# p1an-lin-jung/WavThruVec_pytorch

Hardware: AMD Instinct MI355X
Metric: audio samples/sec (16 kHz) Vec2Wav generator, B=32×256-frame 768-d latents, 1/2/4/8 GPU (higher is better)
Workload: dtype f32; 1 GPU; BASELINE configs[1]: B=32/GPU x T=256 frames, 768-d latents, upsample (5,4,4,2,2) x320, ResBlock2, train-mode CondBN, f32; global_batch=32, frames=256, parallelism=single GPU

## Files before the change

### include/vec2wav_hip.h

```cpp
#ifndef VEC2WAV_HIP_H
#define VEC2WAV_HIP_H

#include <stdint.h>

#ifdef __cplusplus
extern "C" {
#endif

#define V2W_ABI_VERSION 35

#define V2W_E_ARG      (-1)
#define V2W_E_SHAPE    (-2)
#define V2W_E_ALGO     (-3)

#define V2W_ALGO_AUTO   0
#define V2W_ALGO_DIRECT 1
#define V2W_ALGO_MFMA   2
#define V2W_ALGO_BF16   4
#define V2W_ALGO_SPLIT  3
#define V2W_ALGO_WINO   5

int         v2w_abi_version(void);
const char* v2w_build_arch(void);

// ... 86 lines not shown
typedef struct {
    const float* in; const float* in_a; const float* in_s;
    const float* wp1[4]; const float* bias1[4]; const float* wp2[4]; const float* bias2[4];
    int32_t k[4], dil1[4], dil2[4];
    float* out;
    int32_t nk, B, C, L;
    float slope, out_div;
    const float* post_w; const float* post_b; float* post_out;
    int32_t post_k;
    float post_slope;
    const float* bwd_mask1[4]; float* bwd_mid[4];
    const float* bwd_mask2; const float* bwd_mask2_a; const float* bwd_mask2_s;
    float bwd_slope;
    float* bwd_rowsum[4];
} v2w_stage_args;
int v2w_resblock2_stage_fwd(const v2w_stage_args* a, void* stream);
int v2w_resblock2_stage_bwd_rows(const v2w_stage_args* a);
int v2w_resblock2_stage_wino_fwd(const v2w_stage_args* a, void* stream);
int v2w_resblock2_stage_wino_tile(const v2w_stage_args* a);
int v2w_resblock2_stage_wino_fwd_len(const v2w_stage_args* a, const int32_t* len, int len_mul, void* stream);
int v2w_resblock2_stage_small_fwd(const v2w_stage_args* a, void* stream);

typedef struct {
    const float* in; const float* in_a; const float* in_s;
    const void*  wps1[4]; const float* sc1[4]; const float* bias1[4];
    const void*  wps2[4]; const float* sc2[4]; const float* bias2[4];
    int32_t k[4], dil1[4], dil2[4];
    float* out;
    int32_t nk, B, C, L;
    float slope, out_div;
    int32_t bf16;
    int32_t io_bf16;
    const float* post_w; const float* post_b; float* post_out;
    int32_t post_k;
    float post_slope;
    const void* up_wps; const float* up_bias; void* up_out; float* up_stats_part;
    int32_t up_k, up_u;
    float up_slope;
    int32_t rb1;
    const void* in_b[4]; void* out_b[4];
    const void* add0; const void* add1;
} v2w_stage_split_args;
int v2w_resblock2_stage_split_fwd(const v2w_stage_split_args* a, void* stream);
int v2w_resblock2_stage_split_config(const v2w_stage_split_args* a);
int v2w_resblock2_stage_up_tiles(const v2w_stage_split_args* a);

typedef struct {
    const void* in[3];
    const float* in_a; const float* in_s;
    const void* wps[3]; const float* bias[3];
    void* out[3];
    int32_t k[3], dil[3];
    int32_t nbr, mode, B, C, L;
    float slope, out_div;
    int32_t _pad;
} v2w_branch_convs_args;
int v2w_branch_convs_bf16_fwd(const v2w_branch_convs_args* a, void* stream);

typedef struct {
    const float* in; const float* wf; const float* wp; const float* bias; float* out;
    float* stats_part;
    int32_t B, C_in, C_out, L, k, u;
    float   slope;
    int32_t algo;
    int32_t io_bf16;
    int32_t _pad;
    float*  splitk_ws;
    int64_t splitk_ws_bytes;
} v2w_convt1d_args;
int v2w_convt1d_fwd(const v2w_convt1d_args* a, void* stream);
long long v2w_convt1d_splitk_ws_bytes(const v2w_convt1d_args* a);

int       v2w_pack_bf16_convt(const float* wf, void* wps, int k, int c_in, int c_out, int u, void* stream);
long long v2w_pack_bf16_convt_bytes(int k, int c_in, int c_out, int u);
int       v2w_convt1d_bf16_fwd(const v2w_convt1d_args* a, void* stream);
int       v2w_convt1d_bf16_tiles(const v2w_convt1d_args* a);

int v2w_conv1d_tile_config(const v2w_conv1d_args* a, int32_t* cfg);
int v2w_convt1d_tile_config(const v2w_convt1d_args* a, int32_t* cfg);
int v2w_conv1d_bf16_config(const v2w_conv1d_args* a, int n, int32_t* cfg);
int v2w_convt1d_bf16_config(const v2w_convt1d_args* a, int32_t* cfg);

#define V2W_MAX_STAGES 8
typedef struct {
    const float* spk; const float* noise;
    const float* fc_w[V2W_MAX_STAGES]; const float* fc_b[V2W_MAX_STAGES];
    const float* sn_w[V2W_MAX_STAGES]; const float* sn_b[V2W_MAX_STAGES];
    float* sn_u[V2W_MAX_STAGES]; float* sn_v[V2W_MAX_STAGES];
    float* gb[V2W_MAX_STAGES];
    int32_t C[V2W_MAX_STAGES];
    float* z_ws; float* sigma_ws;
    int32_t n_stages, B, spk_dim, noise_dim, training;
} v2w_cond_args;
int v2w_cond_gamma_beta(const v2w_cond_args* a, void* stream);
int v2w_cond_sigma(const v2w_cond_args* a, void* stream);
typedef struct {
    v2w_cond_args c;
    const float* running_mean[V2W_MAX_STAGES]; const float* running_var[V2W_MAX_STAGES];
    float* a_out[V2W_MAX_STAGES]; float* s_out[V2W_MAX_STAGES];
    float eps[V2W_MAX_STAGES];
} v2w_cond_eval_args;
int v2w_cond_affine_eval(const v2w_cond_eval_args* e, void* stream);

#define V2W_BN_SPLITS 64
int v2w_bn_stats(const float* x, double* stats, double* partial_ws, int B, int C, int L, void* stream);
int v2w_bn_reduce_partials(const float* part, int ntiles, int C, double count, double* stats, void* stream);
int v2w_bn_finalize(const double* stats, const float* gb,
                    float* running_mean, float* running_var, int64_t* num_batches_tracked,
                    float* a_out, float* s_out, int B, int C, int training,
                    float momentum, float eps, void* stream);
int v2w_bn_reduce_finalize(const float* part, int ntiles, double count, const float* gb,
                           float* running_mean, float* running_var, int64_t* num_batches_tracked,
                           double* stats, float* a_out, float* s_out, int B, int C, float momentum, float eps, void* stream);
int v2w_bn_reduce_slices(const float* part, int ntiles, int C, double* slices, int nslices, void* stream);
int v2w_bn_finalize_slices(const double* slices, int nslices, double count, const float* gb,
                           float* running_mean, float* running_var, int64_t* num_batches_tracked,
                           float* a_out, float* s_out, int B, int C, float momentum, float eps, void* stream);

int v2w_affine_apply(const float* x, const float* a, const float* s, float* out, int B, int C, int L, void* stream);

int v2w_wgrad_slabs(int B, int c_in, int c_out, int Lq);
int v2w_wgrad(const float* x, const float* x_a, const float* x_s, const float* dy, float* dwf, float* slab_ws,
              int B, int c_in, int c_out, int Lq, int k, int dil, int u, float slope, void* stream);

int v2w_wgrad_bf16_slabs(int B, int c_in, int c_out, int Lq, int k);
int v2w_wgrad_bf16(const void* x, const float* x_a, const float* x_s, const void* dy, float* dwf, float* slab_ws,
                   int B, int c_in, int c_out, int Lq, int k, int dil, float slope, int io_bf16, void* stream);

int v2w_cbn_bwd_sums(const float* dx, const float* xr, const float* gb, const double* stats,
                     const float* running_mean, const float* running_var, float* s12_ws, float* dgb, double* csum,
                     int B, int C, int L, int training, float eps, void* stream);
int v2w_cbn_bwd_apply(const float* dx, const float* xr, const float* gb, const double* stats, const double* csum,
                      const float* running_mean, const float* running_var, float* tab_ws, float* dxr,
                      int B, int C, int L, int training, float eps, void* stream);
int v2w_tail_bwd(const float* dy, const float* y, const float* x, const float* wf, float* dp_ws, double* part_ws,
                 float* dx, float* dwf, int B, int C_in, int L, int k, float slope, void* stream);
int v2w_wn_bwd(const float* dwf, const float* v, const float* g, float* dv, float* dg,
               int c_in, int c_out, int k, int transposed, void* stream);
int v2w_cond_bwd(const float* dgb, const float* z, const float* sn_w, const float* sn_u, const float* sn_v, const float* sigma,
                 const float* spk, const float* noise, float* d_sn_w, float* d_sn_b, float* d_fc_w, float* d_fc_b,
                 float* dz_ws, int B, int C, int spk_dim, int noise_dim, void* stream);

int v2w_conv_post_tanh_bf16in(const void* x_bf16, const float* wf, const float* bias, float* out,
                              int B, int c_in, int L, int k, float slope, void* stream);
int v2w_conv_post_tanh(const float* in, const float* wf, const float* bias, float* out,
                       int B, int C_in, int L, int k, float slope, void* stream);

int v2w_conv1d_fwd_len(const v2w_conv1d_args* a, int n, const int32_t* len, int len_mul, void* stream);
int v2w_convt1d_fwd_len(const v2w_convt1d_args* a, const int32_t* len, int len_mul, void* stream);
int v2w_conv1d_wino_sum_fwd(const v2w_conv1d_args* a, int n, const int32_t* len, int len_mul, void* stream);
int v2w_conv1d_wino_sum_fwd_order(const v2w_conv1d_args* a, int n, const int32_t* len, int len_mul, const int32_t* order, void* stream);
int v2w_wino_sum_order(const int32_t* k, int n, int32_t* order);
int v2w_conv1d_wino_fan_fwd(const v2w_conv1d_args* a, int n, void* stream);
int v2w_resblock2_stage_fwd_len(const v2w_stage_args* a, const int32_t* len, int len_mul, void* stream);
int v2w_conv_post_tanh_len(const float* in, const float* wf, const float* bias, float* out,
                           int B, int C_in, int L, int k, float slope, const int32_t* len, int len_mul, void* stream);

int v2w_mel_phases(const float* y, float* xp, int B, int L, int hop, int pad, int FP, void* stream);
int v2w_mel_finish(const float* spec, const float* basis, float* out, int B, int Cs, int FP, int F, int nb, int n_mels, void* stream);
int v2w_mel_finish_bwd(const float* spec, const float* basis, const float* basisT, const float* gout, float* dspec,
                       int B, int Cs, int FP, int F, int nb, int n_mels, void* stream);
int v2w_mel_phases_bwd(const float* dxp, float* dy, int B, int L, int hop, int pad, int FP, void* stream);
int v2w_mel_phases_len(const float* y, float* xp, int B, int L, int hop, int pad, int FP, const int32_t* len, int len_mul, void* stream);
int v2w_mel_finish_len(const float* spec, const float* basis, float* out, int B, int Cs, int FP, int F, int nb, int n_mels,
                       const int32_t* len, int len_mul, int hop, int n_fft, void* stream);
int v2w_mel_phases_geo(const float* y, float* xp, int B, int L, int n_fft, int win, int hop, int CP, int pad, int left, int k, int FP,
                       void* stream);
int v2w_mel_phases_geo_len(const float* y, float* xp, int B, int L, int n_fft, int win, int hop, int CP, int pad, int left, int k, int FP,
                           const int32_t* len, int len_mul, void* stream);
int v2w_mel_phases_geo_bwd(const float* dxp, float* dy, int B, int L, int n_fft, int win, int hop, int CP, int pad, int left, int k, int FP,
                           void* stream);
int v2w_mel_finish_geo(const float* spec, const float* basis, float* out, int B, int Cs, int FP, int F, int nb, int n_mels, void* stream);
int v2w_mel_finish_geo_len(const float* spec, const float* basis, float* out, int B, int Cs, int FP, int F, int nb, int n_mels,
                           const int32_t* len, int len_mul, int hop, int n_fft, void* stream);
int v2w_mel_finish_geo_bwd(const float* spec, const float* basis, const float* basisT, const float* gout, float* dspec,
                           int B, int Cs, int FP, int F, int nb, int n_mels, void* stream);

int v2w_phase_split(const float* x, float* out, int B, int C, int Cg, int L, int inner, int s, int ipitch, int opitch, void* stream);
int v2w_unfold1(const float* x, float* out, int B, int T, int H, int inner, int s, int k, int pad, int rows, int opitch, void* stream);
int v2w_zero_tail(float* x, long long rows, int pitch, int valid, void* stream);
int v2w_unfold_taps(const float* x, float* out, int B, int C, int L, int inner, int s, int k, int pad, int ipitch, int opitch, void* stream);
int v2w_avgpool4(const float* x, float* out, int B, int L, void* stream);

int v2w_wgrad_slice(const float* x, const float* dy, float* dwf, float* slab_ws, int B, int c_in, int c_out, int Lq,
                    int k, int dil, int tap0, int x_ct, int dy_ct, void* stream);
int v2w_wgrad_group_slabs(int B, int c_in, int c_out, int Lq, int ngroups);
int v2w_wgrad_groups(const float* x, const float* dy, float* dwf, float* slab_ws, int B, int c_in, int c_out, int Lq,
                     int k, int dil, int tap0, int ngroups, void* stream);
int v2w_disc_dz(const float* f, const float* g, const float* d, float* dz, float* rowsum, long long rows, int pitch, int valid, float slope,
                void* stream);
int v2w_rowsum_reduce(const float* rowsum, float* db, int B, int C, void* stream);
int v2w_disc_dz_merge(const float* f, const float* g, const float* dxs, float* dz, float* rowsum, int B, int C, int Cg, int L, int inner,
                      int s, int dpitch, int pitch, float slope, void* stream);
int v2w_phase_merge(const float* dxs, float* out, int B, int C, int Cg, int L, int inner, int s, int ipitch, int opitch, void* stream);
int v2w_fold1(const float* dxu, float* dx, int B, int T, int H, int inner, int s, int k, int pad, int rows, int ipitch, void* stream);
int v2w_avgpool4_bwd(const float* dout, float* dx, int B, int L, void* stream);
int v2w_cout1_wgrad(const float* x, const float* dz, float* dwf, int B, int C, int L, int k, int dil, int tap0, void* stream);

#define V2W_LOSS_MAX_ITEMS 64
#define V2W_L1_TARGET_WGS  2048
typedef struct {
    const float* a; const float* b;
    float* da; float* db;
    int64_t rows;
    int32_t valid, pitch_a, pitch_b, _pad;
} v2w_l1_pair;
typedef struct {
    const float* s;
    float* ds;
    int64_t rows;
    int32_t valid, pitch;
    float target;
    int32_t _pad;
} v2w_lsgan_item;
int       v2w_l1_multi_plan(const v2w_l1_pair* pairs, int n, int32_t* starts);
long long v2w_l1_multi_scratch_bytes(const v2w_l1_pair* pairs, int n);
int v2w_l1_mean_multi(const v2w_l1_pair* pairs, int n, float scale, float* term, float* total, void* scratch, void* stream);
int v2w_l1_mean_multi_bwd(const v2w_l1_pair* pairs, int n, float scale, const float* gout, void* stream);
int v2w_lsgan_multi(const v2w_lsgan_item* items, int n, float* term, float* total, void* stream);
int v2w_lsgan_multi_bwd(const v2w_lsgan_item* items, int n, const float* gout, const float* gterm, void* stream);
int v2w_l1_masked_plan(int C, int F);
int v2w_l1_masked(const float* a, const float* b, int B, int C, int F, const int32_t* len, int len_mul, int hop, int n_fft,
                  float* per_item, float* total, void* ws, void* stream);
int v2w_l1_masked_geo(const float* a, const float* b, int B, int C, int F, const int32_t* len, int len_mul, int hop, int n_fft,
                      float* per_item, float* total, void* ws, void* stream);

#define V2W_STFT_LOSS_MAX_ITEMS  8
#define V2W_STFT_LOSS_TARGET_WGS 1024
typedef struct {
    const float* spec_x; const float* spec_y;
    float* dspec_x;
    int32_t B, Cs, FP, F, nb, _pad;
} v2w_stft_loss_item;
int       v2w_stft_loss_plan(const v2w_stft_loss_item* items, int n, int32_t* starts);
long long v2w_stft_loss_scratch_bytes(const v2w_stft_loss_item* items, int n);
int v2w_stft_loss_multi(const v2w_stft_loss_item* items, int n, float* sc, float* mag, float* total, double* sums, void* scratch,
                        void* stream);
int v2w_stft_loss_multi_bwd(const v2w_stft_loss_item* items, int n, const double* sums, const float* g_sc, const float* g_mag,
                            const float* gterm_sc, const float* gterm_mag, void* stream);

#define V2W_ADAMW_MAX_ITEMS  80
#define V2W_ADAMW_TARGET_WGS 2048
typedef struct {
    float* p;
    const float* g;
    float* m;
    float* v;
    int64_t numel;
} v2w_adamw_item;
typedef struct {
    float lr, beta1, beta2, eps, weight_decay, bias_corr1, bias_corr2_sqrt;
    int32_t _pad;
} v2w_adamw_hyper;
int v2w_adamw_multi_plan(const v2w_adamw_item* items, int n, int32_t* starts);
int v2w_adamw_multi(const v2w_adamw_item* items, int n, const v2w_adamw_hyper* h, void* stream);

int v2w_grad_sumsq_partials(const v2w_adamw_item* items, int n);
int v2w_grad_sumsq_multi(const v2w_adamw_item* items, int n, float* partials, void* stream);
int v2w_grad_norm_finish(const float* partials, int n_partials, float max_norm, float* out, void* stream);
int v2w_scale_multi(const v2w_adamw_item* items, int n, const float* coef, void* stream);
int v2w_adamw_multi_clipped(const v2w_adamw_item* items, int n, const v2w_adamw_hyper* h, const float* clip, int skip_nonfinite, void* stream);

#define V2W_ADAMW_EMA_MAX_ITEMS 64
typedef struct {
    float* p;
    const float* g;
    float* m;
    float* v;
    float* e;
    int64_t numel;
} v2w_adamw_ema_item;
typedef struct {
    const float* p;
    float* e;
    int64_t numel;
} v2w_ema_item;
typedef struct {
    float* p;
    float* e;
    int64_t numel;
} v2w_swap_item;
int v2w_adamw_ema_multi_plan(const v2w_adamw_ema_item* items, int n, int32_t* starts);
int v2w_adamw_ema_multi(const v2w_adamw_ema_item* items, int n, const v2w_adamw_hyper* h, const float* clip, int skip_nonfinite, float ema_omd,
                        void* stream);
int v2w_ema_multi_plan(const v2w_ema_item* items, int n, int32_t* starts);
int v2w_ema_multi(const v2w_ema_item* items, int n, float ema_omd, void* stream);
int v2w_swap_multi(const v2w_swap_item* items, int n, void* stream);

#define V2W_SN_MAX_LAYERS 64
typedef struct {
    const float* w;
    float* u;
    float* v;
    float* wf;
    int32_t c_out, c_in, k;
    int32_t blk_t, blk_r, blk_s;
    int64_t ws_off, keep_off;
} v2w_sn_desc;
typedef struct {
    int32_t n, grid_t, grid_r, grid_s;
    int64_t ws_bytes, keep_bytes;
} v2w_sn_grids;
long long v2w_sn_plan(v2w_sn_desc* descs, int n, v2w_sn_grids* g);
int v2w_sn_step(const v2w_sn_desc* descs_dev, int n, int training, const v2w_sn_grids* g, float* keep, void* ws, long long ws_bytes,
                void* stream);
int v2w_sn_bwd(const v2w_sn_desc* descs_dev, int n, const v2w_sn_grids* g, const float* keep, const float* const* dwf, float* const* dw,
// ... 7 lines not shown
```

### wavthruvec_pytorch_amd/_hip.py

```python
from __future__ import annotations

import ctypes as C
import os
import threading

from . import build as _build

ABI_VERSION = 35
V2W_MAX_STAGES = 8
V2W_BN_SPLITS = 64
ALGO_AUTO, ALGO_DIRECT, ALGO_MFMA, ALGO_SPLIT, ALGO_BF16, ALGO_WINO = 0, 1, 2, 3, 4, 5

_fp = C.c_void_p


class Conv1dArgs(C.Structure):
    _fields_ = [('in_', _fp), ('in_a', _fp), ('in_s', _fp), ('wf', _fp), ('wp', _fp), ('bias', _fp),
                ('res', _fp), ('res_a', _fp), ('res_s', _fp), ('add0', _fp), ('add1', _fp),
                ('mask_src', _fp), ('mask_a', _fp), ('mask_s', _fp), ('out', _fp),
                ('B', C.c_int32), ('C_in', C.c_int32), ('C_out', C.c_int32), ('L', C.c_int32),
                ('k', C.c_int32), ('dil', C.c_int32), ('slope', C.c_float), ('accumulate', C.c_int32),
                ('out_div', C.c_float), ('algo', C.c_int32), ('mask_slope', C.c_float),
                ('in_stride', C.c_int32), ('in_phase', C.c_int32), ('pad_left', C.c_int32),
                ('wps', _fp), ('winv', _fp), ('in_ct', C.c_int32), ('out_ct', C.c_int32), ('out_slope', C.c_float),
# ... 74 lines not shown
    _fields_ = [('c', CondArgs), ('running_mean', _PA), ('running_var', _PA), ('a_out', _PA), ('s_out', _PA),
                ('eps', C.c_float * V2W_MAX_STAGES)]


class L1Pair(C.Structure):
    _fields_ = [('a', _fp), ('b', _fp), ('da', _fp), ('db', _fp), ('rows', C.c_int64),
                ('valid', C.c_int32), ('pitch_a', C.c_int32), ('pitch_b', C.c_int32), ('_pad', C.c_int32)]


class LsganItem(C.Structure):
    _fields_ = [('s', _fp), ('ds', _fp), ('rows', C.c_int64), ('valid', C.c_int32), ('pitch', C.c_int32),
                ('target', C.c_float), ('_pad', C.c_int32)]


LOSS_MAX_ITEMS = 64
L1_TARGET_WGS = 2048


class StftLossItem(C.Structure):
    _fields_ = [('spec_x', _fp), ('spec_y', _fp), ('dspec_x', _fp), ('B', C.c_int32), ('Cs', C.c_int32), ('FP', C.c_int32),
                ('F', C.c_int32), ('nb', C.c_int32), ('_pad', C.c_int32)]


STFT_LOSS_MAX_ITEMS = 8
STFT_LOSS_TARGET_WGS = 1024


class AdamWItem(C.Structure):
    _fields_ = [('p', _fp), ('g', _fp), ('m', _fp), ('v', _fp), ('numel', C.c_int64)]


class AdamWHyper(C.Structure):
    _fields_ = [('lr', C.c_float), ('beta1', C.c_float), ('beta2', C.c_float), ('eps', C.c_float), ('weight_decay', C.c_float),
                ('bias_corr1', C.c_float), ('bias_corr2_sqrt', C.c_float), ('_pad', C.c_int32)]


ADAMW_MAX_ITEMS = 80
ADAMW_TARGET_WGS = 2048


class AdamWEmaItem(C.Structure):
    _fields_ = [('p', _fp), ('g', _fp), ('m', _fp), ('v', _fp), ('e', _fp), ('numel', C.c_int64)]


class EmaItem(C.Structure):
    _fields_ = [('p', _fp), ('e', _fp), ('numel', C.c_int64)]


ADAMW_EMA_MAX_ITEMS = 64


class SnDesc(C.Structure):
    _fields_ = [('w', _fp), ('u', _fp), ('v', _fp), ('wf', _fp), ('c_out', C.c_int32), ('c_in', C.c_int32), ('k', C.c_int32),
                ('blk_t', C.c_int32), ('blk_r', C.c_int32), ('blk_s', C.c_int32), ('ws_off', C.c_int64), ('keep_off', C.c_int64)]


class SnGrids(C.Structure):
    _fields_ = [('n', C.c_int32), ('grid_t', C.c_int32), ('grid_r', C.c_int32), ('grid_s', C.c_int32), ('ws_bytes', C.c_int64), ('keep_bytes', C.c_int64)]


SN_MAX_LAYERS = 64

SIGNATURES = {
    'v2w_abi_version': (C.c_int, []),
    'v2w_build_arch': (C.c_char_p, []),
    'v2w_wn_fold_conv': (C.c_int, [_fp, _fp, _fp, _fp, C.c_int, C.c_int, C.c_int, _fp]),
    'v2w_wn_fold_convt': (C.c_int, [_fp, _fp, _fp, _fp, C.c_int, C.c_int, C.c_int, _fp]),
    'v2w_wf_transpose_flip': (C.c_int, [_fp, _fp, C.c_int, C.c_int, C.c_int, _fp]),
    'v2w_wf_gather_transpose': (C.c_int, [_fp, _fp, C.c_int, C.c_int, C.c_int, C.c_int, C.c_int, C.c_int, _fp]),
    'v2w_pack_mfma': (C.c_int, [_fp, _fp, C.c_int, C.c_int, C.c_int, C.c_int, _fp]),
    'v2w_pack_mfma_batch': (C.c_int, [_fp, _fp, C.c_int, C.c_int, C.c_int, C.c_int, C.c_int, _fp]),
    'v2w_pack_mfma_dgrad': (C.c_int, [_fp, _fp, C.c_int, C.c_int, C.c_int, _fp]),
    'v2w_pack_wino': (C.c_int, [_fp, _fp, C.c_int, C.c_int, C.c_int, _fp]),
    'v2w_wino_terms': (C.c_int, [C.c_int]),
    'v2w_split_supported': (C.c_int, [C.c_int, C.c_int, C.c_int]),
    'v2w_pack_split': (C.c_int, [_fp, _fp, _fp, C.c_int, C.c_int, C.c_int, _fp]),
    'v2w_mel_phases': (C.c_int, [_fp, _fp, C.c_int, C.c_int, C.c_int, C.c_int, C.c_int, _fp]),
    'v2w_mel_finish': (C.c_int, [_fp, _fp, _fp, C.c_int, C.c_int, C.c_int, C.c_int, C.c_int, C.c_int, _fp]),
    'v2w_mel_finish_bwd': (C.c_int, [_fp, _fp, _fp, _fp, _fp, C.c_int, C.c_int, C.c_int, C.c_int, C.c_int, C.c_int, _fp]),
    'v2w_phase_split': (C.c_int, [_fp, _fp, C.c_int, C.c_int, C.c_int, C.c_int, C.c_int, C.c_int, C.c_int, C.c_int, _fp]),
    'v2w_unfold1': (C.c_int, [_fp, _fp, C.c_int, C.c_int, C.c_int, C.c_int, C.c_int, C.c_int, C.c_int, C.c_int, C.c_int, _fp]),
    'v2w_unfold_taps': (C.c_int, [_fp, _fp] + [C.c_int] * 9 + [_fp]),
    'v2w_wgrad_slice': (C.c_int, [_fp, _fp, _fp, _fp] + [C.c_int] * 9 + [_fp]),
    'v2w_wgrad_group_slabs': (C.c_int, [C.c_int] * 5),
    'v2w_wgrad_groups': (C.c_int, [_fp, _fp, _fp, _fp] + [C.c_int] * 8 + [_fp]),
    'v2w_disc_dz': (C.c_int, [_fp, _fp, _fp, _fp, _fp, C.c_longlong, C.c_int, C.c_int, C.c_float, _fp]),
    'v2w_rowsum_reduce': (C.c_int, [_fp, _fp, C.c_int, C.c_int, _fp]),
    'v2w_disc_dz_merge': (C.c_int, [_fp, _fp, _fp, _fp, _fp] + [C.c_int] * 8 + [C.c_float, _fp]),
    'v2w_phase_merge': (C.c_int, [_fp, _fp] + [C.c_int] * 8 + [_fp]),
    'v2w_fold1': (C.c_int, [_fp, _fp] + [C.c_int] * 9 + [_fp]),
    'v2w_avgpool4_bwd': (C.c_int, [_fp, _fp, C.c_int, C.c_int, _fp]),
    'v2w_cout1_wgrad': (C.c_int, [_fp, _fp, _fp] + [C.c_int] * 6 + [_fp]),
    'v2w_zero_tail': (C.c_int, [_fp, C.c_longlong, C.c_int, C.c_int, _fp]),
    'v2w_avgpool4': (C.c_int, [_fp, _fp, C.c_int, C.c_int, _fp]),
    'v2w_mel_phases_bwd': (C.c_int, [_fp, _fp, C.c_int, C.c_int, C.c_int, C.c_int, C.c_int, _fp]),
    'v2w_split_packable': (C.c_int, [C.c_int, C.c_int]),
    'v2w_resblock2_stage_split_fwd': (C.c_int, [C.POINTER(StageSplitArgs), _fp]),
    'v2w_resblock2_stage_split_config': (C.c_int, [C.POINTER(StageSplitArgs)]),
    'v2w_resblock2_stage_up_tiles': (C.c_int, [C.POINTER(StageSplitArgs)]),
    'v2w_pack_bf16': (C.c_int, [_fp, _fp, _fp, C.c_int, C.c_int, C.c_int, _fp]),
    'v2w_split_pack_batch': (C.c_int, [_fp, _fp, C.c_int, C.c_int, C.c_int, C.c_int, C.c_int, _fp]),
    'v2w_fold_plan': (C.c_int, [C.POINTER(FoldDesc), C.c_int, C.POINTER(C.c_int32)]),
    'v2w_fold_pack_batch': (C.c_int, [_fp, _fp, C.c_int, C.c_int, C.c_int, C.c_int, _fp]),
    'v2w_conv1d_fwd': (C.c_int, [C.POINTER(Conv1dArgs), _fp]),
    'v2w_conv1d_fwd_multi': (C.c_int, [C.POINTER(Conv1dArgs), C.c_int, _fp]),
    'v2w_conv1d_splitk_ws_bytes': (C.c_longlong, [C.POINTER(Conv1dArgs), C.c_int]),
    'v2w_convt1d_splitk_ws_bytes': (C.c_longlong, [C.POINTER(ConvT1dArgs)]),
    'v2w_resblock_pair_fwd': (C.c_int, [C.POINTER(PairArgs), C.c_int, _fp]),
    'v2w_resblock2_stage_bwd_rows': (C.c_int, [C.POINTER(StageArgs)]),
    'v2w_resblock2_stage_fwd': (C.c_int, [C.POINTER(StageArgs), _fp]),
    'v2w_resblock2_stage_wino_fwd': (C.c_int, [C.POINTER(StageArgs), _fp]),
    'v2w_resblock2_stage_wino_tile': (C.c_int, [C.POINTER(StageArgs)]),
    'v2w_resblock2_stage_wino_fwd_len': (C.c_int, [C.POINTER(StageArgs), _fp, C.c_int, _fp]),
    'v2w_resblock2_stage_small_fwd': (C.c_int, [C.POINTER(StageArgs), _fp]),
    'v2w_branch_convs_bf16_fwd': (C.c_int, [C.POINTER(BranchConvsArgs), _fp]),
    'v2w_convt1d_fwd': (C.c_int, [C.POINTER(ConvT1dArgs), _fp]),
    'v2w_pack_bf16_convt': (C.c_int, [_fp, _fp, C.c_int, C.c_int, C.c_int, C.c_int, _fp]),
    'v2w_pack_bf16_convt_bytes': (C.c_longlong, [C.c_int, C.c_int, C.c_int, C.c_int]),
    'v2w_convt1d_bf16_fwd': (C.c_int, [C.POINTER(ConvT1dArgs), _fp]),
    'v2w_convt1d_bf16_tiles': (C.c_int, [C.POINTER(ConvT1dArgs)]),
    'v2w_conv1d_tile_config': (C.c_int, [C.POINTER(Conv1dArgs), C.POINTER(C.c_int32)]),
    'v2w_convt1d_tile_config': (C.c_int, [C.POINTER(ConvT1dArgs), C.POINTER(C.c_int32)]),
    'v2w_conv1d_bf16_config': (C.c_int, [C.POINTER(Conv1dArgs), C.c_int, C.POINTER(C.c_int32)]),
    'v2w_convt1d_bf16_config': (C.c_int, [C.POINTER(ConvT1dArgs), C.POINTER(C.c_int32)]),
    'v2w_cond_gamma_beta': (C.c_int, [C.POINTER(CondArgs), _fp]),
    'v2w_cond_sigma': (C.c_int, [C.POINTER(CondArgs), _fp]),
    'v2w_cond_affine_eval': (C.c_int, [C.POINTER(CondEvalArgs), _fp]),
    'v2w_bn_stats': (C.c_int, [_fp, _fp, _fp, C.c_int, C.c_int, C.c_int, _fp]),
    'v2w_bn_reduce_partials': (C.c_int, [_fp, C.c_int, C.c_int, C.c_double, _fp, _fp]),
    'v2w_bn_finalize': (C.c_int, [_fp, _fp, _fp, _fp, _fp, _fp, _fp, C.c_int, C.c_int, C.c_int,
                                  C.c_float, C.c_float, _fp]),
    'v2w_bn_reduce_finalize': (C.c_int, [_fp, C.c_int, C.c_double, _fp, _fp, _fp, _fp, _fp, _fp, _fp, C.c_int, C.c_int, C.c_float, C.c_float, _fp]),
    'v2w_bn_reduce_slices': (C.c_int, [_fp, C.c_int, C.c_int, _fp, C.c_int, _fp]),
    'v2w_bn_finalize_slices': (C.c_int, [_fp, C.c_int, C.c_double, _fp, _fp, _fp, _fp, _fp, _fp, C.c_int, C.c_int, C.c_float, C.c_float, _fp]),
    'v2w_affine_apply': (C.c_int, [_fp, _fp, _fp, _fp, C.c_int, C.c_int, C.c_int, _fp]),
    'v2w_wgrad_slabs': (C.c_int, [C.c_int, C.c_int, C.c_int, C.c_int]),
    'v2w_wgrad': (C.c_int, [_fp, _fp, _fp, _fp, _fp, _fp, C.c_int, C.c_int, C.c_int, C.c_int, C.c_int, C.c_int, C.c_int,
                            C.c_float, _fp]),
    'v2w_wgrad_bf16_slabs': (C.c_int, [C.c_int] * 5),
    'v2w_wgrad_bf16': (C.c_int, [_fp] * 6 + [C.c_int] * 6 + [C.c_float, C.c_int, _fp]),
    'v2w_cbn_bwd_sums': (C.c_int, [_fp] * 9 + [C.c_int, C.c_int, C.c_int, C.c_int, C.c_float, _fp]),
    'v2w_cbn_bwd_apply': (C.c_int, [_fp] * 9 + [C.c_int, C.c_int, C.c_int, C.c_int, C.c_float, _fp]),
    'v2w_tail_bwd': (C.c_int, [_fp] * 8 + [C.c_int, C.c_int, C.c_int, C.c_int, C.c_float, _fp]),
    'v2w_wn_bwd': (C.c_int, [_fp] * 5 + [C.c_int, C.c_int, C.c_int, C.c_int, _fp]),
    'v2w_cond_bwd': (C.c_int, [_fp] * 13 + [C.c_int, C.c_int, C.c_int, C.c_int, _fp]),
    'v2w_conv_post_tanh_bf16in': (C.c_int, [_fp, _fp, _fp, _fp, C.c_int, C.c_int, C.c_int, C.c_int, C.c_float, _fp]),
    'v2w_conv_post_tanh': (C.c_int, [_fp, _fp, _fp, _fp, C.c_int, C.c_int, C.c_int, C.c_int, C.c_float, _fp]),
    'v2w_conv1d_fwd_len': (C.c_int, [C.POINTER(Conv1dArgs), C.c_int, _fp, C.c_int, _fp]),
    'v2w_convt1d_fwd_len': (C.c_int, [C.POINTER(ConvT1dArgs), _fp, C.c_int, _fp]),
    'v2w_conv1d_wino_sum_fwd': (C.c_int, [C.POINTER(Conv1dArgs), C.c_int, _fp, C.c_int, _fp]),
    'v2w_conv1d_wino_sum_fwd_order': (C.c_int, [C.POINTER(Conv1dArgs), C.c_int, _fp, C.c_int, C.POINTER(C.c_int32), _fp]),
    'v2w_wino_sum_order': (C.c_int, [C.POINTER(C.c_int32), C.c_int, C.POINTER(C.c_int32)]),
    'v2w_conv1d_wino_fan_fwd': (C.c_int, [C.POINTER(Conv1dArgs), C.c_int, _fp]),
    'v2w_resblock2_stage_fwd_len': (C.c_int, [C.POINTER(StageArgs), _fp, C.c_int, _fp]),
    'v2w_conv_post_tanh_len': (C.c_int, [_fp, _fp, _fp, _fp, C.c_int, C.c_int, C.c_int, C.c_int, C.c_float, _fp, C.c_int, _fp]),
    'v2w_mel_phases_len': (C.c_int, [_fp, _fp, C.c_int, C.c_int, C.c_int, C.c_int, C.c_int, _fp, C.c_int, _fp]),
    'v2w_mel_finish_len': (C.c_int, [_fp, _fp, _fp, C.c_int, C.c_int, C.c_int, C.c_int, C.c_int, C.c_int, _fp, C.c_int, C.c_int, C.c_int, _fp]),
    'v2w_l1_masked_plan': (C.c_int, [C.c_int, C.c_int]),
    'v2w_l1_masked': (C.c_int, [_fp, _fp, C.c_int, C.c_int, C.c_int, _fp, C.c_int, C.c_int, C.c_int, _fp, _fp, _fp, _fp]),
    'v2w_mel_phases_geo': (C.c_int, [_fp, _fp] + [C.c_int] * 10 + [_fp]),
    'v2w_mel_phases_geo_len': (C.c_int, [_fp, _fp] + [C.c_int] * 10 + [_fp, C.c_int, _fp]),
    'v2w_mel_phases_geo_bwd': (C.c_int, [_fp, _fp] + [C.c_int] * 10 + [_fp]),
    'v2w_mel_finish_geo': (C.c_int, [_fp, _fp, _fp] + [C.c_int] * 6 + [_fp]),
    'v2w_mel_finish_geo_len': (C.c_int, [_fp, _fp, _fp] + [C.c_int] * 6 + [_fp, C.c_int, C.c_int, C.c_int, _fp]),
    'v2w_mel_finish_geo_bwd': (C.c_int, [_fp] * 5 + [C.c_int] * 6 + [_fp]),
    'v2w_l1_masked_geo': (C.c_int, [_fp, _fp, C.c_int, C.c_int, C.c_int, _fp, C.c_int, C.c_int, C.c_int, _fp, _fp, _fp, _fp]),
    'v2w_l1_multi_plan': (C.c_int, [C.POINTER(L1Pair), C.c_int, C.POINTER(C.c_int32)]),
    'v2w_l1_multi_scratch_bytes': (C.c_longlong, [C.POINTER(L1Pair), C.c_int]),
    'v2w_l1_mean_multi': (C.c_int, [C.POINTER(L1Pair), C.c_int, C.c_float, _fp, _fp, _fp, _fp]),
    'v2w_l1_mean_multi_bwd': (C.c_int, [C.POINTER(L1Pair), C.c_int, C.c_float, _fp, _fp]),
    'v2w_lsgan_multi': (C.c_int, [C.POINTER(LsganItem), C.c_int, _fp, _fp, _fp]),
    'v2w_lsgan_multi_bwd': (C.c_int, [C.POINTER(LsganItem), C.c_int, _fp, _fp, _fp]),
    'v2w_stft_loss_plan': (C.c_int, [C.POINTER(StftLossItem), C.c_int, C.POINTER(C.c_int32)]),
    'v2w_stft_loss_scratch_bytes': (C.c_longlong, [C.POINTER(StftLossItem), C.c_int]),
    'v2w_stft_loss_multi': (C.c_int, [C.POINTER(StftLossItem), C.c_int, _fp, _fp, _fp, _fp, _fp, _fp]),
    'v2w_stft_loss_multi_bwd': (C.c_int, [C.POINTER(StftLossItem), C.c_int, _fp, _fp, _fp, _fp, _fp, _fp]),
    'v2w_adamw_multi_plan': (C.c_int, [C.POINTER(AdamWItem), C.c_int, C.POINTER(C.c_int32)]),
    'v2w_adamw_multi': (C.c_int, [C.POINTER(AdamWItem), C.c_int, C.POINTER(AdamWHyper), _fp]),
    'v2w_grad_sumsq_partials': (C.c_int, [C.POINTER(AdamWItem), C.c_int]),
    'v2w_grad_sumsq_multi': (C.c_int, [C.POINTER(AdamWItem), C.c_int, _fp, _fp]),
    'v2w_grad_norm_finish': (C.c_int, [_fp, C.c_int, C.c_float, _fp, _fp]),
    'v2w_scale_multi': (C.c_int, [C.POINTER(AdamWItem), C.c_int, _fp, _fp]),
    'v2w_adamw_multi_clipped': (C.c_int, [C.POINTER(AdamWItem), C.c_int, C.POINTER(AdamWHyper), _fp, C.c_int, _fp]),
    'v2w_adamw_ema_multi_plan': (C.c_int, [C.POINTER(AdamWEmaItem), C.c_int, C.POINTER(C.c_int32)]),
    'v2w_adamw_ema_multi': (C.c_int, [C.POINTER(AdamWEmaItem), C.c_int, C.POINTER(AdamWHyper), _fp, C.c_int, C.c_float, _fp]),
    'v2w_ema_multi_plan': (C.c_int, [C.POINTER(EmaItem), C.c_int, C.POINTER(C.c_int32)]),
    'v2w_ema_multi': (C.c_int, [C.POINTER(EmaItem), C.c_int, C.c_float, _fp]),
    'v2w_swap_multi': (C.c_int, [C.POINTER(EmaItem), C.c_int, _fp]),
    'v2w_sn_plan': (C.c_longlong, [C.POINTER(SnDesc), C.c_int, C.POINTER(SnGrids)]),
    'v2w_sn_step': (C.c_int, [_fp, C.c_int, C.c_int, C.POINTER(SnGrids), _fp, _fp, C.c_longlong, _fp]),
    'v2w_sn_bwd': (C.c_int, [_fp, C.c_int, C.POINTER(SnGrids), _fp, C.POINTER(_fp), C.POINTER(_fp), _fp, C.c_longlong, _fp]),
}

LAUNCHERS = frozenset(n for n, (_r, a) in SIGNATURES.items() if a and a[-1] is _fp)

_lib = None
_tls = threading.local()


class HipLibraryError(RuntimeError):

    def __init__(self, msg, code=None):
        super().__init__(msg)
        self.code = code


E_ARG, E_SHAPE, E_ALGO = -1, -2, -3


def lib_path() -> str:
    return os.environ.get('V2W_LIB') or _build.LIB_PATH


def load():
    global _lib
    rec = getattr(_tls, 'recorder', None)
    if rec is not None:
        return rec
    if _lib is not None:
        return _lib
    import torch
    path = lib_path()
    if not os.path.exists(path):
        raise HipLibraryError(
            f'{path} not found: build it with `python -m wavthruvec_pytorch_amd.build` '
            '(or __graft_entry__.build()); there is no CPU/PyTorch fallback for the Vec2Wav hot path')
    lib = C.CDLL(path)
    for name, (res, args) in SIGNATURES.items():
        try:
            fn = getattr(lib, name)
        except AttributeError as e:
            raise HipLibraryError(f'{path} does not export {name}') from e
        fn.restype = res
        fn.argtypes = args
    if lib.v2w_abi_version() != ABI_VERSION:
        raise HipLibraryError(f'ABI version mismatch: library {lib.v2w_abi_version()}, binding {ABI_VERSION}')
    _lib = lib
    return lib


def set_recorder(rec):
    prev = getattr(_tls, 'recorder', None)
    _tls.recorder = rec
    return prev


class NameSink(C.Structure):
    _fields_ = [('magic', C.c_uint64), ('buf', C.c_void_p), ('cap', C.c_int32), ('len', C.c_int32)]


NAME_SINK_MAGIC = 0x5632574e414d4531


def kernel_name_short(full: str) -> str:
    s = full.strip()
    if s.startswith('void '):
        s = s[5:]
    s = s.replace('(anonymous namespace)::', '')
    depth = 0
    for i, ch in enumerate(s):
        if ch == '<':
            depth += 1
        elif ch == '>':
            depth -= 1
        elif ch == '(' and depth == 0:
            return s[:i]
    return s


def kernel_names(fn, *args, short=True):
    buf = C.create_string_buffer(8192)
    sink = NameSink(NAME_SINK_MAGIC, C.addressof(buf), len(buf), 0)
    rc = fn(*args, C.c_void_p(C.addressof(sink) | 1))
    names = [n for n in buf.value.decode().split('\n') if n]
    return rc, ([kernel_name_short(n) for n in names] if short else names)


def check(rc: int, what: str) -> None:
    if rc == 0:
        return
    if rc < 0:
        msg = {-1: 'bad argument', -2: 'unsupported shape for the requested algorithm', -3: 'unknown algorithm'}.get(rc, '?')
        raise HipLibraryError(f'{what}: V2W error {rc} ({msg})', rc)
    raise HipLibraryError(f'{what}: hipError_t {rc}', rc)


def ptr(t):
    return None if t is None else t.data_ptr()


def on_tensor_device(fn):
    import functools

    @functools.wraps(fn)
    def wrapper(*args, **kw):
        import torch
        for a in args:
            if isinstance(a, torch.Tensor) and a.is_cuda:
                with torch.cuda.device(a.device):
                    return fn(*args, **kw)
        return fn(*args, **kw)
    return wrapper


def current_stream_handle(device) -> int:
    import torch
# ... 2 lines not shown
```

### wavthruvec_pytorch_amd/csrc/v2w_conv_mfma.hip

```cpp
#include <type_traits>
#include "v2w_tile.h"
#include "v2w_internal.h"
#include "v2w_wino.h"

#ifdef V2W_TIMELINE
V2W_TL_SETTER(v2w_timeline_set_tile)
#endif

namespace {

template <int MF, int U, int MI, int NI, int WM, int WN, int CK, int NPF, int RING, int EPI, bool VEC>
__global__ void __launch_bounds__(64 * WM * WN, (U == 1 && MI * NI >= 4) ? 3 : 1)
conv_tile_kernel(const MultiArgs m) {
    constexpr bool LEN = EPI == 3;
    typedef Frag<MF> F;
    typedef typename F::acc_t acc_t;
    constexpr int NTHREADS = 64 * WM * WN;
    constexpr int MT = MF * MI * WM;
    constexpr int NT = MF * NI * WN;
    constexpr int KSTEP = F::KSTEP;
    constexpr int CKG = 4 * KSTEP;
    constexpr int GPC = CK / CKG;
    constexpr int RS = TileGeom<MF, CK>::RS;
    static_assert(CK % CKG == 0, "chunk must hold whole A fragments");
// ... 592 lines not shown
        for (int i = 0; i < nprob && ok; ++i) {
            const TileArgs& p = m.p[i];
            const size_t n = (size_t)p.B * p.Cout * p.L * U;
            ok = !p.stats_part && p.CoutT == p.Cout && p.Cin / CK == nch;
            vec = vec && (p.L * U) % 4 == 0 && v2w_al16(p.out) && v2w_al16(p.res) && v2w_al16(p.add0) && v2w_al16(p.add1);
            floats += n * s2;
        }
        if (m.p[0].ws_query) {
            *m.p[0].ws_query = ok ? (long long)(floats * sizeof(float)) : 0;
            return 0;
        }
        if (ok && m.p[0].splitk_ws && (long long)(floats * sizeof(float)) <= m.p[0].splitk_ws_bytes) {
            float* ws = m.p[0].splitk_ws;
            {
                S = s2;
                red_vec = vec;
                size_t off = 0;
                long long f4 = 0;
                for (int i = 0; i < nprob; ++i) {
                    TileArgs& p = m.p[i];
                    const size_t n = (size_t)p.B * p.Cout * p.L * U;
                    red.e[i] = SplitEpi{ws + off, p.out, p.bias, p.res, p.res_a, p.res_s, p.add0, p.add1, p.accumulate, p.out_div, p.Cout, p.L * U, n};
                    red.start[i] = f4;
                    f4 += vec ? (long long)(n / 4) : (long long)p.B * p.Cout * p.L * U;
                    p.out = ws + off; p.bias = nullptr; p.res = p.res_a = p.res_s = nullptr; p.add0 = p.add1 = nullptr;
                    p.accumulate = 0; p.out_div = 0.f; p.ksplit = S;
                    p.evec = U == 1 && p.L % 4 == 0;
                    off += n * S;
                    blocks[i] *= S;
                }
                grid = v2w_fill_starts(m.start, V2W_MAX_MULTI, blocks, nprob);
                red.start[nprob] = f4;
                red.n = nprob; red.S = S;
            }
        }
    }
    if (m.p[0].ws_query) { *m.p[0].ws_query = 0; return 0; }
    bool vec = true, len = false;
    for (int i = 0; i < nprob; ++i) { vec = vec && m.p[i].vec4; len = len || m.p[i].len; }
    if (len && epi != 0) return V2W_E_ARG;
    const int e = len ? 3 : epi;
    auto pick = [&](auto vec_c) {
        constexpr bool V = decltype(vec_c)::value;
        return e == 1 ? conv_tile_kernel<MF, U, MI, NI, WM, WN, CK, NPF, RING, 1, V>
             : e == 2 ? conv_tile_kernel<MF, U, MI, NI, WM, WN, CK, NPF, RING, 2, V>
             : e == 3 ? conv_tile_kernel<MF, U, MI, NI, WM, WN, CK, NPF, RING, 3, V> : conv_tile_kernel<MF, U, MI, NI, WM, WN, CK, NPF, RING, 0, V>;
    };
    const int rc = v2w_launch_lds(vec ? pick(std::true_type{}) : pick(std::false_type{}), dim3(grid), dim3(NTHREADS), lds, stream, m);
    if (rc != 0 || S == 1) return rc;
    long long rblocks = (red.start[nprob] + 255) / 256;
    if (rblocks > 2048) rblocks = 2048;
    if (red_vec) V2W_LAUNCH(splitk_reduce_kernel<true>, dim3((int)rblocks), dim3(256), 0, stream, red);
    else V2W_LAUNCH(splitk_reduce_kernel<false>, dim3((int)rblocks), dim3(256), 0, stream, red);
    return v2w_launch_status();
}

template <int U>
int launch_convt_u(TileArgs p, hipStream_t stream) {
    if (p.Cout % 64 == 0) return launch_tile<32, U, 1, 1, 2, 2, 16>(&p, 1, stream);
    if (p.Cout == 32) return launch_tile<32, U, 1, 1, 1, 4, 16>(&p, 1, stream);
    if (p.Cout == 16) return launch_tile<16, U, 1, 2, 1, 4, 16>(&p, 1, stream);
    return V2W_E_SHAPE;
}

__global__ void __launch_bounds__(256)
pack_mfma_kernel(const float* wf, float* wp, int K, int Cin, int Cout, int MF, int CK, int U, int tflip = 0) {
    const int KSTEP = MF == 32 ? 2 : 4, CKG = 4 * KSTEP, GPC = CK / CKG, nch = Cin / CK;
    const int pad = (K - U) / 2;
    const size_t total = (size_t)K * Cin * Cout;
    wf += (size_t)blockIdx.y * total; wp += (size_t)blockIdx.y * total;
    for (size_t o = (size_t)blockIdx.x * 256 + threadIdx.x; o < total; o += (size_t)gridDim.x * 256) {
        const int j = o & 3;
        const int lane = (o >> 2) & 63;
        size_t rest = o >> 8;
        const int gg = rest % GPC; rest /= GPC;
        const int ts = rest % K; rest /= K;
        const int ch = rest % nch;
        const int mb = rest / nch;
        int t = ts;
        if (U > 1) {
            int left = ts;
            for (int r = 0; r < U; ++r) {
                const int t0 = (r + pad) % U, nt = (K - t0 + U - 1) / U;
                if (left < nt) { t = t0 + left * U; break; }
                left -= nt;
            }
        }
        const int c = ch * CK + gg * CKG + j * KSTEP + lane / MF;
        const int co = mb * MF + lane % MF;
        wp[o] = tflip ? wf[((size_t)(K - 1 - t) * Cout + co) * Cin + c] : wf[((size_t)t * Cin + c) * Cout + co];
    }
}


__device__ __forceinline__ int find_layer(const int32_t* __restrict__ starts, int n, int blk) {
    int lo = 0, hi = n;
    while (hi - lo > 1) { const int mid = (lo + hi) >> 1; if (starts[mid] <= blk) lo = mid; else hi = mid; }
    return lo;
}

__global__ void __launch_bounds__(256)
fold_scale_batch_kernel(const v2w_fold_desc* __restrict__ descs, const int32_t* __restrict__ starts, int n) {
    __shared__ double red[16];
    const int li = find_layer(starts, n, blockIdx.x);
    const v2w_fold_desc d = descs[li];
    const int row = blockIdx.x - starts[li];
    const int inner = (d.transposed ? d.c_out : d.c_in) * d.k;
    const float* src = d.v + (size_t)row * inner;
    double acc = 0.0;
    if (d.g)
        for (int i = threadIdx.x; i < inner; i += 256) { const double x = (double)src[i]; acc += x * x; }
    const double n2 = v2w_block_sum(acc, red);
    if (threadIdx.x == 0) d.scale[row] = d.g ? (float)((double)d.g[row] / sqrt(n2)) : 1.f;
}

__global__ void __launch_bounds__(256)
fold_pack_batch_kernel(const v2w_fold_desc* __restrict__ descs, const int32_t* __restrict__ starts, int n) {
    extern __shared__ float tile[];
    const int li = find_layer(starts, n, blockIdx.x);
    const v2w_fold_desc d = descs[li];
    const int blk = blockIdx.x - starts[li];
    const int MF = d.mf, CK = d.ck, K = d.k, U = d.u;
    const int KSTEP = MF == 32 ? 2 : 4, CKG = 4 * KSTEP, GPC = CK / CKG, nch = d.c_in / CK;
    const int mb = blk / nch, ch = blk % nch;
    const int nrow = d.transposed ? CK : MF;
    const int rlen = (d.transposed ? MF : CK) * K;
    const int rstride = rlen + 1;
    for (int idx = threadIdx.x; idx < nrow * rlen; idx += 256) {
        const int r = idx / rlen, x = idx - r * rlen;
        const float* src = d.transposed ? d.v + ((size_t)(ch * CK + r) * d.c_out + mb * MF) * K
                                        : d.v + ((size_t)(mb * MF + r) * d.c_in + ch * CK) * K;
        const float sc = d.scale[d.transposed ? ch * CK + r : mb * MF + r];
        tile[r * rstride + x] = src[x] * sc;
    }
    __syncthreads();
    const int pad = (K - U) / 2;
    float* dst = d.wp + (size_t)(mb * nch + ch) * K * GPC * 256;
    for (int o = threadIdx.x; o < K * GPC * 256; o += 256) {
        const int j = o & 3, lane = (o >> 2) & 63;
        const int rest = o >> 8;
        const int gg = rest % GPC, ts = rest / GPC;
        int t = ts;
        if (U > 1) {
            int left = ts;
            for (int r = 0; r < U; ++r) {
                const int t0 = (r + pad) % U, nt = (K - t0 + U - 1) / U;
                if (left < nt) { t = t0 + left * U; break; }
                left -= nt;
            }
        }
        const int c = gg * CKG + j * KSTEP + lane / MF, co = lane % MF;
        dst[o] = d.transposed ? tile[c * rstride + co * K + t] : tile[co * rstride + c * K + t];
    }
    if (d.wpw) {
        const int nfr = wino_terms(K) * GPC;
        float* dw = d.wpw + (size_t)(mb * nch + ch) * nfr * 256;
        for (int o = threadIdx.x; o < nfr * 256; o += 256) {
            const int j = o & 3, lane = (o >> 2) & 63;
            int s0, ntap, gg, term;
            wino_frag(K, GPC, o >> 8, s0, ntap, gg, term);
            const int c = gg * CKG + j * KSTEP + lane / MF, co = lane % MF;
            const float* w = tile + co * rstride + c * K + s0;
            dw[o] = wino_weight(ntap, term, w[0], ntap > 1 ? w[1] : 0.f, ntap > 2 ? w[2] : 0.f);
        }
    }
    if (d.wf) {
        for (int idx = threadIdx.x; idx < K * CK * MF; idx += 256) {
            const int col = idx % MF, c = (idx / MF) % CK, t = idx / (MF * CK);
            d.wf[((size_t)t * d.c_in + ch * CK + c) * d.c_out + mb * MF + col] =
                d.transposed ? tile[c * rstride + col * K + t] : tile[col * rstride + c * K + t];
        }
    }
    if (d.wpd) {
        const int nchd = d.c_out / CK;
        float* dd = d.wpd + (size_t)(ch * nchd + mb) * K * GPC * 256;
        for (int o = threadIdx.x; o < K * GPC * 256; o += 256) {
            const int j = o & 3, lane = (o >> 2) & 63;
            const int rest = o >> 8;
            const int gg = rest % GPC, ts = rest / GPC;
            const int kc = gg * CKG + j * KSTEP + lane / MF, row = lane % MF;
            dd[o] = tile[kc * rstride + row * K + (K - 1 - ts)];
        }
    }
}

}

struct LayerCfg { int mf, ck; };
static LayerCfg v2w_layer_cfg(int c_in, int c_out, int u) {
    LayerCfg c{0, 0};
    if (c_in % 16 != 0) return c;
    if (u == 1) {
        if (c_out % 32 == 0 && c_in % 32 == 0) c = {32, 32};
        else if (c_out % 32 == 0) c = {32, 16};
        else if (c_out == 16) c = {16, 16};
    } else if (u == 2 || u == 4 || u == 5 || u == 8) {
        if (c_out % 64 == 0 || c_out == 32) c = {32, 16};
        else if (c_out == 16) c = {16, 16};
    }
    return c;
}

static int pack_mfma(const float* wf, float* wp, int k, int c_in, int c_out, int u, int n, int tflip, void* stream) {
    if (!wf || !wp || k <= 0 || c_in <= 0 || c_out <= 0 || u <= 0) return V2W_E_ARG;
    const LayerCfg cfg = v2w_layer_cfg(c_in, c_out, u);
    if (!cfg.mf) return V2W_E_SHAPE;
    const size_t total = (size_t)k * c_in * c_out;
    int grid = (int)((total + 255) / 256); if (grid > 4096) grid = 4096;
    V2W_LAUNCH(pack_mfma_kernel, dim3(grid, n), dim3(256), 0, (hipStream_t)stream, wf, wp, k, c_in, c_out, cfg.mf, cfg.ck, u, tflip);
    return v2w_launch_status();
}

extern "C" int v2w_pack_mfma(const float* wf, float* wp, int k, int c_in, int c_out, int u, void* stream) {
    return pack_mfma(wf, wp, k, c_in, c_out, u, 1, 0, stream);
}

extern "C" int v2w_pack_mfma_dgrad(const float* wf, float* wp, int k, int c_in, int c_out, void* stream) {
    return pack_mfma(wf, wp, k, c_in, c_out, 1, 1, 1, stream);
}

extern "C" int v2w_pack_mfma_batch(const float* wf, float* wp, int k, int c_in, int c_out, int u, int n, void* stream) {
    if (n <= 0 || n > 65535) return V2W_E_ARG;
    return pack_mfma(wf, wp, k, c_in, c_out, u, n, 0, stream);
}

int v2w_conv1d_mfma(const v2w_conv1d_args* a, int n, hipStream_t stream, int* cfg_out, long long* ws_query, const int32_t* len, int len_mul) {
    if (n < 1 || n > V2W_MAX_MULTI) return V2W_E_ARG;
    const LayerCfg cfg = v2w_layer_cfg(a->C_in, a->C_out, 1);
    if (!cfg.mf) return V2W_E_SHAPE;
    TileArgs ps[V2W_MAX_MULTI];
    long tiles128 = 0;
    for (int i = 0; i < n; ++i) {
        const v2w_conv1d_args* q = a + i;
        if (q->B != a->B || q->C_in != a->C_in || q->C_out != a->C_out || q->L != a->L) return V2W_E_SHAPE;
        if (!q->wp && !cfg_out && !ws_query) return V2W_E_SHAPE;
        TileArgs p{};
        p.cfg_out = cfg_out;
        p.in = q->in; p.in_a = q->in_a; p.in_s = q->in_s; p.wp = q->wp; p.bias = q->bias;
        p.res = q->res; p.res_a = q->res_a; p.res_s = q->res_s; p.out = q->out;
        p.add0 = q->add0; p.add1 = q->add1;
        p.mask_src = q->mask_src; p.mask_a = q->mask_a; p.mask_s = q->mask_s; p.mask_slope = q->mask_slope;
        p.stats_part = q->rowsum_part;
        p.B = q->B; p.Cin = q->C_in; p.Cout = q->C_out; p.L = q->L; p.K = q->k; p.dil = q->dil;
        p.CinT = q->in_ct > 0 ? q->in_ct : q->C_in; p.CoutT = q->out_ct > 0 ? q->out_ct : q->C_out;
        p.out_slope = q->out_slope > 0.f ? q->out_slope : 1.f;
        p.pad = 0; p.hl = p.hr = q->dil * (q->k - 1) / 2;
        if (q->pad_left >= 0) { p.hl = q->pad_left; p.hr = q->dil * (q->k - 1) - q->pad_left; if (p.hr < 0) return V2W_E_ARG; }
        p.in_stride = q->in_stride > 0 ? q->in_stride : 1; p.in_phase = q->in_phase;
        p.slope = q->slope; p.accumulate = q->accumulate; p.out_div = q->out_div;
        p.splitk_ws = a->splitk_ws; p.splitk_ws_bytes = a->splitk_ws ? a->splitk_ws_bytes : 0; p.ws_query = ws_query;
        if (len) {
            if (len_mul < 1 || q->mask_src || q->rowsum_part || p.out_slope != 1.f || p.in_stride != 1 || p.CinT != p.Cin || p.CoutT != p.Cout)
                return V2W_E_ARG;
            p.len = len; p.len_mul = len_mul;
        }
        ps[i] = p;
        tiles128 += (long)p.B * ((p.L + 127) / 128) * (p.Cout / 128);
    }
    int halo = 0;
    for (int i = 0; i < n; ++i) { const int h = ((ps[i].hl + 3) & ~3) > ps[i].hr ? ((ps[i].hl + 3) & ~3) : ps[i].hr; if (h > halo) halo = h; }
    if (halo > 32) {
        if (halo > 48 || cfg.mf != 32 || cfg.ck != 32 || a->C_out % 64 != 0) return V2W_E_SHAPE;
        if (a->C_out % 128 == 0 && tiles128 >= 4 * 256) return launch_tile<32, 1, 2, 2, 2, 2, 32, 48>(ps, n, stream);
        return launch_tile<32, 1, 1, 2, 2, 2, 32, 48>(ps, n, stream);
    }
    if (cfg.mf == 32 && cfg.ck == 32 && a->C_out % 64 == 0 && (long)n * a->B * ((a->L + 63) / 64) * (a->C_out / 64) < 512)
        return launch_tile<32, 1, 1, 1, 2, 2, 32>(ps, n, stream);
    if (cfg.mf == 32 && cfg.ck == 32 && a->C_out % 128 == 0) {
        if (tiles128 >= 4 * 256) return launch_tile<32, 1, 2, 2, 2, 2, 32>(ps, n, stream);
        return launch_tile<32, 1, 2, 1, 2, 2, 32>(ps, n, stream);
    }
    if (cfg.mf == 32 && cfg.ck == 32 && a->C_out % 64 == 0) return launch_tile<32, 1, 1, 2, 2, 2, 32>(ps, n, stream);
    if (cfg.mf == 32 && cfg.ck == 16) return launch_tile<32, 1, 1, 2, 1, 4, 16>(ps, n, stream);
    if (cfg.mf == 32) return launch_tile<32, 1, 1, 2, 1, 4, 32>(ps, n, stream);
    if (cfg.mf == 16) return launch_tile<16, 1, 1, 4, 1, 4, 16>(ps, n, stream);
    return V2W_E_SHAPE;
}

int v2w_convt1d_mfma(const v2w_convt1d_args* a, hipStream_t stream, int* cfg_out, long long* ws_query, const int32_t* len, int len_mul) {
    const LayerCfg cfg = v2w_layer_cfg(a->C_in, a->C_out, a->u);
    if ((!a->wp && !cfg_out && !ws_query) || !cfg.mf) return V2W_E_SHAPE;
    TileArgs p{};
    p.cfg_out = cfg_out;
    p.splitk_ws = a->splitk_ws; p.splitk_ws_bytes = a->splitk_ws ? a->splitk_ws_bytes : 0; p.ws_query = ws_query;
    p.in = a->in; p.wp = a->wp; p.bias = a->bias; p.out = a->out; p.stats_part = a->stats_part;
    if (len && (len_mul < 1 || a->stats_part)) return V2W_E_ARG;
    p.len = len; p.len_mul = len_mul;
    p.B = a->B; p.Cin = a->C_in; p.Cout = a->C_out; p.L = a->L; p.K = a->k; p.dil = 1;
    p.CinT = p.Cin; p.CoutT = p.Cout; p.out_slope = 1.f;
    p.pad = (a->k - a->u) / 2;
    p.slope = a->slope; p.accumulate = 0; p.out_div = 0.f;
    int hl = 0, hr = 0;
    for (int r = 0; r < a->u; ++r) {
        const int rp = r + p.pad, t0 = rp % a->u, c = rp / a->u, nt = (a->k - t0 + a->u - 1) / a->u;
        if (c > hr) hr = c;
        if (nt - 1 - c > hl) hl = nt - 1 - c;
    }
    p.hl = hl; p.hr = hr;
    switch (a->u) {
        case 2: return launch_convt_u<2>(p, stream);
        case 4: return launch_convt_u<4>(p, stream);
        case 5: return launch_convt_u<5>(p, stream);
        case 8: return launch_convt_u<8>(p, stream);
        default: return V2W_E_SHAPE;
    }
}

extern "C" int v2w_fold_plan(v2w_fold_desc* descs, int n, int32_t* starts) {
    if (!descs || !starts || n <= 0) return V2W_E_ARG;
    int bs = 0, bp = 0, lds = 0;
    for (int i = 0; i < n; ++i) {
        v2w_fold_desc& d = descs[i];
        if (d.c_in <= 0 || d.c_out <= 0 || d.k <= 0 || d.u <= 0) return V2W_E_ARG;
        const LayerCfg cfg = v2w_layer_cfg(d.c_in, d.c_out, d.transposed ? d.u : 1);
        if (!cfg.mf) return V2W_E_SHAPE;
        d.mf = cfg.mf; d.ck = cfg.ck;
        if (d.wpd && (d.transposed || d.c_in != d.c_out || cfg.mf != cfg.ck)) return V2W_E_ARG;
        if (d.wpw && (d.transposed || cfg.mf != 32 || cfg.ck != 32 || wino_terms(d.k) == 0)) return V2W_E_ARG;
        starts[i] = bs; starts[n + 1 + i] = bp;
        bs += d.transposed ? d.c_in : d.c_out;
        bp += (d.c_out / cfg.mf) * (d.c_in / cfg.ck);
        const int nrow = d.transposed ? cfg.ck : cfg.mf, rlen = (d.transposed ? cfg.mf : cfg.ck) * d.k;
        const int bytes = nrow * (rlen + 1) * (int)sizeof(float);
        if (bytes > lds) lds = bytes;
    }
    starts[n] = bs; starts[2 * n + 1] = bp;
    if (lds > 160 * 1024) return V2W_E_SHAPE;
    return lds;
}

extern "C" int v2w_fold_pack_batch(const v2w_fold_desc* descs_dev, const int32_t* starts_dev, int n,
                                   int nblk_scale, int nblk_pack, int lds_bytes, void* stream) {
    if (!descs_dev || !starts_dev || n <= 0 || nblk_scale <= 0 || nblk_pack <= 0 || lds_bytes <= 0) return V2W_E_ARG;
    hipStream_t st = (hipStream_t)stream;
    if (lds_bytes > 64 * 1024) {
        hipError_t e = v2w_max_lds(reinterpret_cast<const void*>(fold_pack_batch_kernel), lds_bytes, st);
        if (e != hipSuccess) return (int)e;
    }
    V2W_LAUNCH(fold_scale_batch_kernel, dim3(nblk_scale), dim3(256), 0, st, descs_dev, starts_dev, n);
    V2W_LAUNCH(fold_pack_batch_kernel, dim3(nblk_pack), dim3(256), lds_bytes, st, descs_dev, starts_dev + n + 1, n);
    return v2w_launch_status();
}
```

### wavthruvec_pytorch_amd/csrc/v2w_conv_wino.hip

```cpp
#include "v2w_tile.h"
#include "v2w_internal.h"
#include "v2w_wino.h"

namespace {

constexpr int WCK = 32;
typedef TileGeom<32, WCK> WG;
constexpr int WGPC = 4;
constexpr int WHMAX = 32;
__host__ __device__ inline int wino_tpos(int P, int d) { const int q = P / d; return 2 * d * q + (P - q * d); }
__host__ __device__ inline int wino_npairs(int L, int d) { return d * ((L + 2 * d - 1) / (2 * d)); }

__host__ __device__ inline void wino_tile_order(int v, int B, int ntl, bool tail_last, int& b, int& tl) {
    b = v / ntl; tl = v - b * ntl;
    if (tail_last) {
        const int nf = ntl - 1, nfull = B * nf;
        if (v >= nfull) { b = v - nfull; tl = nf; }
        else { b = v / nf; tl = v - b * nf; }
    }
}

constexpr int WSRC = 3;
struct WinoSumArgs {
    TileArgs p;
    const float* in[WSRC]; const float* wp[WSRC];
    int K[WSRC], hl[WSRC];
    const float* res[WSRC]; const float* bias[WSRC];
    int nsrc;
};
struct WinoFanArgs {
    TileArgs p;
    const float* wp[WSRC]; const float* bias[WSRC]; float* out[WSRC];
    int K[WSRC], hl[WSRC];
    int nsrc;
};
__device__ __forceinline__ const TileArgs& wino_problem(const MultiArgs& m, int pq) { return m.p[pq]; }
__device__ __forceinline__ const TileArgs& wino_problem(const WinoSumArgs& a, int) { return a.p; }
__device__ __forceinline__ const TileArgs& wino_problem(const WinoFanArgs& a, int) { return a.p; }

template <int MI, int WN, int NPF, bool VEC, bool LEN, class ARGS>
__device__ __forceinline__ void conv_wino_body(const ARGS& m) {
    constexpr bool SUM = std::is_same<ARGS, WinoSumArgs>::value;
    constexpr bool FAN = std::is_same<ARGS, WinoFanArgs>::value;
    static_assert(!FAN || (MI == 1 && !LEN), "the fan-out form is written for MI = 1 without per-item lengths");
    typedef Frag<32> F;
    typedef F::acc_t acc_t;
    constexpr int WM = 2;
    constexpr int NTHREADS = 64 * WM * WN;
    constexpr int MT = 32 * MI * WM;
    constexpr int NTP = 32 * WN;
    constexpr int RING = 4;

    extern __shared__ __attribute__((aligned(16))) float smem[];

    int pq = 0, id = blockIdx.x;
    if constexpr (!SUM && !FAN) { pq = tile_problem(m); id = blockIdx.x - m.start[pq]; }
    const TileArgs& p = wino_problem(m, pq);
    const int mtiles = p.Cout / MT;
    const TileId ti = tile_coords(mtiles, id);
    const int mt = ti.mt;
    if (ti.tile >= p.ntiles) return;
    const int d = p.dil;
    int b, tl;
    wino_tile_order(ti.tile, p.B, p.ntl, wino_npairs(p.L, d) % NTP != 0, b, tl);
    const int P0 = tl * NTP;
    const int m0 = mt * MT;
    int Lb = p.L;
    if constexpr (LEN) {
        const int lv = p.len[b] * p.len_mul;
        Lb = lv < p.L ? lv : p.L;
        if (wino_tpos(P0, d) >= Lb) return;
    }

    const int tid = threadIdx.x;
    const int lane = tid & 63;
    const int wave = __builtin_amdgcn_readfirstlane(tid >> 6);
    const int lr = lane & 31;
    const int hk = lane >> 5;
    const int wm0 = (wave / WN) * (32 * MI);
    const int wn0 = (wave % WN) * 32;
    const bool live = wino_tpos(P0 + wn0, d) < Lb;
    const int L = p.L;
    int K = p.K, hl = p.hl;
    const float* sin = p.in;
    int pos0 = (wino_tpos(P0, d) - hl) & ~3;
    if constexpr (FAN) { K = m.K[0]; hl = m.hl[0]; }
    const float slope = p.slope;
    const int nch = p.Cin / WCK;
    const int bufsz = p.xrows * WG::RS;
    float* const etab = smem + p.atab_off;
    float* const atab = etab + (FAN ? WSRC + 2 : 3) * MT;

    acc_t acc[4][MI];
#pragma unroll
    for (int c = 0; c < 4; ++c)
#pragma unroll
        for (int i = 0; i < MI; ++i)
#pragma unroll
            for (int e = 0; e < 16; ++e) acc[c][i][e] = 0.f;

    const int nq = p.xrows >> 2;
    const int nq8 = (nq + 7) >> 3;
    const unsigned magic = (unsigned)(((1ull << 32) + nq8 - 1) / nq8);
    f32x4 pf[NPF][2];
    const f32x4 zero4 = {0.f, 0.f, 0.f, 0.f};
    auto item = [&](int s, int& c0, int& row, bool& in_img, bool& in_seq) {
        int t = tid;
        asm volatile("" : "+v"(t));
        const int idx = t + s * NTHREADS;
        const int g = idx >> 4;
        const int pg = (int)__umulhi((unsigned)g, magic);
        const int quad = (g - pg * nq8) * 8 + (idx & 7);
        const int P = 2 * pg + ((idx >> 3) & 1);
        row = quad * 4;
        in_img = quad < nq && P < WCK / 2;
        c0 = WG::pair_c0(in_img ? P : 0);
        const int pos = pos0 + row;
        in_seq = in_img && pos >= 0 && pos < L;
    };
    auto prefetch = [&](int ci0) {
        const float* xsrc = sin + (size_t)(b * p.CinT + ci0) * L + pos0;
#pragma unroll
        for (int s = 0; s < NPF; ++s) {
            int c0, row; bool in_img, in_seq;
            item(s, c0, row, in_img, in_seq);
            pf[s][0] = zero4; pf[s][1] = zero4;
            if (in_seq) {
                pf[s][0] = *reinterpret_cast<const f32x4*>(xsrc + (size_t)c0 * L + row);
                pf[s][1] = *reinterpret_cast<const f32x4*>(xsrc + (size_t)(c0 + 2) * L + row);
            }
        }
    };
    auto commit = [&](int ci0, float* Xs) {
#pragma unroll
        for (int s = 0; s < NPF; ++s) {
            int c0, row; bool in_img, in_seq;
            item(s, c0, row, in_img, in_seq);
            if (!in_img) continue;
            float a0 = 1.f, s0 = 0.f, a1 = 1.f, s1 = 0.f;
            if (!SUM && p.in_a) {
                a0 = atab[ci0 + c0]; s0 = atab[p.Cin + ci0 + c0];
                a1 = atab[ci0 + c0 + 2]; s1 = atab[p.Cin + ci0 + c0 + 2];
            }
            float* dst = Xs + row * WG::RS + WG::slot(c0);
#pragma unroll
            for (int e = 0; e < 4; ++e) {
                f32x2 v = {0.f, 0.f};
                if (in_seq && (!LEN || pos0 + row + e < Lb)) {
                    v[0] = v2w_lrelu(fmaf(a0, pf[s][0][e], s0), slope); v[1] = v2w_lrelu(fmaf(a1, pf[s][1][e], s1), slope);
                }
                *reinterpret_cast<f32x2*>(dst + e * WG::RS) = v;
            }
        }
    };
    auto stage_scalar = [&](int ci0, float* Xs) {
        for (int c = wave; c < WCK; c += WM * WN) {
            const int ch = b * p.CinT + ci0 + c;
            const float* xsrc = sin + (size_t)ch * L;
            const float av = !SUM && p.in_a ? p.in_a[ch] : 1.f;
            const float sv = !SUM && p.in_s ? p.in_s[ch] : 0.f;
            float* dst = Xs + WG::slot(c);
            for (int j = lane; j < p.xrows; j += 64) {
                const int l = pos0 + j;
                float v = 0.f;
                if (l >= 0 && l < Lb) v = v2w_lrelu(fmaf(av, xsrc[l], sv), slope);
                dst[j * WG::RS] = v;
            }
        }
    };

    int nfrag = nch * wino_terms(K) * WGPC;
    const f32x4* ap[MI];
#pragma unroll
    for (int i = 0; i < MI; ++i)
        ap[i] = reinterpret_cast<const f32x4*>(p.wp) + ((size_t)((m0 + wm0) / 32 + i) * nfrag) * 64;
    int fidx = 0;
    f32x4 ar[RING][MI];
    const unsigned lane16 = (unsigned)lane * 16u;
    auto load_next = [&](f32x4 (&a)[MI]) {
        const int f = fidx < nfrag ? fidx : nfrag - 1;
        unsigned l16 = lane16;
        asm volatile("" : "+v"(l16));
#pragma unroll
        for (int i = 0; i < MI; ++i)
            a[i] = *reinterpret_cast<const f32x4*>(reinterpret_cast<const char*>(ap[i] + (size_t)f * 64) + l16);
        ++fidx;
    };

    auto segment = [&](auto ntap_c, const float* x, int dstep) {
        constexpr int NTAP = decltype(ntap_c)::value;
        constexpr int NX = NTAP + 1;
        constexpr int NTERM = wino_seg_terms(NTAP);
#pragma unroll
        for (int gg = 0; gg < WGPC; ++gg) {
            f32x4 xr[NX];
#pragma unroll
            for (int j = 0; j < NX; ++j) xr[j] = *reinterpret_cast<const f32x4*>(x + j * dstep + 8 * gg);
            f32x4 u[NTERM];
            if constexpr (NTAP == 3) {
                u[0] = xr[0] - xr[2]; u[1] = xr[1] + xr[2];
                u[2] = xr[2] - xr[1]; u[3] = xr[1] - xr[3];
            } else if constexpr (NTAP == 2) {
                u[0] = xr[0] - xr[1]; u[1] = xr[1]; u[2] = xr[1] - xr[2];
            } else {
                u[0] = xr[0]; u[1] = xr[1];
            }
            __builtin_amdgcn_sched_barrier(0);
#pragma unroll
            for (int t = 0; t < NTERM; ++t) {
                const int cls = NTAP == 3 ? t : (NTAP == 2 ? (t == 2 ? 3 : t) : (t == 1 ? 3 : 0));
                const int slot = (gg * NTERM + t) % RING;
                load_next(ar[(slot + RING - 1) % RING]);
#pragma unroll
                for (int kk = 0; kk < 4; ++kk)
#pragma unroll
                    for (int i = 0; i < MI; ++i) acc[cls][i] = F::mfma(ar[slot][i][kk], u[t][kk], acc[cls][i]);
            }
        }
    };

    int nsrc = 1;
    if constexpr (SUM || FAN) nsrc = m.nsrc;
    for (int c = tid; c < MT; c += NTHREADS) {
        if constexpr (FAN) {
            for (int j = 0; j < nsrc; ++j) etab[j * MT + c] = m.bias[j] ? m.bias[j][m0 + c] : 0.f;
            etab[WSRC * MT + c] = p.res_a ? p.res_a[b * p.Cout + m0 + c] : 1.f;
            etab[(WSRC + 1) * MT + c] = p.res_a ? p.res_s[b * p.Cout + m0 + c] : 0.f;
            continue;
        }
        if constexpr (SUM) {
            float bv = m.bias[0] ? m.bias[0][m0 + c] : 0.f;
            for (int j = 1; j < nsrc; ++j) bv += m.bias[j] ? m.bias[j][m0 + c] : 0.f;
            etab[c] = bv;
            continue;
        }
        etab[c] = p.bias ? p.bias[m0 + c] : 0.f;
        etab[MT + c] = p.res_a ? p.res_a[b * p.Cout + m0 + c] : 1.f;
        etab[2 * MT + c] = p.res_a ? p.res_s[b * p.Cout + m0 + c] : 0.f;
    }
    if (!SUM && p.in_a) {
        for (int c = tid; c < p.Cin; c += NTHREADS) {
            atab[c] = p.in_a[b * p.Cin + c];
            atab[p.Cin + c] = p.in_s[b * p.Cin + c];
        }
        __syncthreads();
    }
    if constexpr (VEC) { prefetch(0); commit(0, smem); }
    else stage_scalar(0, smem);
#pragma unroll
    for (int g = 0; g + 1 < RING; ++g) load_next(ar[g]);
    __builtin_amdgcn_sched_barrier(0);
    __syncthreads();

    const int P = P0 + wn0 + lr;
    const int t0 = wino_tpos(P, d);
    int lbase = (t0 - hl - pos0) * WG::RS + 4 * hk;
    const int dstep = d * WG::RS;
    typedef std::integral_constant<int, 3> S3;
    typedef std::integral_constant<int, 2> S2;
    typedef std::integral_constant<int, 1> S1;
    auto fan_epilogue = [&](int j) {
        if constexpr (FAN) {
            float* const outp = m.out[j];
            const float* const res = p.res;
            const float* const bt = etab + j * MT;
            constexpr int EB = 4;
            int lq = tid;
            asm volatile("" : "+v"(lq));
            const int tq = wino_tpos(P0 + wn0 + (lq & 31), d), hq = (lq & 63) >> 5;
#pragma unroll
            for (int e0 = 0; e0 < 16; e0 += EB) {
                float rv[EB][2];
#pragma unroll
                for (int q = 0; q < EB; ++q) {
                    const size_t rowoff = ((size_t)b * p.CoutT + m0 + wm0 + F::row(e0 + q, hq)) * L;
#pragma unroll
                    for (int h = 0; h < 2; ++h) {
                        const int pos = tq + h * d;
                        rv[q][h] = (res && pos < L) ? res[rowoff + pos] : 0.f;
                    }
                }
#pragma unroll
                for (int q = 0; q < EB; ++q) {
                    const int e = e0 + q, col = wm0 + F::row(e, hq);
                    const float M0 = acc[0][0][e], M1 = acc[1][0][e], M2 = acc[2][0][e], M3 = acc[3][0][e];
                    const float y[2] = {(M0 + M1) + M2, (M1 - M2) - M3};
                    const size_t rowoff = ((size_t)b * p.CoutT + m0 + col) * L;
                    const float bias = bt[col], ra = etab[WSRC * MT + col], rs = etab[(WSRC + 1) * MT + col];
#pragma unroll
                    for (int h = 0; h < 2; ++h) {
                        const int pos = tq + h * d;
                        if (pos >= L) continue;
                        float t = y[h] + bias;
                        if (res) t += fmaf(ra, rv[q][h], rs);
                        outp[rowoff + pos] = t;
                    }
                }
            }
        }
    };
    for (int js = 0, cc = 0; js < nsrc; ++js) {
        for (int ch = 0; ch < nch; ++ch, ++cc) {
            const int par = SUM ? cc : ch;
            const float* Xs = smem + (par & 1) * bufsz;
            float* Xn = smem + ((par + 1) & 1) * bufsz;
            bool more = ch + 1 < nch;
            if constexpr (FAN) more = more && js == 0;
            int cn = (ch + 1) * WCK;
            if (live) {
                const float* xt = Xs + lbase;
                int s = 0;
                for (; s + 3 <= K; s += 3) segment(S3{}, xt + s * dstep, dstep);
                if (K - s == 2) segment(S2{}, xt + s * dstep, dstep);
                else if (K - s == 1) segment(S1{}, xt + s * dstep, dstep);
            }
            if constexpr (SUM) {
                if (!more && js + 1 < nsrc) {
                    more = true; cn = 0;
                    K = m.K[js + 1]; hl = m.hl[js + 1]; sin = m.in[js + 1];
                    pos0 = (wino_tpos(P0, d) - hl) & ~3;
                    lbase = (t0 - hl - pos0) * WG::RS + 4 * hk;
                    nfrag = nch * wino_terms(K) * WGPC;
#pragma unroll
                    for (int i = 0; i < MI; ++i)
                        ap[i] = reinterpret_cast<const f32x4*>(m.wp[js + 1]) + ((size_t)((m0 + wm0) / 32 + i) * nfrag) * 64;
                    fidx = 0;
#pragma unroll
                    for (int g = 0; g + 1 < RING; ++g) load_next(ar[g]);
                }
            }
            if (more) {
                if constexpr (VEC) { prefetch(cn); commit(cn, Xn); }
                else stage_scalar(cn, Xn);
                __syncthreads();
            }
        }
        if constexpr (FAN) {
            if (!live) return;
            if (js + 1 < nsrc) {
                K = m.K[js + 1];
                lbase += (hl - m.hl[js + 1]) * WG::RS;
                hl = m.hl[js + 1];
                nfrag = nch * wino_terms(K) * WGPC;
#pragma unroll
                for (int i = 0; i < MI; ++i)
                    ap[i] = reinterpret_cast<const f32x4*>(m.wp[js + 1]) + ((size_t)((m0 + wm0) / 32 + i) * nfrag) * 64;
                fidx = 0;
#pragma unroll
                for (int g = 0; g + 1 < RING; ++g) load_next(ar[g]);
            }
            fan_epilogue(js);
#pragma unroll
            for (int c = 0; c < 4; ++c)
#pragma unroll
                for (int i = 0; i < MI; ++i)
#pragma unroll
                    for (int e = 0; e < 16; ++e) acc[c][i][e] = 0.f;
        }
    }
    if constexpr (FAN) return;

    if (!live) return;
    float* const outp = p.out;
    const float dinv = p.out_div != 0.f ? 1.f / p.out_div : 1.f;
    if constexpr (SUM) {
        auto epilogue = [&](auto ns_c) {
            constexpr int NS = decltype(ns_c)::value;
            constexpr int NR = NS ? NS : WSRC;
            constexpr int EB = 4;
            const int ns = NS ? NS : nsrc;
#pragma unroll
            for (int e0 = 0; e0 < 16; e0 += EB) {
                float rv[EB][2][NR];
#pragma unroll
                for (int q = 0; q < EB; ++q) {
                    const size_t rowoff = ((size_t)b * p.CoutT + m0 + wm0 + F::row(e0 + q, hk)) * L;
#pragma unroll
                    for (int h = 0; h < 2; ++h) {
                        const int pos = t0 + h * d;
#pragma unroll
                        for (int j = 0; j < NR; ++j) rv[q][h][j] = (pos < L && j < ns) ? m.res[j][rowoff + pos] : 0.f;
                    }
                }
#pragma unroll
                for (int q = 0; q < EB; ++q) {
                    const int e = e0 + q, col = wm0 + F::row(e, hk);
                    const float M0 = acc[0][0][e], M1 = acc[1][0][e], M2 = acc[2][0][e], M3 = acc[3][0][e];
                    const float y[2] = {(M0 + M1) + M2, (M1 - M2) - M3};
                    const size_t rowoff = ((size_t)b * p.CoutT + m0 + col) * L;
                    const float bias = etab[col];
#pragma unroll
                    for (int h = 0; h < 2; ++h) {
                        const int pos = t0 + h * d;
                        if (pos >= L) continue;
                        float t = y[h] + bias;
                        float r = rv[q][h][0];
                        if (NS == 3) r = (r + rv[q][h][1]) + rv[q][h][2];
                        else {
#pragma unroll
                            for (int j = 1; j < NR; ++j) if (j < ns) r += rv[q][h][j];
                        }
                        t += r;
                        if (p.out_div != 0.f) t = v2w_div_by(t, p.out_div, dinv);
                        outp[rowoff + pos] = t;
                    }
                }
            }
        };
        static_assert(!SUM || MI == 1, "the summed form's epilogue is written for MI = 1");
        if (nsrc == 3) epilogue(std::integral_constant<int, 3>{});
        else epilogue(std::integral_constant<int, 0>{});
        return;
    }
#pragma unroll
    for (int i = 0; i < MI; ++i) {
#pragma unroll
        for (int e = 0; e < 16; ++e) {
            const int col = wm0 + i * 32 + F::row(e, hk);
            const float M0 = acc[0][i][e], M1 = acc[1][i][e], M2 = acc[2][i][e], M3 = acc[3][i][e];
            const float y[2] = {(M0 + M1) + M2, (M1 - M2) - M3};
            const size_t rowoff = ((size_t)b * p.CoutT + m0 + col) * L;
            const float bias = etab[col], ra = etab[MT + col], rs = etab[2 * MT + col];
#pragma unroll
            for (int h = 0; h < 2; ++h) {
                const int pos = t0 + h * d;
                if (pos >= L) continue;
                const size_t go = rowoff + pos;
                float t = y[h] + bias;
                if (p.res) t += fmaf(ra, p.res[go], rs);
                if (p.add1) t += p.add0[go] + p.add1[go];
                else if (p.accumulate) t += outp[go];
                else if (p.add0) t += p.add0[go];
                if (p.out_div != 0.f) t = v2w_div_by(t, p.out_div, dinv);
                outp[go] = t;
            }
        }
    }
}

template <int MI, int WN, int NPF, bool VEC>
__global__ void __launch_bounds__(128 * WN, 3)
conv_wino_kernel(const MultiArgs m) {
    conv_wino_body<MI, WN, NPF, VEC, false>(m);
}

template <int MI, int WN, int NPF, bool VEC>
__global__ void __launch_bounds__(128 * WN, 3)
conv_wino_len_kernel(const MultiArgs m) {
    conv_wino_body<MI, WN, NPF, VEC, true>(m);
}

template <int MI, int WN, int NPF, bool VEC>
__global__ void __launch_bounds__(128 * WN, 3)
conv_wino_sum_kernel(const WinoSumArgs a) {
    conv_wino_body<MI, WN, NPF, VEC, false>(a);
}

template <int MI, int WN, int NPF, bool VEC>
__global__ void __launch_bounds__(128 * WN, 3)
conv_wino_sum_len_kernel(const WinoSumArgs a) {
    conv_wino_body<MI, WN, NPF, VEC, true>(a);
}

template <int MI, int WN, int NPF, bool VEC>
__global__ void __launch_bounds__(128 * WN, 3)
conv_wino_fan_kernel(const WinoFanArgs a) {
    conv_wino_body<MI, WN, NPF, VEC, false>(a);
}

template <int MI, int WN>
int launch_wino(const TileArgs* ps, int nprob, hipStream_t stream) {
    constexpr int MT = 64 * MI, NTP = 32 * WN, NTHREADS = 128 * WN;
    constexpr int NPF = ((WCK / 2) * (((2 * NTP + 2 * WHMAX) / 4 + 7) / 8 * 8) + NTHREADS - 1) / NTHREADS;
    static_assert(NTHREADS * NPF < 8 * 8192, "item index range of the magic division");
    MultiArgs m{};
    size_t lds = 0;
    int blocks[V2W_MAX_MULTI];
    bool vec = true;
    for (int i = 0; i < nprob; ++i) {
        TileArgs p = ps[i];
        if (p.Cout % MT != 0) return V2W_E_SHAPE;
        const int d = p.dil;
        p.ntl = (wino_npairs(p.L, d) + NTP - 1) / NTP;
        p.ntiles = p.B * p.ntl;
        int rows = 0;
        for (int tl = 0; tl < p.ntl; ++tl) {
            const int P0 = tl * NTP;
            const int pos0 = (wino_tpos(P0, d) - p.hl) & ~3;
            const int r = wino_tpos(P0 + NTP - 1, d) + d + p.hr - pos0 + 1;
            if (r > rows) rows = r;
        }
        p.xrows = (rows + 3) & ~3;
        if (p.xrows > 2 * NTP + 2 * WHMAX) return V2W_E_SHAPE;
        p.vec4 = (p.L % 4 == 0) && v2w_al16(p.in);
        vec = vec && p.vec4;
        const int nbuf = p.Cin / WCK > 1 ? 2 : 1;
        p.atab_off = nbuf * p.xrows * WG::RS;
        const size_t l = ((size_t)p.atab_off + 3 * MT + (p.in_a ? 2 * p.Cin : 0)) * sizeof(float);
        if (l > lds) lds = l;
        m.p[i] = p;
        blocks[i] = tile_blocks(p.ntiles, p.Cout / MT);
    }
    const int grid = v2w_fill_starts(m.start, V2W_MAX_MULTI, blocks, nprob);
    const bool lens = m.p[0].len != nullptr;
    auto kern = lens ? (vec ? conv_wino_len_kernel<MI, WN, NPF, true> : conv_wino_len_kernel<MI, WN, NPF, false>)
                    : (vec ? conv_wino_kernel<MI, WN, NPF, true> : conv_wino_kernel<MI, WN, NPF, false>);
    return v2w_launch_lds(kern, dim3(grid), dim3(NTHREADS), lds, stream, m);
}

inline void wino_sum_order(const int* Ks, int nsrc, int* walk) {
    (void)Ks;
    for (int j = 0; j < nsrc; ++j) walk[j] = j;
}

template <int MI, int WN>
int launch_wino_sum(const TileArgs* ps, int nsrc, const int32_t* order, hipStream_t stream) {
    constexpr int MT = 64 * MI, NTP = 32 * WN, NTHREADS = 128 * WN;
    constexpr int NPF = ((WCK / 2) * (((2 * NTP + 2 * WHMAX) / 4 + 7) / 8 * 8) + NTHREADS - 1) / NTHREADS;
    WinoSumArgs a{};
    int walk[WSRC];
    int Ks[WSRC];
    for (int j = 0; j < nsrc; ++j) Ks[j] = ps[j].K;
    wino_sum_order(Ks, nsrc, walk);
    if (order) {
        unsigned seen = 0;
        for (int j = 0; j < nsrc; ++j) {
            if (order[j] < 0 || order[j] >= nsrc || (seen >> order[j] & 1u)) return V2W_E_ARG;
            seen |= 1u << order[j];
            walk[j] = order[j];
        }
    }
    TileArgs p = ps[walk[0]];
    if (p.Cout % MT != 0) return V2W_E_SHAPE;
    const int d = p.dil;
    p.ntl = (wino_npairs(p.L, d) + NTP - 1) / NTP;
    p.ntiles = p.B * p.ntl;
    int rows = 0;
    bool vec = p.L % 4 == 0;
    for (int j = 0; j < nsrc; ++j) {
        for (int tl = 0; tl < p.ntl; ++tl) {
            const int P0 = tl * NTP;
            const int pos0 = (wino_tpos(P0, d) - ps[j].hl) & ~3;
            const int r = wino_tpos(P0 + NTP - 1, d) + d + ps[j].hr - pos0 + 1;
            if (r > rows) rows = r;
        }
        vec = vec && v2w_al16(ps[j].in);
        const TileArgs& w = ps[walk[j]];
        a.in[j] = w.in; a.wp[j] = w.wp; a.K[j] = w.K; a.hl[j] = w.hl;
        a.res[j] = ps[j].in; a.bias[j] = ps[j].bias;
    }
    a.nsrc = nsrc;
    p.xrows = (rows + 3) & ~3;
    if (p.xrows > 2 * NTP + 2 * WHMAX) return V2W_E_SHAPE;
    p.vec4 = vec;
    const int nbuf = nsrc * (p.Cin / WCK) > 1 ? 2 : 1;
    p.atab_off = nbuf * p.xrows * WG::RS;
    const size_t lds = ((size_t)p.atab_off + 3 * MT) * sizeof(float);
    a.p = p;
    const int grid = tile_blocks(p.ntiles, p.Cout / MT);
    auto kern = p.len ? (vec ? conv_wino_sum_len_kernel<MI, WN, NPF, true> : conv_wino_sum_len_kernel<MI, WN, NPF, false>)
                      : (vec ? conv_wino_sum_kernel<MI, WN, NPF, true> : conv_wino_sum_kernel<MI, WN, NPF, false>);
    return v2w_launch_lds(kern, dim3(grid), dim3(NTHREADS), lds, stream, a);
}

template <int MI, int WN>
int launch_wino_fan(const TileArgs* ps, int nsrc, hipStream_t stream) {
    constexpr int MT = 64 * MI, NTP = 32 * WN, NTHREADS = 128 * WN;
    constexpr int NPF = ((WCK / 2) * (((2 * NTP + 2 * WHMAX) / 4 + 7) / 8 * 8) + NTHREADS - 1) / NTHREADS;
    WinoFanArgs a{};
    TileArgs p = ps[0];
    const int nch = p.Cin / WCK;
    if (p.Cout % MT != 0 || nch > 2) return V2W_E_SHAPE;
    int hmax = 0;
    for (int j = 0; j < nsrc; ++j) {
        a.wp[j] = ps[j].wp; a.bias[j] = ps[j].bias; a.out[j] = ps[j].out; a.K[j] = ps[j].K; a.hl[j] = ps[j].hl;
        if (ps[j].hl > hmax) hmax = ps[j].hl;
    }
    a.nsrc = nsrc;
    p.hl = p.hr = hmax;
    const int d = p.dil;
    p.ntl = (wino_npairs(p.L, d) + NTP - 1) / NTP;
    p.ntiles = p.B * p.ntl;
    int rows = 0;
    for (int tl = 0; tl < p.ntl; ++tl) {
        const int P0 = tl * NTP;
        const int pos0 = (wino_tpos(P0, d) - hmax) & ~3;
        const int r = wino_tpos(P0 + NTP - 1, d) + d + hmax - pos0 + 1;
        if (r > rows) rows = r;
    }
    p.xrows = (rows + 3) & ~3;
    if (p.xrows > 2 * NTP + 2 * WHMAX) return V2W_E_SHAPE;
    const bool vec = (p.L % 4 == 0) && v2w_al16(p.in);
    p.vec4 = vec;
    p.atab_off = nch * p.xrows * WG::RS;
    const size_t lds = ((size_t)p.atab_off + (WSRC + 2) * MT + (p.in_a ? 2 * p.Cin : 0)) * sizeof(float);
    a.p = p;
    const int grid = tile_blocks(p.ntiles, p.Cout / MT);
    auto kern = vec ? conv_wino_fan_kernel<MI, WN, NPF, true> : conv_wino_fan_kernel<MI, WN, NPF, false>;
    return v2w_launch_lds(kern, dim3(grid), dim3(NTHREADS), lds, stream, a);
}

__global__ void __launch_bounds__(256)
pack_wino_kernel(const float* __restrict__ wf, float* __restrict__ wp, int K, int Cin, int Cout) {
    const int nch = Cin / WCK, nfr = wino_terms(K) * WGPC;
    const size_t total = (size_t)(Cout / 32) * nch * nfr * 256;
    for (size_t o = (size_t)blockIdx.x * 256 + threadIdx.x; o < total; o += (size_t)gridDim.x * 256) {
        const int j = o & 3, lane = (o >> 2) & 63;
        size_t rest = o >> 8;
        const int fi = rest % nfr; rest /= nfr;
        const int ch = rest % nch;
        const int mb = rest / nch;
        int s0, ntap, gg, term;
        wino_frag(K, WGPC, fi, s0, ntap, gg, term);
        const int c = ch * WCK + gg * 8 + 2 * j + lane / 32, co = mb * 32 + lane % 32;
        auto g = [&](int t) { return t < ntap ? wf[((size_t)(s0 + t) * Cin + c) * Cout + co] : 0.f; };
        wp[o] = wino_weight(ntap, term, g(0), g(1), g(2));
    }
}

}

int v2w_conv1d_wino(const v2w_conv1d_args* a, int n, hipStream_t stream, const int32_t* len, int len_mul) {
    if (n < 1 || n > V2W_MAX_MULTI) return V2W_E_ARG;
    TileArgs ps[V2W_MAX_MULTI];
    long wgs = 0;
    const int MT = 64;
    for (int i = 0; i < n; ++i) {
        const v2w_conv1d_args* q = a + i;
        if (q->B != a->B || q->C_in != a->C_in || q->C_out != a->C_out || q->L != a->L) return V2W_E_SHAPE;
        if (q->C_in % WCK != 0 || q->C_in < 64 || q->C_out % 64 != 0 || wino_terms(q->k) == 0 || q->pad_left >= 0) return V2W_E_SHAPE;
        if (q->in_stride > 1 || q->mask_src || q->rowsum_part || (q->out_slope != 0.f && q->out_slope != 1.f)) return V2W_E_SHAPE;
        if ((q->in_ct > 0 && q->in_ct != q->C_in) || (q->out_ct > 0 && q->out_ct != q->C_out)) return V2W_E_SHAPE;
        if (!q->wp) return V2W_E_ARG;
        if (len && len_mul < 1) return V2W_E_ARG;
        TileArgs p{};
        p.len = len; p.len_mul = len_mul;
        p.in = q->in; p.in_a = q->in_a; p.in_s = q->in_s; p.wp = q->wp; p.bias = q->bias;
        p.res = q->res; p.res_a = q->res_a; p.res_s = q->res_s; p.out = q->out;
        p.add0 = q->add0; p.add1 = q->add1;
        p.B = q->B; p.Cin = q->C_in; p.Cout = q->C_out; p.L = q->L; p.K = q->k; p.dil = q->dil;
        p.CinT = q->C_in; p.CoutT = q->C_out;
        p.hl = p.hr = q->dil * (q->k - 1) / 2;
        p.slope = q->slope; p.accumulate = q->accumulate; p.out_div = q->out_div;
        ps[i] = p;
        wgs += (long)q->B * ((wino_npairs(q->L, q->dil) + 63) / 64) * (q->C_out / MT);
    }
    if (wgs <= 128) return V2W_E_SHAPE;
    return launch_wino<1, 2>(ps, n, stream);
}

extern "C" int v2w_conv1d_wino_sum_fwd(const v2w_conv1d_args* a, int n, const int32_t* len, int len_mul, void* stream) {
    return v2w_conv1d_wino_sum_fwd_order(a, n, len, len_mul, nullptr, stream);
}

extern "C" int v2w_conv1d_wino_sum_fwd_order(const v2w_conv1d_args* a, int n, const int32_t* len, int len_mul, const int32_t* order, void* stream) {
    if (!a || n < 1 || n > WSRC || (len && len_mul < 1)) return V2W_E_ARG;
    TileArgs ps[WSRC];
    for (int i = 0; i < n; ++i) {
        const v2w_conv1d_args* q = a + i;
        if (!q->in || !q->wp || !a->out) return V2W_E_ARG;
        if (q->B <= 0 || q->C_in <= 0 || q->L <= 0 || q->k <= 0 || q->dil <= 0) return V2W_E_ARG;
        if (q->res || q->res_a || q->add0 || q->add1 || q->accumulate || (q->in_a == nullptr) != (q->in_s == nullptr)) return V2W_E_ARG;
        if (q->B != a->B || q->C_in != a->C_in || q->C_out != a->C_in || q->L != a->L || q->dil != a->dil || q->slope != a->slope) return V2W_E_SHAPE;
        if (q->in_a) return V2W_E_SHAPE;
        if (q->C_in % 64 != 0 || wino_terms(q->k) == 0 || q->pad_left >= 0) return V2W_E_SHAPE;
        if (q->in_stride > 1 || q->mask_src || q->rowsum_part || q->out_slope != 0.f || q->in_ct > 0 || q->out_ct > 0) return V2W_E_SHAPE;
        TileArgs p{};
        p.len = len; p.len_mul = len_mul;
        p.in = q->in; p.wp = q->wp; p.bias = q->bias; p.out = a->out;
        p.B = q->B; p.Cin = p.Cout = p.CinT = p.CoutT = q->C_in; p.L = q->L; p.K = q->k; p.dil = q->dil;
        p.hl = p.hr = q->dil * (q->k - 1) / 2;
        p.slope = q->slope; p.out_div = a->out_div;
        ps[i] = p;
    }
    return launch_wino_sum<1, 2>(ps, n, order, (hipStream_t)stream);
}

extern "C" int v2w_conv1d_wino_fan_fwd(const v2w_conv1d_args* a, int n, void* stream) {
    if (!a || n < 1 || n > WSRC) return V2W_E_ARG;
    TileArgs ps[WSRC];
    for (int i = 0; i < n; ++i) {
        const v2w_conv1d_args* q = a + i;
        if (!q->in || !q->wp || !q->out) return V2W_E_ARG;
        if (q->B <= 0 || q->C_in <= 0 || q->C_out <= 0 || q->L <= 0 || q->k <= 0 || q->dil <= 0) return V2W_E_ARG;
        if ((q->in_a == nullptr) != (q->in_s == nullptr) || (q->res_a == nullptr) != (q->res_s == nullptr)) return V2W_E_ARG;
        if (q->in != a->in || q->in_a != a->in_a || q->in_s != a->in_s || q->res != a->res || q->res_a != a->res_a || q->res_s != a->res_s)
            return V2W_E_ARG;
        if (q->B != a->B || q->C_in != a->C_in || q->C_out != a->C_out || q->L != a->L || q->dil != a->dil || q->slope != a->slope) return V2W_E_ARG;
        for (int j = 0; j < i; ++j)
            if (a[j].out == q->out) return V2W_E_ARG;
        if (q->C_in % WCK != 0 || q->C_in < 64 || q->C_out % 64 != 0 || wino_terms(q->k) == 0 || q->pad_left >= 0) return V2W_E_SHAPE;
        if (q->in_stride > 1 || q->mask_src || q->rowsum_part || (q->out_slope != 0.f && q->out_slope != 1.f)) return V2W_E_SHAPE;
        if (q->in_ct > 0 || q->out_ct > 0) return V2W_E_SHAPE;
        if (q->add0 || q->add1 || q->accumulate || q->out_div != 0.f) return V2W_E_SHAPE;
        TileArgs p{};
        p.in = q->in; p.in_a = q->in_a; p.in_s = q->in_s; p.wp = q->wp; p.bias = q->bias;
        p.res = q->res; p.res_a = q->res_a; p.res_s = q->res_s; p.out = q->out;
        p.B = q->B; p.Cin = q->C_in; p.Cout = q->C_out; p.L = q->L; p.K = q->k; p.dil = q->dil;
        p.CinT = q->C_in; p.CoutT = q->C_out;
        p.hl = p.hr = q->dil * (q->k - 1) / 2;
        p.slope = q->slope;
        ps[i] = p;
    }
    return launch_wino_fan<1, 2>(ps, n, (hipStream_t)stream);
}

extern "C" int v2w_wino_sum_order(const int32_t* k, int n, int32_t* order) {
    if (!k || !order || n < 1 || n > WSRC) return V2W_E_ARG;
    int Ks[WSRC], walk[WSRC];
    for (int j = 0; j < n; ++j) Ks[j] = k[j];
    wino_sum_order(Ks, n, walk);
    for (int j = 0; j < n; ++j) order[j] = walk[j];
    return 0;
}

extern "C" int v2w_wino_terms(int k) { return wino_terms(k); }

extern "C" int v2w_pack_wino(const float* wf, float* wpw, int k, int c_in, int c_out, void* stream) {
    if (!wf || !wpw || k <= 0 || c_in <= 0 || c_out <= 0) return V2W_E_ARG;
    if (wino_terms(k) == 0 || c_in % WCK != 0 || c_out % 32 != 0) return V2W_E_SHAPE;
    const size_t total = (size_t)wino_terms(k) * c_in * c_out;
    int grid = (int)((total + 255) / 256); if (grid > 4096) grid = 4096;
    V2W_LAUNCH(pack_wino_kernel, dim3(grid), dim3(256), 0, (hipStream_t)stream, wf, wpw, k, c_in, c_out);
    return v2w_launch_status();
}
```

### wavthruvec_pytorch_amd/forward_plan.py

```python
from __future__ import annotations

import contextlib

import torch

from . import hipops

LRELU_SLOPE = 0.1
_Z_CHANNEL = 128


class DirectStreams:

    def __init__(self, main, side, side2=None):
        self.main, self.side, self.side2 = main, side, side if side2 is None else side2
        self.events = {}
        self.nfork = 1
        self.tag = None

    def stream(self, sid):
        return (self.main, self.side, self.side2)[sid]

    def fork(self, sides=1):
        self.nfork = sides
        for q in (self.side, self.side2)[:sides]:
            q.wait_stream(self.main)

    def join(self):
        for q in (self.side, self.side2)[:self.nfork]:
            self.main.wait_stream(q)

    def mark(self, name, sid=1):
        ev = torch.cuda.Event()
        ev.record(self.stream(sid))
        self.events[name] = ev

    def need(self, name):
        self.main.wait_event(self.events[name])

    def py(self, fn, tag=None):
        return fn()

    def keep(self, obj):
        pass


STAGE_WINO_BLOCKS = [(3, 1, 3), (7, 1, 3), (11, 1, 3)]


def stage_wino_selected(wino_stage, precision, algo, C, blocks) -> bool:
    return bool(wino_stage) and precision == 'f32' and algo != hipops.ALGO_DIRECT and C == 32 and list(blocks) == STAGE_WINO_BLOCKS


def wino_sum_selected(wino_sum, precision, algo, C, blocks) -> bool:
    blocks = list(blocks)
    return (C in tuple(wino_sum or ()) and precision == 'f32' and algo != hipops.ALGO_DIRECT and C % 64 == 0 and 2 <= len(blocks) <= 3
            and all(k >= 3 and k % 2 == 1 and d == blocks[0][1] for k, d in blocks))


def wino_fan_selected(wino_fan, precision, algo, C, blocks, *, save=False, lengths=False, streams=True) -> bool:
    blocks = list(blocks)
    return (C in tuple(wino_fan or ()) and precision == 'f32' and algo != hipops.ALGO_DIRECT and not save and not lengths and bool(streams)
            and 1 <= len(blocks) <= 3 and all(k >= 3 and k % 2 == 1 and d == blocks[0][1] for k, d in blocks))


def _branches(rbs, names, wps):
    return [dict(wps1=wps[nm + '.convs.0'], b1=rb.convs[0].bias.detach(), wps2=wps[nm + '.convs.1'], b2=rb.convs[1].bias.detach(),
                 k=rb.kernel_size, dil1=rb.convs[0].dilation, dil2=rb.convs[1].dilation) for nm, rb in zip(names, rbs)]


class ForwardPlanner:
    def __init__(self, g, x, spk, nz, save, S, lens=None):
        self.g, self.x, self.spk, self.nz, self.save, self.S = g, x, spk, nz, save, S
        self.lens = lens
        self.lmul = 1
        self.dev = x.device
        self.B, _, self.T = x.shape
        self.training = g.training
        self.algo = g.algo
        self.nk, self.ns = g.num_kernels, g.num_upsamples
        self.marked = set()
        self.order = []
        self.needed = set()

    def run(self):
        g = self.g
        keep_ws = None
        if self.save is not None:
            keep_ws, g._ws = g._ws, {}
        try:
            with torch.no_grad():
                self.begin()
                self.weights()
                self.conv_pre()
                for i in range(self.ns):
                    self.stage(i)
                y = self.tail()
            if self.save is not None:
                self.hand_over(y)
        finally:
            if keep_ws is not None:
                g._ws = keep_ws
        return y

    def timed(self, tag, fn, *args, **kw):
        g = self.g
        self.S.tag = tag
        try:
            if g._profile is None or not isinstance(self.S, DirectStreams):
                return fn(*args, **kw)
            e0, e1 = torch.cuda.Event(enable_timing=True), torch.cuda.Event(enable_timing=True)
            pn = g._profile_names
            e0.record()
            if pn is not None:
                from . import _hip, schedule
                prev = _hip.set_recorder(schedule.NameProbe(_hip.load(), pn.setdefault(tag, [])))
                try:
                    r = fn(*args, **kw)
                finally:
                    _hip.set_recorder(prev)
            else:
                r = fn(*args, **kw)
            e1.record()
            g._profile.append((tag, e0, e1))
            return r
        finally:
            self.S.tag = None

    def on_side(self, sid=1):
        return torch.cuda.stream(self.S.stream(sid))

    def mark(self, name, sid=1):
        self.S.mark(name, sid)
        self.marked.add(name)
        self.order.append((name, sid))

    def need(self, *names):
        want = [nm for nm in names if nm in self.marked and nm not in self.needed]
        if not self.g.merge_waits:
            for nm in want:
                self.needed.add(nm)
                self.S.need(nm)
            return
        for sid in sorted({s for n, s in self.order if n in want}):
            seq = [n for n, s in self.order if s == sid]
            last = max(seq.index(n) for n in want if n in seq)
            self.S.need(seq[last])
            self.needed.update(seq[:last + 1])

    def join_side(self):
        if not self.joined:
            self.S.join()
            self.joined = True

    def begin(self):
        g, x = self.g, self.x
        from .models import ResBlock1, ResBlock2
        self.fuse_stage = () if self.save is not None else g.fuse_stage
        self.fuse_pairs = () if self.save is not None else g.fuse_pairs
        self.adt = torch.float32
        rb1_net = all(isinstance(rb, ResBlock1) for rb in g.resblocks)
        if (g.precision == 'bf16' and g.bf16_storage and self.save is None and self.algo == hipops.ALGO_AUTO and self.nk <= 3
                and (all(isinstance(rb, ResBlock2) for rb in g.resblocks) or rb1_net) and x.shape[2] % 4 == 0 and g.h.num_wv_feat % 32 == 0
                and all((up.out_channels >= 64 and up.out_channels % 64 == 0) or up.out_channels in self.fuse_stage for up in g.ups)
                and all(up.in_channels % 32 == 0 and 2 <= up.stride <= 8 for up in g.ups)
                and g._bf16_storage_kernels_exist(self.B, self.T)):
            self.adt = torch.bfloat16
        self.st = self.adt == torch.bfloat16
        cs = g.cond_stream if g.cond_stream is not None else 3072 <= self.B * self.T <= 10240
        self.cond_sid = 2 if (self.st and self.training and cs) else 1
        self.joined = False
        self.S.fork(self.cond_sid)
        self.slab = g._slab(self.dev)
        self.y = None
        self.wps32 = {}
        self.up_done = None

    def buf(self, name, shape, dtype=torch.float32):
        return self.g._buf(name, shape, dtype=dtype, device=self.dev)

    def lkw(self, mul=None):
        if self.lens is None:
            return {}
        return dict(lengths=self.lens, len_mul=self.lmul if mul is None else mul)

    def weights(self):
        g, st, dev = self.g, self.st, self.dev
        B, ns = self.B, self.ns
        self.gbs = [self.buf(f'gb.{i}', (B, 2 * g.cbns[i].num_features)) for i in range(ns)]
        self.z_ws = self.buf('z_ws', (ns * B * _Z_CHANNEL,))
        self.sigma_ws = self.buf('sigma_ws', (ns,))
        self.affs = None
        self.cond_ran = False
        if self.cond_sid == 2:
            self.cond()
        with (self.on_side() if st else contextlib.nullcontext()):
            self.wf, self.wp = g._fold_weights(dev, need_wf=self.save is not None, bf16_only=st)
        self.wps = g._split_weights(dev, all_ups=st, ups_stream=self.S.side, mark=self.mark if st else None,
                                    between=self.cond if st else None)
        self.cond()

    def cond(self):
        if self.cond_ran:
            return
        self.cond_ran = True
        g, dev, ns, B = self.g, self.dev, self.ns, self.B
        with self.on_side(self.cond_sid):
            if not self.training and self.save is None:
                sn_p = [q for c in g.cbns for q in (c.layer.weight_orig, c.layer.weight_u, c.layer.weight_v)]
                skey = (tuple((q.data_ptr(), q._version) for q in sn_p), str(dev))
                if g._fold_key.get('sigma') != skey:
                    hipops.cond_sigma([c.layer.weight_orig.detach() for c in g.cbns], [c.layer.weight_u for c in g.cbns],
                                      [c.layer.weight_v for c in g.cbns], self.sigma_ws, training=False)
                    g._fold_key['sigma'] = skey
                self.affs = [(self.buf(f'bn.a{i}', (B, g.cbns[i].num_features)), self.buf(f'bn.s{i}', (B, g.cbns[i].num_features))) for i in range(ns)]
                hipops.cond_affine_eval(
                    self.spk, self.nz, [f.weight.detach() for f in g.fcs], [f.bias.detach() for f in g.fcs],
                    [c.layer.weight_orig.detach() for c in g.cbns], [c.layer.bias.detach() for c in g.cbns], self.sigma_ws,
                    [c.batch_nrom.running_mean for c in g.cbns], [c.batch_nrom.running_var for c in g.cbns],
                    [c.batch_nrom.eps for c in g.cbns], [q[0] for q in self.affs], [q[1] for q in self.affs])
            else:
                g._fold_key.pop('sigma', None)
                hipops.cond_gamma_beta(
                    self.spk, self.nz, [f.weight.detach() for f in g.fcs], [f.bias.detach() for f in g.fcs],
                    [c.layer.weight_orig.detach() for c in g.cbns], [c.layer.bias.detach() for c in g.cbns],
                    [c.layer.weight_u for c in g.cbns], [c.layer.weight_v for c in g.cbns], self.gbs, self.z_ws, self.sigma_ws, self.training)
        if self.st:
            self.mark('cond', self.cond_sid)

    def ck(self, nm, io=3):
        g = self.g
        if nm in self.wps32:
            return dict(algo=hipops.ALGO_BF16, wps=self.wps32[nm])
        if nm in self.wps and nm in g._split_wide:
            if self.st:
                return dict(algo=hipops.ALGO_BF16, wps=self.wps[nm], io_bf16=io)
            return dict(algo=hipops.ALGO_BF16 if g.precision == 'bf16' else hipops.ALGO_SPLIT, wps=self.wps[nm])
        if self.st:
            raise RuntimeError(f'bf16 storage: layer {nm} has no bf16 kernel (set generator.bf16_storage = False)')
        wpw = g._fold_key.get('wpw', {}).get(nm)
        if wpw is not None:
            return dict(algo=self.algo, wp=self.wp[nm], wpw=wpw)
        return dict(algo=self.algo, wp=self.wp[nm])

    def conv_pre(self):
        g = self.g
        self.cur = self.buf('act.pre', (self.B, g.h.upsample_initial_channel, self.T), dtype=self.adt)
        self.timed('conv_pre', hipops.conv1d, self.x, self.wf['conv_pre'], g.conv_pre.bias.detach(), self.cur, k=7, dil=1,
                   slope=1.0, splitk_ws=self.slab, **self.ck('conv_pre', io=2), **self.lkw())
        self.L = self.T

    def stage(self, i):
        self.stage_i = i
        up = self.g.ups[i]
        self.C, self.Lo = up.out_channels, self.L * up.stride
        self.xr = self.buf(f'act.up{i}', (self.B, self.C, self.Lo), dtype=self.adt)
        nt_stats, part = self.upsample(i)
        self.aff = self.statistics(i, nt_stats, part)
        self.need('rest', f'ups.{i + 1}' if i + 1 < self.ns else 'post')
        self.xs = self.buf(f'act.rb{i}', (self.B, self.C, self.Lo), dtype=self.adt)
        self.residual(i)
        self.cur, self.L = self.xs, self.Lo
        self.lmul *= self.g.ups[i].stride

    def upsample(self, i):
        g, st, up, C = self.g, self.st, self.g.ups[i], self.C
        B, L, dev = self.B, self.L, self.dev
        if st:
            if self.up_done is None:
                self.need(f'ups.{i}')
        elif f'ups.{i}' in self.wps:
            self.join_side()
        part, nt_stats = None, 0
        if self.training:
            if self.up_done is not None:
                nt_stats = self.up_done
            elif f'ups.{i}' in self.wps:
                nt_stats = hipops.convt_bf16_stats_tiles(self.cur, self.xr, up.kernel_size, up.stride, io_bf16=3 if st else 0)
            elif self.algo != hipops.ALGO_DIRECT and self.wp[f'ups.{i}'] is not None:
                nt_stats = hipops.convt_stats_tiles(B, up.in_channels, C, L, up.kernel_size, up.stride)
            if nt_stats:
                part = self.buf(f'bn.part{i}', (nt_stats * C * 2,))
        if self.up_done is not None:
            pass
        elif f'ups.{i}' in self.wps and (nt_stats or not self.training):
            self.timed(f'ups.{i}', hipops.convt1d_bf16, self.cur, self.wps[f'ups.{i}'], up.bias.detach(), self.xr, k=up.kernel_size,
                       u=up.stride, slope=LRELU_SLOPE, stats_part=part, io_bf16=3 if st else 0)
        elif st:
            raise RuntimeError(f'bf16 storage: ups.{i} has no bf16 kernel (set generator.bf16_storage = False)')
        else:
            self.timed(f'ups.{i}', hipops.convt1d, self.cur, self.wf[f'ups.{i}'], up.bias.detach(), self.xr, k=up.kernel_size,
                       u=up.stride, slope=LRELU_SLOPE, algo=self.algo, wp=self.wp[f'ups.{i}'], stats_part=part, splitk_ws=self.slab, **self.lkw())
        self.up_done = None
        return nt_stats, part

    def statistics(self, i, nt_stats, part):
        g, C, B, Lo = self.g, self.C, self.B, self.Lo
        bn = g.cbns[i].batch_nrom
        sliced = self.training and nt_stats >= 4096 and g.stat_sync is None and self.save is None
        stats = None
        fused = g.fuse_bn_finalize and self.training and not sliced and nt_stats and g.stat_sync is None and self.affs is None
        if self.training and not sliced:
            stats = self.buf(f'bn.stats{i}', (2 * C + 1,), dtype=torch.float64)
            if fused:
                pass
            elif nt_stats:
                hipops.bn_reduce_partials(part, nt_stats, C, B * Lo, stats)
            else:
                hipops.bn_stats(self.xr, stats, self.buf('bn.partial', (2 * max(C, 256) * 64,), dtype=torch.float64))
            if g.stat_sync is not None:
                sync = g.stat_sync
                self.timed(f'stat_sync.{i}', self.S.py, lambda: sync(stats))
        a_t, s_t = self.buf(f'bn.a{i}', (B, C)), self.buf(f'bn.s{i}', (B, C))
        self.need('cond')
        if not self.st:
            self.join_side()
        if sliced:
            sl = self.buf(f'bn.slices{i}', (hipops.BN_SLICES * 2 * C,), dtype=torch.float64)
            hipops.bn_reduce_finalize_slices(part, nt_stats, B * Lo, sl, self.gbs[i], bn.running_mean, bn.running_var, bn.num_batches_tracked,
                                             a_t, s_t, momentum=bn.momentum, eps=bn.eps)
        elif fused:
            hipops.bn_reduce_finalize(part, nt_stats, B * Lo, stats, self.gbs[i], bn.running_mean, bn.running_var, bn.num_batches_tracked,
                                      a_t, s_t, momentum=bn.momentum, eps=bn.eps)
        elif self.affs is None:
            hipops.bn_finalize(stats, self.gbs[i], bn.running_mean, bn.running_var, bn.num_batches_tracked, a_t, s_t,
                               training=self.training, momentum=bn.momentum, eps=bn.eps)
        return a_t, s_t

    def residual(self, i):
        from .models import ResBlock2
        g, nk = self.g, self.nk
        self.rbs = [g.resblocks[i * nk + j] for j in range(nk)]
        self.names = [f'resblocks.{i * nk + j}' for j in range(nk)]
        self.wps32 = {}
        if (self.save is not None and g.precision == 'bf16' and not self.st and self.C == 32 and self.Lo % 4 == 0 and self.algo == hipops.ALGO_AUTO
                and all(isinstance(rb, ResBlock2) and rb.kernel_size >= 3 and rb.kernel_size % 2 == 1 for rb in self.rbs)):
            for nm in self.names:
                for c in (0, 1):
                    self.wps32[f'{nm}.convs.{c}'] = hipops.pack_split(self.wf[f'{nm}.convs.{c}'], bf16=True)
        if not (self.algo != hipops.ALGO_DIRECT and nk <= 3):
            return self.residual_serial(i)
        B, C, Lo = self.B, self.C, self.Lo
        self.t1s = [self.buf(f'act.t1_{i}_{j}', (B, C, Lo), dtype=self.adt) for j in range(nk)]
        self.outs = [self.buf(f'act.o_{i}_{j}', (B, C, Lo), dtype=self.adt) for j in range(nk - 1)] + [self.xs]
        self.heavy_first = sorted(range(nk), key=lambda j: -self.rbs[j].kernel_size)
        if not isinstance(self.rbs[0], ResBlock2):
            return self.residual1(i)
        self.all_wps = all(f'{nm}.convs.{c}' in self.wps for nm in self.names for c in (0, 1))
        self.all_wp = all(self.wp.get(f'{nm}.convs.{c}') is not None for nm in self.names for c in (0, 1))
        for cand in (self.rb2_stage_with_upsampler, self.rb2_narrow_stage_split, self.rb2_wide_stage_bf16, self.rb2_stage_f32,
                     self.rb2_stage_small, self.rb2_pairs, self.rb2_branch_convs_bf16, self.rb2_layers):
            if cand(i):
                return
            if self.st and cand is self.rb2_wide_stage_bf16 and C in (16, 32):
                raise RuntimeError('bf16 storage: the fused narrow-stage kernel did not take this shape (set generator.bf16_storage = False)')

    def launch(self, tag_sfx, probs):
        probs = [probs[j] for j in self.heavy_first if j in probs]
        if self.lens is not None:
            lk = self.lkw(self.lmul * self.g.ups[self.stage_i].stride)
            probs = [(j, (*pr[:4], {**pr[4], **lk})) for j, pr in probs]
        tag = '+'.join(f'{self.names[j]}.{tag_sfx}' for j, _ in probs)
        self.timed(tag, hipops.conv1d_multi, [pr for _, pr in probs], splitk_ws=self.slab)

    def final_kw(self, j):
        if j < self.nk - 1:
            return {}
        return dict(add=self.outs[:self.nk - 1], out_div=float(self.nk))

    def stage_tag(self, sfx=''):
        return 'stage:' + '+'.join(f'{nm}.0&1' for nm in self.names) + sfx

    def rb2_stage_with_upsampler(self, i):
        g, C, B, Lo, rbs = self.g, self.C, self.B, self.Lo, self.rbs
        if not (self.st and g.fuse_up and i + 1 < self.ns and C >= 32 and (C >= 64 and g.fuse_wide_stage or C in self.fuse_stage)
                and f'ups.{i + 1}' in self.wps and self.all_wps):
            return False
        nup = g.ups[i + 1]
        if not (nup.kernel_size == 2 * nup.stride and nup.stride in (2, 4) and nup.out_channels * 2 == C):
            return False
        ntn = hipops.resblock2_stage_up_tiles(B, C, Lo, [rb.kernel_size for rb in rbs], [rb.convs[0].dilation for rb in rbs],
                                              [rb.convs[1].dilation for rb in rbs], slope=LRELU_SLOPE,
                                              up_k=nup.kernel_size, up_u=nup.stride, up_slope=LRELU_SLOPE)
        if not ntn:
            return False
        xr_n = self.buf(f'act.up{i + 1}', (B, nup.out_channels, Lo * nup.stride), dtype=self.adt)
        part_n = self.buf(f'bn.part{i + 1}', (ntn * nup.out_channels * 2,)) if self.training else None
        ok = self.timed(self.stage_tag(f'+ups.{i + 1}'), hipops.resblock2_stage_split, self.xr, self.aff, _branches(rbs, self.names, self.wps), None,
                        slope=LRELU_SLOPE, out_div=float(self.nk), bf16=True, io_bf16=3,
                        up=(self.wps[f'ups.{i + 1}'], nup.bias.detach(), xr_n, part_n, nup.kernel_size, nup.stride, LRELU_SLOPE))
        if ok:
            self.up_done = ntn
        return ok

    def rb2_narrow_stage_split(self, i):
        g, C, B, Lo, rbs = self.g, self.C, self.B, self.Lo, self.rbs
        if not (C in (16, 32) and C in self.fuse_stage and self.all_wps):
            return False
        branches = _branches(rbs, self.names, self.wps)
        std_set = [(rb.kernel_size, rb.convs[0].dilation, rb.convs[1].dilation) for rb in rbs] == [(3, 1, 3), (7, 1, 3), (11, 1, 3)]
        kp = g.conv_post.kernel_size
        if self.st and g.fuse_post and i == self.ns - 1 and C == 16 and kp <= 9 and ((std_set and kp == 7) or g.fuse_post == 'any'):
            y = torch.empty((B, 1, Lo), device=self.dev, dtype=torch.float32)
            if self.timed(self.stage_tag('+conv_post'), hipops.resblock2_stage_split, self.xr, self.aff, branches, None, slope=LRELU_SLOPE,
                          out_div=float(self.nk), bf16=True, io_bf16=3, post=(self.wf['conv_post'], g.conv_post.bias.detach(), y, kp, 0.01)):
                self.y = y
                return True
        return self.timed(self.stage_tag(), hipops.resblock2_stage_split, self.xr, self.aff, branches, self.xs, slope=LRELU_SLOPE,
                          out_div=float(self.nk), bf16=g.precision == 'bf16', io_bf16=3 if self.st else 0)

    def rb2_wide_stage_bf16(self, i):
        g = self.g
        if not (self.st and g.fuse_wide_stage and self.C >= 64 and self.all_wps):
            return False
        return self.timed(self.stage_tag(), hipops.resblock2_stage_split, self.xr, self.aff, _branches(self.rbs, self.names, self.wps), self.xs,
                          slope=LRELU_SLOPE, out_div=float(self.nk), bf16=True, io_bf16=3)

    def _f32_branches(self, w, k1, k2):
        return [dict(**{k1: w[nm + '.convs.0'], k2: w[nm + '.convs.1']}, b1=rb.convs[0].bias.detach(), b2=rb.convs[1].bias.detach(),
                     k=rb.kernel_size, dil1=rb.convs[0].dilation, dil2=rb.convs[1].dilation) for nm, rb in zip(self.names, self.rbs)]

    def rb2_stage_f32(self, i):
        g = self.g
        if self.st or not (self.C in self.fuse_stage and self.all_wp):
            return False
        lk = self.lkw(self.lmul * g.ups[i].stride)
        wpw = g._fold_key.get('wpw_stage', {})
        if (all(f'{nm}.convs.{c}' in wpw for nm in self.names for c in (0, 1)) and stage_wino_selected(
                g.wino_stage, g.precision, self.algo, self.C, [(rb.kernel_size, rb.convs[0].dilation, rb.convs[1].dilation) for rb in self.rbs])):
            if self.timed(self.stage_tag(), hipops.resblock2_stage_wino, self.xr, self.aff, self._f32_branches(wpw, 'wpw1', 'wpw2'), self.xs,
                          slope=LRELU_SLOPE, out_div=float(self.nk), **lk):
                return True
        branches = self._f32_branches(self.wp, 'wp1', 'wp2')
        kp = g.conv_post.kernel_size
        if g.fuse_post and i == self.ns - 1 and self.C == 16 and kp <= 9 and kp % 2 == 1 and g.conv_post.in_channels == 16:
            y = torch.empty((self.B, 1, self.Lo), device=self.dev, dtype=torch.float32)
            if self.timed(self.stage_tag('+conv_post'), hipops.resblock2_stage, self.xr, self.aff, branches, None, slope=LRELU_SLOPE,
                          out_div=float(self.nk), post=(self.wf['conv_post'], g.conv_post.bias.detach(), y, kp, 0.01), **lk):
                self.y = y
                return True
        return self.timed(self.stage_tag(), hipops.resblock2_stage, self.xr, self.aff, branches, self.xs, slope=LRELU_SLOPE, out_div=float(self.nk),
                          **lk)

    def rb2_stage_small(self, i):
        if not (self.C == 8 and 8 in self.fuse_stage and not self.st and self.nk <= 4
                and all(self.wf.get(f'{nm}.convs.{c}') is not None for nm in self.names for c in (0, 1))):
            return False
# ... 173 lines not shown
```

### wavthruvec_pytorch_amd/hipops.py

```python
from __future__ import annotations

import ctypes as C
from typing import Optional, Sequence

import torch

from . import _hip

ALGO_AUTO, ALGO_DIRECT, ALGO_MFMA, ALGO_SPLIT, ALGO_BF16, ALGO_WINO = (_hip.ALGO_AUTO, _hip.ALGO_DIRECT, _hip.ALGO_MFMA, _hip.ALGO_SPLIT,
                                                                        _hip.ALGO_BF16, _hip.ALGO_WINO)


def _chk(t: Optional[torch.Tensor], name: str, dtype=torch.float32):
    if t is None:
        return
    if not t.is_cuda:
        raise RuntimeError(f'{name} must live on a GPU: the Vec2Wav HIP path has no CPU fallback')
    if t.dtype != dtype:
        raise TypeError(f'{name} must be {dtype}, got {t.dtype}')
    if not t.is_contiguous():
        raise RuntimeError(f'{name} must be contiguous')


def _stream(t: torch.Tensor) -> int:
# ... 170 lines not shown
    def __init__(self):
        self.t = None
        self.retired = []

    def ensure(self, nbytes, device):
        if self.t is None or self.t.device != device or self.t.numel() * 4 < nbytes:
            if self.t is not None:
                self.retired.append(self.t)
            self.t = torch.empty(((nbytes + 3) // 4,), device=device, dtype=torch.float32)
        return self.t


def _attach_slab(a, slab, nbytes, device):
    if slab is not None and nbytes > 0:
        t = slab.ensure(int(nbytes), device)
        a.splitk_ws, a.splitk_ws_bytes = t.data_ptr(), t.numel() * 4


_SPLITK_BYTES = {}


def _splitk_bytes(a, n):
    qs = [a[i] for i in range(n)] if n > 1 else [a]
    key = (n,) + tuple((q.B, q.C_in, q.C_out, q.L, q.k, q.dil, q.algo, q.accumulate, q.in_stride, q.pad_left, q.in_ct, q.out_ct, q.io_bf16,
                        bool(q.res), bool(q.add0), bool(q.add1), bool(q.mask_src), bool(q.in_a), bool(q.rowsum_part), bool(q.wps), bool(q.wp),
                        q.out_div != 0.0, q.out_slope != 0.0) for q in qs)
    v = _SPLITK_BYTES.get(key)
    if v is None:
        v = _SPLITK_BYTES[key] = int(_hip.load().v2w_conv1d_splitk_ws_bytes(a if n > 1 else C.byref(a), n))
    return v


def conv1d(x, wf, bias, out, splitk_ws=None, **kw):
    if kw.get('wpw') is not None:
        conv1d_wino_multi([(x, wf, bias, out, kw)], splitk_ws=splitk_ws)
        return out
    kw.pop('wpw', None)
    kw, lengths, len_mul = _pop_len(kw)
    a = _hip.Conv1dArgs()
    _conv1d_args(a, x, wf, bias, out, **kw)
    if splitk_ws is not None:
        _attach_slab(a, splitk_ws, _splitk_bytes(a, 1), x.device)
    if lengths is not None:
        _hip.check(_hip.load().v2w_conv1d_fwd_len(C.byref(a), 1, _len_ptr(lengths, len_mul), len_mul, _stream(x)), 'v2w_conv1d_fwd_len')
        return out
    _hip.check(_hip.load().v2w_conv1d_fwd(C.byref(a), _stream(x)), 'v2w_conv1d_fwd')
    return out


def conv1d_multi(problems, splitk_ws=None):
    n = len(problems)
    if any(kw.get('wpw') is not None for *_r, kw in problems):
        return conv1d_wino_multi(problems, splitk_ws=splitk_ws)
    problems = [(x, wf, bias, out, {q: v for q, v in kw.items() if q != 'wpw'}) for x, wf, bias, out, kw in problems]
    if 1 < n <= 4:
        arr = (_hip.Conv1dArgs * n)()
        lengths = len_mul = None
        for a, (x, wf, bias, out, kw) in zip(arr, problems):
            kw, lengths, len_mul = _pop_len(kw)
            _conv1d_args(a, x, wf, bias, out, **kw)
        if splitk_ws is not None:
            _attach_slab(arr[0], splitk_ws, _splitk_bytes(arr, n), problems[0][0].device)
        if lengths is not None:
            rc = _hip.load().v2w_conv1d_fwd_len(arr, n, _len_ptr(lengths, len_mul), len_mul, _stream(problems[0][0]))
        else:
            rc = _hip.load().v2w_conv1d_fwd_multi(arr, n, _stream(problems[0][0]))
        if rc == 0:
            return
        if rc != -2:
            _hip.check(rc, 'v2w_conv1d_fwd_multi')
    for x, wf, bias, out, kw in problems:
        conv1d(x, wf, bias, out, splitk_ws=splitk_ws, **kw)


def conv1d_wino_multi(problems, splitk_ws=None):
    n = len(problems)
    if 1 <= n <= 4 and all(kw.get('wpw') is not None for *_r, kw in problems):
        arr = (_hip.Conv1dArgs * n)()
        lengths = len_mul = None
        for a, (x, wf, bias, out, kw) in zip(arr, problems):
            kw2, lengths, len_mul = _pop_len({q: v for q, v in kw.items() if q != 'wpw'})
            _conv1d_args(a, x, wf, bias, out, **{**kw2, 'algo': ALGO_WINO, 'wp': kw['wpw']})
        if lengths is not None:
            rc = _hip.load().v2w_conv1d_fwd_len(arr, n, _len_ptr(lengths, len_mul), len_mul, _stream(problems[0][0]))
        else:
            rc = _hip.load().v2w_conv1d_fwd_multi(arr, n, _stream(problems[0][0]))
        if rc == 0:
            return
        if rc != -2:
            _hip.check(rc, 'v2w_conv1d_fwd_multi')
    conv1d_multi([(x, wf, bias, out, {q: v for q, v in kw.items() if q != 'wpw'}) for x, wf, bias, out, kw in problems], splitk_ws=splitk_ws)


def conv1d_wino_sum(sources, out, *, dil, slope, out_div=0.0, in_affine=None, lengths=None, len_mul=1, order=None):
    n = len(sources)
    arr = (_hip.Conv1dArgs * max(n, 1))()
    for a, (x, wpw, bias, k) in zip(arr, sources):
        _conv1d_args(a, x, None, bias, out, k=k, dil=dil, slope=slope, out_div=out_div, algo=ALGO_WINO, wp=wpw, in_affine=in_affine)
    lp = _len_ptr(lengths, len_mul) if lengths is not None else None
    if order is None:
        rc = _hip.load().v2w_conv1d_wino_sum_fwd(arr, n, lp, int(len_mul), _stream(out))
    else:
        rc = _hip.load().v2w_conv1d_wino_sum_fwd_order(arr, n, lp, int(len_mul), (C.c_int32 * max(n, 1))(*order), _stream(out))
    if rc == -2:
        return False
    _hip.check(rc, 'v2w_conv1d_wino_sum_fwd')
    return True


def wino_multi_taken(n, B, c_out, L, dil):
    npairs = dil * ((L + 2 * dil - 1) // (2 * dil))
    return n * B * ((npairs + 63) // 64) * (c_out // 64) > 128


def conv1d_wino_fan(x, branches, *, dil, slope, in_affine=None, res=None, res_affine=None, lengths=None, len_mul=1, only_if_multi_wino=False):
    if lengths is not None:
        return False
    n = len(branches)
    if only_if_multi_wino and not wino_multi_taken(n, x.shape[0], branches[0][2].shape[1], x.shape[2], dil):
        return False
    arr = (_hip.Conv1dArgs * max(n, 1))()
    for a, (wpw, bias, out, k) in zip(arr, branches):
        _conv1d_args(a, x, None, bias, out, k=k, dil=dil, slope=slope, algo=ALGO_WINO, wp=wpw, in_affine=in_affine, res=res, res_affine=res_affine)
    rc = _hip.load().v2w_conv1d_wino_fan_fwd(arr, n, _stream(x))
    if rc == -2:
        return False
    _hip.check(rc, 'v2w_conv1d_wino_fan_fwd')
    return True


def wino_sum_order(ks):
    n = len(ks)
    out = (C.c_int32 * n)()
    _hip.check(_hip.load().v2w_wino_sum_order((C.c_int32 * n)(*ks), n, out), 'v2w_wino_sum_order')
    return tuple(out)


def convt1d(x, wf, bias, out, *, k, u, slope=1.0, algo=ALGO_AUTO, wp=None, stats_part=None, splitk_ws=None, lengths=None, len_mul=1):
    B, ci, L = x.shape
    a = _hip.ConvT1dArgs()
    a.in_ = x.data_ptr(); a.wf = _hip.ptr(wf); a.wp = _hip.ptr(wp); a.bias = _hip.ptr(bias); a.out = out.data_ptr()
    a.stats_part = _hip.ptr(stats_part)
    a.B, a.C_in, a.C_out, a.L, a.k, a.u = B, ci, out.shape[1], L, k, u
    a.slope = slope; a.algo = algo
    if splitk_ws is not None:
        _attach_slab(a, splitk_ws, _hip.load().v2w_convt1d_splitk_ws_bytes(C.byref(a)), x.device)
    if lengths is not None:
        _hip.check(_hip.load().v2w_convt1d_fwd_len(C.byref(a), _len_ptr(lengths, len_mul), int(len_mul), _stream(x)), 'v2w_convt1d_fwd_len')
        return out
    _hip.check(_hip.load().v2w_convt1d_fwd(C.byref(a), _stream(x)), 'v2w_convt1d_fwd')
    return out


def pack_bf16_convt(wf, u, out=None):
    k, ci, co = wf.shape
    nbytes = int(_hip.load().v2w_pack_bf16_convt_bytes(k, ci, co, u))
    if nbytes == 0:
        return None
    if out is None or out.numel() * out.element_size() < nbytes:
        out = torch.empty((nbytes // 2,), device=wf.device, dtype=torch.bfloat16)
    _hip.check(_hip.load().v2w_pack_bf16_convt(wf.data_ptr(), out.data_ptr(), k, ci, co, u, _stream(wf)), 'v2w_pack_bf16_convt')
    return out


def _convt_bf16_args(x, wps, bias, out, k, u, slope, stats_part, io_bf16=0):
    B, ci, L = x.shape
    a = _hip.ConvT1dArgs()
    a.in_ = x.data_ptr(); a.wf = None; a.wp = _hip.ptr(wps); a.bias = _hip.ptr(bias); a.out = _hip.ptr(out)
    a.stats_part = _hip.ptr(stats_part)
    a.B, a.C_in, a.C_out, a.L, a.k, a.u = B, ci, out.shape[1], L, k, u
    a.slope = slope; a.algo = ALGO_BF16; a.io_bf16 = io_bf16
    return a


def convt_bf16_stats_tiles(x, out, k, u, io_bf16=0):
    n = _hip.load().v2w_convt1d_bf16_tiles(C.byref(_convt_bf16_args(x, None, None, out, k, u, 1.0, None, io_bf16)))
    return n if n > 0 else 0


def convt1d_bf16(x, wps, bias, out, *, k, u, slope=1.0, stats_part=None, io_bf16=0):
    _hip.check(_hip.load().v2w_convt1d_bf16_fwd(C.byref(_convt_bf16_args(x, wps, bias, out, k, u, slope, stats_part, io_bf16)), _stream(x)),
               'v2w_convt1d_bf16_fwd')
    return out


def cond_gamma_beta(spk, noise, fc_w: Sequence, fc_b: Sequence, sn_w: Sequence, sn_b: Sequence,
                    sn_u: Sequence, sn_v: Sequence, gb: Sequence, z_ws, sigma_ws, training: bool):
    n = len(fc_w)
    if n > _hip.V2W_MAX_STAGES:
        raise ValueError(f'at most {_hip.V2W_MAX_STAGES} upsample stages are supported')
    a = _hip.CondArgs()
    a.spk = spk.data_ptr(); a.noise = noise.data_ptr()
    for i in range(n):
        a.fc_w[i] = fc_w[i].data_ptr(); a.fc_b[i] = fc_b[i].data_ptr()
        a.sn_w[i] = sn_w[i].data_ptr(); a.sn_b[i] = sn_b[i].data_ptr()
        a.sn_u[i] = sn_u[i].data_ptr(); a.sn_v[i] = sn_v[i].data_ptr()
        a.gb[i] = gb[i].data_ptr()
        a.C[i] = sn_w[i].shape[0] // 2
    a.z_ws = z_ws.data_ptr(); a.sigma_ws = sigma_ws.data_ptr()
    a.n_stages = n; a.B = spk.shape[0]; a.spk_dim = spk.shape[1]; a.noise_dim = noise.shape[1]
    a.training = int(training)
    _hip.check(_hip.load().v2w_cond_gamma_beta(C.byref(a), _stream(spk)), 'v2w_cond_gamma_beta')


def _cond_args(a, spk, noise, fc_w, fc_b, sn_w, sn_b, sn_u, sn_v, sigma_ws):
    n = len(sn_w)
    if n > _hip.V2W_MAX_STAGES:
        raise ValueError(f'at most {_hip.V2W_MAX_STAGES} upsample stages are supported')
    a.spk = _hip.ptr(spk); a.noise = _hip.ptr(noise)
    for i in range(n):
        a.fc_w[i] = _hip.ptr(fc_w[i]) if fc_w is not None else None
        a.fc_b[i] = _hip.ptr(fc_b[i]) if fc_b is not None else None
        a.sn_w[i] = sn_w[i].data_ptr(); a.sn_b[i] = _hip.ptr(sn_b[i]) if sn_b is not None else None
        a.sn_u[i] = _hip.ptr(sn_u[i]) if sn_u is not None else None
        a.sn_v[i] = _hip.ptr(sn_v[i]) if sn_v is not None else None
        a.C[i] = sn_w[i].shape[0] // 2
    a.sigma_ws = sigma_ws.data_ptr()
    a.n_stages = n
    if spk is not None:
        a.B = spk.shape[0]; a.spk_dim = spk.shape[1]; a.noise_dim = noise.shape[1]


def cond_sigma(sn_w: Sequence, sn_u: Sequence, sn_v: Sequence, sigma_ws, training: bool = False):
    a = _hip.CondArgs()
    _cond_args(a, None, None, None, None, sn_w, None, sn_u, sn_v, sigma_ws)
    a.training = int(training)
    _hip.check(_hip.load().v2w_cond_sigma(C.byref(a), _stream(sigma_ws)), 'v2w_cond_sigma')


def cond_affine_eval(spk, noise, fc_w: Sequence, fc_b: Sequence, sn_w: Sequence, sn_b: Sequence, sigma_ws,
                     running_mean: Sequence, running_var: Sequence, eps: Sequence, a_out: Sequence, s_out: Sequence):
    e = _hip.CondEvalArgs()
    _cond_args(e.c, spk, noise, fc_w, fc_b, sn_w, sn_b, None, None, sigma_ws)
    for i in range(len(sn_w)):
        e.running_mean[i] = running_mean[i].data_ptr(); e.running_var[i] = running_var[i].data_ptr()
        e.a_out[i] = a_out[i].data_ptr(); e.s_out[i] = s_out[i].data_ptr()
        e.eps[i] = eps[i]
    _hip.check(_hip.load().v2w_cond_affine_eval(C.byref(e), _stream(spk)), 'v2w_cond_affine_eval')


def bn_stats(x, stats, partial_ws):
    B, Cc, L = x.shape
    _hip.check(_hip.load().v2w_bn_stats(x.data_ptr(), stats.data_ptr(), partial_ws.data_ptr(), B, Cc, L, _stream(x)),
               'v2w_bn_stats')
    return stats


def bn_finalize(stats, gb, running_mean, running_var, num_batches_tracked, a_out, s_out, *, training: bool,
                momentum=0.1, eps=1e-5):
    B, C2 = gb.shape
    _hip.check(_hip.load().v2w_bn_finalize(_hip.ptr(stats), gb.data_ptr(), running_mean.data_ptr(), running_var.data_ptr(),
                                           _hip.ptr(num_batches_tracked), a_out.data_ptr(), s_out.data_ptr(),
                                           B, C2 // 2, int(training), momentum, eps, _stream(gb)), 'v2w_bn_finalize')


BN_SLICES = 128


def bn_reduce_finalize_slices(part, ntiles, count, slices, gb, running_mean, running_var, num_batches_tracked, a_out, s_out, *,
                              momentum=0.1, eps=1e-5):
    B, C2 = gb.shape
    Cc = C2 // 2
    lib, st = _hip.load(), _stream(part)
    _hip.check(lib.v2w_bn_reduce_slices(part.data_ptr(), ntiles, Cc, slices.data_ptr(), BN_SLICES, st), 'v2w_bn_reduce_slices')
    _hip.check(lib.v2w_bn_finalize_slices(slices.data_ptr(), BN_SLICES, float(count), gb.data_ptr(), running_mean.data_ptr(),
                                          running_var.data_ptr(), _hip.ptr(num_batches_tracked), a_out.data_ptr(), s_out.data_ptr(),
                                          B, Cc, momentum, eps, st), 'v2w_bn_finalize_slices')


def affine_apply(x, a, s, out):
    B, Cc, L = x.shape
    _hip.check(_hip.load().v2w_affine_apply(x.data_ptr(), a.data_ptr(), s.data_ptr(), out.data_ptr(), B, Cc, L, _stream(x)),
               'v2w_affine_apply')
    return out


def conv_post_tanh(x, wf, bias, out, *, k, slope, lengths=None, len_mul=1):
    B, ci, L = x.shape
    if lengths is not None:
        if x.dtype != torch.float32:
            raise NotImplementedError('conv_post_tanh: per-item lengths need fp32 input')
        _hip.check(_hip.load().v2w_conv_post_tanh_len(x.data_ptr(), wf.data_ptr(), _hip.ptr(bias), out.data_ptr(),
                                                      B, ci, L, k, slope, _len_ptr(lengths, len_mul), int(len_mul), _stream(x)), 'v2w_conv_post_tanh_len')
        return out
    if x.dtype == torch.bfloat16:
        _hip.check(_hip.load().v2w_conv_post_tanh_bf16in(x.data_ptr(), wf.data_ptr(), _hip.ptr(bias), out.data_ptr(),
                                                         B, ci, L, k, slope, _stream(x)), 'v2w_conv_post_tanh_bf16in')
        return out
    _hip.check(_hip.load().v2w_conv_post_tanh(x.data_ptr(), wf.data_ptr(), _hip.ptr(bias), out.data_ptr(),
                                              B, ci, L, k, slope, _stream(x)), 'v2w_conv_post_tanh')
    return out


def conv_tile_config(B, c_in, c_out, L, k, dil=1, u=1, prefix=False):
    cfg = (C.c_int32 * 10)()
    if u == 1:
        a = _hip.Conv1dArgs(); a.B, a.C_in, a.C_out, a.L, a.k, a.dil = B, c_in, c_out, L, k, dil
        a.pad_left = -1
        rc = _hip.load().v2w_conv1d_tile_config(C.byref(a), cfg)
    else:
        a = _hip.ConvT1dArgs(); a.B, a.C_in, a.C_out, a.L, a.k, a.u = B, c_in, c_out, L, k, u
        rc = _hip.load().v2w_convt1d_tile_config(C.byref(a), cfg)
    if rc != 0:
        return None
    pre = 'conv_tile_kernel<' + ', '.join(str(v) for v in cfg[:9]) + ', 0, '
    return pre if prefix else pre + ('true>' if L % 4 == 0 else 'false>')
# ... 1071 lines not shown
```

### wavthruvec_pytorch_amd/models.py

```python
from __future__ import annotations

import math
import warnings
from typing import Dict, List, Optional

import contextlib
import torch
import torch.nn as nn

from . import _hip, hipops
from .modules import ConditionalBatchNorm1d
from .utils import get_padding, init_weights

LRELU_SLOPE = 0.1
_SIDE_STREAMS: Dict[str, 'torch.cuda.Stream'] = {}
_CAPTURE_STREAMS: Dict[str, 'torch.cuda.Stream'] = {}
_Z_CHANNEL = 128


class _WNConvBase(nn.Module):
    transposed = False

    def __init__(self, in_channels, out_channels, kernel_size, stride=1, dilation=1, padding=0):
        super().__init__()
# ... 19 lines not shown
            w = v * (g / v.flatten(1).norm(dim=1).view(-1, 1, 1))
        del self._parameters['weight_g']
        del self._parameters['weight_v']
        self.weight = nn.Parameter(w.detach())

    def extra_repr(self):
        s = f'{self.in_channels}, {self.out_channels}, kernel_size=({self.kernel_size},), stride=({self.stride},)'
        if self.padding:
            s += f', padding=({self.padding},)'
        if self.dilation != 1:
            s += f', dilation=({self.dilation},)'
        return s


class Conv1d(_WNConvBase):
    transposed = False


class ConvTranspose1d(_WNConvBase):
    transposed = True


def _lrelu_conv(m, src, res=None):
    v, g = (m.weight_v.detach(), m.weight_g.detach()) if m.weight_normed else (m.weight.detach(), None)
    wf = hipops.fold_conv_weight(v, g)
    out = torch.empty_like(src)
    hipops.conv1d(src, wf, m.bias.detach(), out, k=m.kernel_size, dil=m.dilation, slope=LRELU_SLOPE, res=res, wp=hipops.pack_mfma(wf))
    return out, wf


def _resblock_steps(rb, x, pairs, keep=False):
    from .backward import PairStep
    name = {id(m): n for n, m in rb.named_modules()}
    cur, steps = x.detach().contiguous().float(), []
    for ca, cb in pairs:
        u = wfb = None
        if cb is None:
            out, wfa = _lrelu_conv(ca, cur, res=cur)
        else:
            u, wfa = _lrelu_conv(ca, cur)
            out, wfb = _lrelu_conv(cb, u, res=cur)
        if keep:
            steps.append(PairStep(cur, None, u, ca, name[id(ca)], wfa, cb, name.get(id(cb)), wfb))
        cur = out
    return cur, steps


def _resblock_forward(rb, x, pairs):
    if not x.is_cuda:
        raise RuntimeError('ResBlock (HIP): GPU tensors only; there is no CPU fallback')
    if torch.is_grad_enabled() and (x.requires_grad or any(p.requires_grad for p in rb.parameters())):
        from .backward import ResBlockFunction
        names, params = zip(*rb.named_parameters())
        return ResBlockFunction.apply(rb, pairs, names, x, *params)
    with torch.no_grad():
        return _resblock_steps(rb, x, pairs)[0]


class ResBlock1(nn.Module):

    def __init__(self, h, channels, kernel_size=3, dilation=(1, 3, 5)):
        super().__init__()
        self.h = h
        self.channels, self.kernel_size, self.dilation = channels, kernel_size, tuple(dilation)
        self.convs1 = nn.ModuleList([
            Conv1d(channels, channels, kernel_size, 1, dilation=d, padding=get_padding(kernel_size, d))
            for d in dilation[:3]])
        self.convs2 = nn.ModuleList([
            Conv1d(channels, channels, kernel_size, 1, dilation=1, padding=get_padding(kernel_size, 1))
            for _ in range(3)])

    @_hip.on_tensor_device
    def forward(self, x):
        return _resblock_forward(self, x, [(c1, c2) for c1, c2 in zip(self.convs1, self.convs2)])

    def remove_weight_norm(self):
        for l in self.convs1:
            l.remove_weight_norm()
        for l in self.convs2:
            l.remove_weight_norm()


class ResBlock2(nn.Module):

    def __init__(self, h, channels, kernel_size=3, dilation=(1, 3)):
        super().__init__()
        self.h = h
        self.channels, self.kernel_size, self.dilation = channels, kernel_size, tuple(dilation)
        self.convs = nn.ModuleList([
            Conv1d(channels, channels, kernel_size, 1, dilation=d, padding=get_padding(kernel_size, d))
            for d in dilation[:2]])

    @_hip.on_tensor_device
    def forward(self, x):
        return _resblock_forward(self, x, [(c, None) for c in self.convs])

    def remove_weight_norm(self):
        for l in self.convs:
            l.remove_weight_norm()


class Generator(nn.Module):

    def __init__(self, h):
        super().__init__()
        self.h = h
        self.num_kernels = len(h.resblock_kernel_sizes)
        self.num_upsamples = len(h.upsample_rates)
        if self.num_upsamples > 8:
            raise ValueError('at most 8 upsample stages are supported')
        c0 = h.upsample_initial_channel
        self.conv_pre = Conv1d(h.num_wv_feat, c0, 7, 1, padding=3)
        resblock = ResBlock1 if h.resblock == '1' else ResBlock2

        self.ups = nn.ModuleList()
        for i, (u, k) in enumerate(zip(h.upsample_rates, h.upsample_kernel_sizes)):
            self.ups.append(ConvTranspose1d(c0 // (2 ** i), c0 // (2 ** (i + 1)), k, u, padding=(k - u) // 2))

        self.resblocks = nn.ModuleList()
        ch = c0
        for i in range(len(self.ups)):
            ch = c0 // (2 ** (i + 1))
            for j, (k, d) in enumerate(zip(h.resblock_kernel_sizes, h.resblock_dilation_sizes)):
                self.resblocks.append(resblock(h, ch, k, d))

        self.conv_post = Conv1d(ch, 1, 7, 1, padding=3)

        self.cbns = nn.ModuleList()
        self.fcs = nn.ModuleList()
        for i in range(len(self.ups)):
            self.fcs.append(nn.Linear(h.spk_dim + h.noise_dim, _Z_CHANNEL))
            self.cbns.append(ConditionalBatchNorm1d(256 // pow(2, i)))
            if self.cbns[i].num_features != self.ups[i].out_channels:
                raise ValueError('ConditionalBatchNorm1d widths are 256 // 2**i (models.py:113): '
                                 'upsample_initial_channel must be 512')

        self.algo = hipops.ALGO_AUTO
        self.stat_sync = None
        self.always_refold = True
        self.fuse_pairs = (16,)
        self.fuse_stage = (8, 16, 32)
        self.precision = 'f32'
        self.split_min_channels = 64
        self.bf16_storage = True
        self.fuse_wide = True
        self.fuse_wide_stage = True
        self.fuse_up = True
        self.fuse_bn_finalize = True
        self.wino = True
        self.wino_stage = True
        self.wino_sum = (64,)
        self.wino_sum_wide = (256, 128)
        self.wino_fan = (64,)
        self.merge_waits = True
        self.cond_stream = None
        self.fuse_post = True
        self.fuse_stage_backward = False
        self._split_wide = set()
        self._ws: Dict[str, torch.Tensor] = {}
        self._slabs: Dict[tuple, 'hipops.SplitKSlab'] = {}
        self._wts: Dict[str, torch.Tensor] = {}
        self._fold_key: Dict[str, tuple] = {}
        self._profile = None
        self._profile_names = None
        self.use_launch_plan = True
        self._tapes: Dict[tuple, object] = {}
        self._ws_epoch = 0
        self._tape_refused = 0

    def __getstate__(self):
        st = self.__dict__.copy()
        st.update(_tapes={}, _ws={}, _slabs={}, _wts={}, _fold_key={}, _profile=None, _profile_names=None, _ws_epoch=0)
        return st

    def enable_sync_batchnorm(self, group=None, single_rank_collective=None):
        from .distributed import BNStatSync
        self.stat_sync = BNStatSync(group, single_rank_collective=single_rank_collective)
        return self

    def profile_kernel_names(self, x, spk_emb, noise):
        keep = self._profile
        self._profile, self._profile_names = [], {}
        try:
            with torch.no_grad():
                self.forward(x, spk_emb, noise)
            return dict(self._profile_names)
        finally:
            self._profile, self._profile_names = keep, None

    def capture_graph(self, x, spk_emb, noise, warmup: int = 2):
        if self.stat_sync is not None:
            raise RuntimeError('capture_graph: the RCCL statistics all-reduce cannot be part of a captured graph')
        sx, ss, sn = x.detach().clone().contiguous(), spk_emb.detach().clone().contiguous(), noise.detach().clone().contiguous()
        with torch.no_grad():
            side = _CAPTURE_STREAMS.get(str(sx.device))
            if side is None:
                side = _CAPTURE_STREAMS[str(sx.device)] = torch.cuda.Stream(device=sx.device)
            side.wait_stream(torch.cuda.current_stream(sx.device))
            with torch.cuda.stream(side):
                for _ in range(max(1, warmup)):
                    self.forward(sx, ss, sn)
            torch.cuda.current_stream(sx.device).wait_stream(side)
            graph = torch.cuda.CUDAGraph()
            with torch.cuda.graph(graph, stream=side):
                sy = self.forward(sx, ss, sn)

        epoch = self._ws_epoch

        def run(x, spk_emb, noise):
            if self._ws_epoch != epoch:
                raise RuntimeError('capture_graph: the module reallocated its buffers since this graph was captured (a forward of another '
                                   'configuration ran): capture again - a module serves one captured configuration at a time')
            if x.dtype == sx.dtype and spk_emb.dtype == ss.dtype and noise.dtype == sn.dtype and x.device == sx.device:
                torch._foreach_copy_([sx, ss, sn], [x, spk_emb, noise])
            else:
                sx.copy_(x); ss.copy_(spk_emb); sn.copy_(noise)
            graph.replay()
            return sy

        run.graph = graph
        return run

    def remove_weight_norm(self):
        print('Removing weight norm...')
        for l in self.ups:
            l.remove_weight_norm()
        for l in self.resblocks:
            l.remove_weight_norm()
        self.conv_pre.remove_weight_norm()
        self.conv_post.remove_weight_norm()

    @staticmethod
    def _side_stream(device, index=0):
        key = str(device) if index == 0 else f'{device}#{index}'
        st = _SIDE_STREAMS.get(key)
        if st is None:
            st = _SIDE_STREAMS[key] = torch.cuda.Stream(device=device)
        return st

    def _buf(self, name, shape, dtype=torch.float32, device=None):
        t = self._ws.get(name)
        if t is None or tuple(t.shape) != tuple(shape) or t.dtype != dtype or t.device != device:
            if t is not None:
                self._drop_tapes()
            t = torch.empty(shape, device=device, dtype=dtype)
            self._ws[name] = t
        return t

    def _drop_tapes(self):
        self._ws_epoch += 1
        self._tapes.clear()

    def _slab(self, device):
        key = (str(device), torch.cuda.current_stream(device).cuda_stream)
        slab = self._slabs.get(key)
        if slab is None:
            if len(self._slabs) >= 16:
                self._slabs.pop(next(iter(self._slabs)))
                self._drop_tapes()
            slab = self._slabs[key] = hipops.SplitKSlab()
        return slab

    def _wbuf(self, name, shape, dtype=torch.float32, device=None):
        t = self._wts.get(name)
        if t is None or tuple(t.shape) != tuple(shape) or t.dtype != dtype or t.device != device:
            if t is not None:
                self._drop_tapes()
            t = torch.empty(shape, device=device, dtype=dtype)
            self._wts[name] = t
        return t

    def _conv_layers(self):
        yield 'conv_pre', self.conv_pre
        for i, m in enumerate(self.ups):
            yield f'ups.{i}', m
        for i, rb in enumerate(self.resblocks):
            if isinstance(rb, ResBlock1):
                for n, m in enumerate(rb.convs1):
                    yield f'resblocks.{i}.convs1.{n}', m
                for n, m in enumerate(rb.convs2):
                    yield f'resblocks.{i}.convs2.{n}', m
            else:
                for n, m in enumerate(rb.convs):
                    yield f'resblocks.{i}.convs.{n}', m
        yield 'conv_post', self.conv_post

    def invalidate_weight_cache(self):
        self._fold_key.clear()

    def _fold_weights(self, device, need_wf=False, bf16_only=False):
        layers = list(self._conv_layers())
        vers = []
        for name, m in layers:
            ps = (m.weight_v, m.weight_g) if m.weight_normed else (m.weight,)
            vers.append(tuple((p.data_ptr(), p._version) for p in ps))
        wino = self.wino and self.precision == 'f32' and self.algo != hipops.ALGO_DIRECT
        stage_names = self._wino_stage_layers()
        sum_names = self._wino_sum_layers()
        state = (tuple(vers), self.algo, str(device), need_wf, bf16_only, wino, bool(stage_names), tuple(sorted(sum_names)))
        force = (self.training and self.always_refold) or need_wf
        if not force and self._fold_key.get('state') == state:
            return self._fold_key['wf'], self._fold_key['wp']
        wf, wp, batch = {}, {}, []
        wpd = {}
        wpw = {}
        wpw_stage = {}
        wpw_sum = {}
        for name, m in layers:
            if bf16_only and name != 'conv_post':
                wf[name], wp[name] = None, None
                continue
            v, g = (m.weight_v.detach(), m.weight_g.detach()) if m.weight_normed else (m.weight.detach(), None)
            u = m.stride if m.transposed else 1
            mfma_ok = (self.algo != hipops.ALGO_DIRECT and name != 'conv_post' and
                       hipops.conv_tile_config(1, m.in_channels, m.out_channels, 64, m.kernel_size,
                                               1 if m.transposed else m.dilation, u) is not None)
            wpwb = None
            if (mfma_ok and wino and not m.transposed and hipops.wino_terms(m.kernel_size) and m.in_channels % 32 == 0 and m.in_channels >= 64
                    and m.out_channels % 64 == 0 and (m.out_channels >= 128 or m.dilation == 1)):
                wpwb = wpw[name] = self._wbuf('wpw.' + name, (hipops.wino_terms(m.kernel_size) * m.in_channels * m.out_channels,), device=device)
            if mfma_ok and name in stage_names:
                wpwb = wpw_stage[name] = self._wbuf('wpw.' + name, (hipops.wino_terms(m.kernel_size) * m.in_channels * m.out_channels,), device=device)
            if mfma_ok and wpwb is None and name in sum_names:
                wpwb = wpw_sum[name] = self._wbuf('wpw.' + name, (hipops.wino_terms(m.kernel_size) * m.in_channels * m.out_channels,), device=device)
            if mfma_ok and need_wf:
                n_el = m.kernel_size * m.in_channels * m.out_channels
                wfb = self._wbuf('wf.' + name, (m.kernel_size, m.in_channels, m.out_channels), device=device)
                wpb = self._wbuf('wp.' + name, (n_el,), device=device)
                wdb = None
                if not m.transposed and m.in_channels == m.out_channels and name.startswith('resblocks.'):
                    wdb = wpd[name] = self._wbuf('wpd.' + name, (n_el,), device=device)
                batch.append((v, g, wpb, m.in_channels, m.out_channels, m.kernel_size, u, m.transposed, wfb, wdb, wpwb))
                wf[name], wp[name] = wfb, wpb
            elif mfma_ok:
                wpb = self._wbuf('wp.' + name, (m.kernel_size * m.in_channels * m.out_channels,), device=device)
                batch.append((v, g, wpb, m.in_channels, m.out_channels, m.kernel_size, u, m.transposed, None, None, wpwb))
                wf[name], wp[name] = None, wpb
            else:
                wfb = self._wbuf('wf.' + name, (m.kernel_size, m.in_channels, m.out_channels), device=device)
                scratch = self._wbuf('wf_scratch', (max(2048, m.out_channels, m.in_channels),), device=device)
                (hipops.fold_convt_weight if m.transposed else hipops.fold_conv_weight)(v, g, wfb, scratch)
                wf[name], wp[name] = wfb, None
        if batch:
            key = tuple((q[0].data_ptr(), 0 if q[1] is None else q[1].data_ptr(), q[2].data_ptr(),
                         0 if len(q) < 9 or q[8] is None else q[8].data_ptr(), 0 if len(q) < 11 or q[10] is None else q[10].data_ptr()) for q in batch)
            plan = self._fold_key.get('plan')
            if plan is None or plan.key != key:
                self._drop_tapes()
                plan = hipops.FoldPlan(batch, device)
                plan.key = key
                self._fold_key['plan'] = plan
            plan.run()
        self._fold_key.update(state=state, wf=wf, wp=wp, wpd=wpd, wpw=wpw, wpw_stage=wpw_stage, wpw_sum=wpw_sum, vers=tuple(vers), gen=self._fold_key.get('gen', 0) + 1)
        return wf, wp

    def _wino_stage_layers(self):
        from .forward_plan import stage_wino_selected
        names, nk = set(), self.num_kernels
        for i, up in enumerate(self.ups):
            rbs = [self.resblocks[i * nk + j] for j in range(nk)]
            if all(isinstance(rb, ResBlock2) for rb in rbs) and stage_wino_selected(
                    self.wino_stage, self.precision, self.algo, up.out_channels,
                    [(rb.kernel_size, rb.convs[0].dilation, rb.convs[1].dilation) for rb in rbs]):
                names.update(f'resblocks.{i * nk + j}.convs.{c}' for j in range(nk) for c in (0, 1))
        return names

    def _wino_sum_layers(self):
        from .forward_plan import wino_sum_selected
        names, nk = set(), self.num_kernels
        for i, up in enumerate(self.ups):
            rbs = [self.resblocks[i * nk + j] for j in range(nk)]
            if all(isinstance(rb, ResBlock2) for rb in rbs) and wino_sum_selected(
                    self.wino_sum, self.precision, self.algo, up.out_channels, [(rb.kernel_size, rb.convs[1].dilation) for rb in rbs]):
                names.update(f'resblocks.{i * nk + j}.convs.1' for j in range(nk))
        return names

    def _split_weights(self, device, all_ups=False, ups_stream=None, mark=None, between=None):
        if self.precision == 'f32' or self.algo == hipops.ALGO_DIRECT:
            return {}
        if self.precision not in ('f16x3', 'bf16'):
            raise ValueError(f"Generator.precision must be 'f32', 'f16x3' or 'bf16', got {self.precision!r}")
        gen = (self._fold_key.get('gen', 0), self.precision, all_ups)
        cached = self._fold_key.get('wps')
        if cached is not None and cached[0] == gen:
            return cached[1]
        out, batch = {}, []
        self._split_wide = set()
        picked = []
        for name, m in self._conv_layers():
            if m.transposed or name == 'conv_post':
                continue
            stage32 = (m.in_channels == m.out_channels and m.out_channels in (16, 32) and m.out_channels in self.fuse_stage
                       and name.startswith('resblocks.') and ('.convs.' in name or (all_ups and self.precision == 'bf16')))
            wide = (m.out_channels >= self.split_min_channels and hipops.split_supported(m.in_channels, m.out_channels)
                    and m.kernel_size % 2 == 1 and m.kernel_size >= 3)
            if wide or stage32:
                picked.append((name, m, wide))
        sizes = [hipops.split_halves(m.kernel_size, m.in_channels, m.out_channels) if wide
                 else hipops.split_units_halves(m.kernel_size, m.in_channels, m.out_channels) for _n, m, wide in picked]
        arena = self._buf('wps.arena', (sum(sizes) + 1024,), dtype=torch.float16, device=device)
        scs = self._buf('wsc.arena', (4 * max(1, len(picked)),), device=device)
        off = 0
        for i, ((name, m, wide), n) in enumerate(zip(picked, sizes)):
            v, g = (m.weight_v.detach(), m.weight_g.detach()) if m.weight_normed else (m.weight.detach(), None)
            wpsb, scb = arena[off:off + n], scs[4 * i:4 * i + 4]
            off += n
            batch.append((v.contiguous(), g, wpsb, scb))
            out[name] = (wpsb, scb)
            if wide:
                self._split_wide.add(name)
        first = [q for (nm, _m, _w), q in zip(picked, batch) if nm == 'conv_pre'] if ups_stream is not None else batch
        rest = [q for (nm, _m, _w), q in zip(picked, batch) if nm != 'conv_pre'] if ups_stream is not None else []
        if mark is None or ups_stream is None:
            def mark(name):
                pass

        def run_plan(slot, sub, strm):
            if not sub:
                return
            key = tuple((v.data_ptr(), 0 if g is None else g.data_ptr(), w.data_ptr()) for (v, g, w, _s) in sub) + (self.precision,)
            plan = self._fold_key.get(slot)
            if plan is None or plan.key != key:
                self._drop_tapes()
                plan = hipops.SplitPlan(sub, device, bf16=self.precision == 'bf16')
                plan.key = key
                self._fold_key[slot] = plan
            with (torch.cuda.stream(strm) if strm is not None else contextlib.nullcontext()):
                plan.run()

        def fold_up(i, m):
            v, g = (m.weight_v.detach(), m.weight_g.detach()) if m.weight_normed else (m.weight.detach(), None)
            wfb = self._buf(f'wfbf.ups.{i}', (m.kernel_size, m.in_channels, m.out_channels), device=device)
            scratch = self._buf('wf_scratch_ups', (max(2048, m.out_channels, m.in_channels),), device=device)
            with (torch.cuda.stream(ups_stream) if ups_stream is not None else contextlib.nullcontext()):
                hipops.fold_convt_weight(v, g, wfb, scratch)
                w = hipops.pack_bf16_convt(wfb, m.stride, out=self._ws.get(f'wpsbf.ups.{i}'))
            if w is not None:
                if self._ws.get(f'wpsbf.ups.{i}') is not w:
                    self._drop_tapes()
                self._ws[f'wpsbf.ups.{i}'] = w
                out[f'ups.{i}'] = w
            if i == 0:
                mark(f'ups.{i}')

        ups_bf = [(i, m) for i, m in enumerate(self.ups) if self.precision == 'bf16' and (m.out_channels >= 64 or all_ups)]
        run_plan('split_plan', first, None)
        if ups_bf and ups_bf[0][0] == 0:
            fold_up(*ups_bf.pop(0))
        if between is not None:
            between()
        for i, m in ups_bf:
            fold_up(i, m)
        run_plan('split_plan_rest', rest, ups_stream)
        mark('rest')
        self._fold_key['wps'] = (gen, out)
        return out

    def _bf16_storage_kernels_exist(self, B, T) -> bool:
        key = (B, T, self.num_kernels, tuple(self.fuse_stage))
        hit = self._fold_key.get('bf16_storage_ok')
        if hit is not None and hit[0] == key:
            return hit[1]
        ok = hipops.conv_bf16_config(B, 1, self.conv_pre.in_channels, self.conv_pre.out_channels, T, 7, 1, 1, io_bf16=2) is not None
        L, nk = T, self.num_kernels
        for i, up in enumerate(self.ups):
            ok = ok and hipops.conv_bf16_config(B, 1, up.in_channels, up.out_channels, L, up.kernel_size, 1, up.stride, io_bf16=3) is not None
            L *= up.stride
            C = up.out_channels
            rbs = self.resblocks[i * nk:(i + 1) * nk]
            if isinstance(rbs[0], ResBlock1):
                for n in range(3):
                    pair = hipops.resblock1_pairs_ok(B, C, L, [rb.kernel_size for rb in rbs], [rb.convs1[n].dilation for rb in rbs],
                                                     [1] * len(rbs), slope=LRELU_SLOPE)
                    convs = C >= 64 and all(rb.kernel_size >= 3 and
                                            hipops.conv_bf16_config(B, 1, C, C, L, rb.kernel_size, rb.convs1[n].dilation, 1, io_bf16=3) is not None and
                                            hipops.conv_bf16_config(B, 1, C, C, L, rb.kernel_size, 1, 1, io_bf16=3) is not None for rb in rbs)
                    ok = ok and all(rb.kernel_size % 2 == 1 for rb in rbs) and (pair or convs)
            elif C in (16, 32):
                ok = ok and all(rb.kernel_size % 2 == 1 for rb in rbs) and hipops.resblock2_stage_split_ok(
                    B, C, L, [rb.kernel_size for rb in rbs], [rb.convs[0].dilation for rb in rbs], [rb.convs[1].dilation for rb in rbs],
                    slope=LRELU_SLOPE)
            else:
                for rb in rbs:
                    for c in rb.convs:
                        ok = ok and rb.kernel_size % 2 == 1 and rb.kernel_size >= 3 and \
                            hipops.conv_bf16_config(B, 1, C, C, L, rb.kernel_size, c.dilation, 1, io_bf16=3) is not None
        self._fold_key['bf16_storage_ok'] = (key, bool(ok))
        return bool(ok)

    @_hip.on_tensor_device
    def forward(self, x, spk_emb=None, noise=None, lengths=None):
        if spk_emb is None or noise is None:
            raise TypeError('Generator.forward: spk_emb and noise are required')
        if not (x.is_cuda and spk_emb.is_cuda and noise.is_cuda):
            raise RuntimeError('Generator.forward runs on the MI355X HIP path only: move inputs and module to a GPU '
                               '(there is no CPU/PyTorch fallback)')
        dev = x.device
        if self.conv_pre.bias.device != dev:
            raise RuntimeError(f'Generator parameters live on {self.conv_pre.bias.device}, inputs on {dev}')
        if x.dim() != 3 or x.shape[1] != self.h.num_wv_feat:
            raise RuntimeError(f'expected x of shape (B, {self.h.num_wv_feat}, T), got {tuple(x.shape)}')
        needs_grad = torch.is_grad_enabled() and (x.requires_grad or any(p.requires_grad for p in self.parameters()))
        x_in = x.contiguous().float()
        x = x_in.detach()
        spk = spk_emb.detach().contiguous().float()
        nz = noise.detach().contiguous().float()
        if spk.shape != (x.shape[0], self.h.spk_dim) or nz.shape != (x.shape[0], self.h.noise_dim):
            raise RuntimeError('spk_emb / noise must be (B, spk_dim) / (B, noise_dim)')
        if lengths is not None:
            lens = self._lengths_buffer(lengths, x, needs_grad)
            return self._forward_hip(x, spk, nz, None, lens=lens)
        if needs_grad:
            if self.algo == hipops.ALGO_DIRECT:
                raise NotImplementedError('Generator (HIP): the scalar cross-check kernels (algo = ALGO_DIRECT) serve no-grad forwards only; '
                                          'back-propagation needs the MFMA schedule (algo = ALGO_AUTO)')
            from .backward import GeneratorFunction
            names, params = zip(*[(n, q) for n, q in self.named_parameters()])
            return GeneratorFunction.apply(self, names, x_in if x_in.requires_grad else x, spk, nz, *params)
        return self._forward_hip(x, spk, nz, None)

    def _lengths_buffer(self, lengths, x, needs_grad):
        if self.training:
            raise ValueError('Generator.forward(lengths=...): eval mode only - BatchNorm batch statistics over a padded batch are not the '
                             "reference's per-utterance semantics")
        if needs_grad:
            raise NotImplementedError('Generator.forward(lengths=...): no-grad forwards only (run it under torch.no_grad())')
        if self.precision != 'f32':
            raise NotImplementedError(f"Generator.forward(lengths=...): precision 'f32' only, not {self.precision!r}")
        if self.algo != hipops.ALGO_AUTO:
            raise NotImplementedError('Generator.forward(lengths=...): algo = ALGO_AUTO only')
        if not all(isinstance(rb, ResBlock2) for rb in self.resblocks) or self.num_upsamples != 5 or self.num_kernels > 3:
            raise NotImplementedError('Generator.forward(lengths=...): ResBlock2 generators with five upsample stages and at most three '
                                      'branches only')
        B, T = x.shape[0], x.shape[2]
        if torch.is_tensor(lengths):
            if lengths.dtype.is_floating_point or lengths.dtype.is_complex or lengths.dtype == torch.bool or tuple(lengths.shape) != (B,):
                raise ValueError(f'lengths must hold {B} integers')
            src = lengths.detach()
        else:
            vals = [int(n) for n in lengths]
            if len(vals) != B:
                raise ValueError(f'lengths must hold {B} integers, got {len(vals)}')
            src = torch.tensor(vals, dtype=torch.int32)
        if not src.is_cuda and (src.numel() and (int(src.min()) < 1 or int(src.max()) > T)):
            raise ValueError(f'lengths must lie in [1, T = {T}]')
        buf = self._buf('lengths', (B,), dtype=torch.int32, device=x.device)
        buf.copy_(src.to(torch.int32))
        return buf

    def _plan_key(self, x):
        ptrs = tuple(p.data_ptr() for p in self.parameters()) + tuple(b.data_ptr() for b in self.buffers())
        return (tuple(x.shape), str(x.device), torch.cuda.current_stream(x.device).cuda_stream, self.training, self.precision, self.algo, self.bf16_storage, tuple(self.fuse_stage), tuple(self.fuse_pairs),
                self.fuse_wide, self.fuse_wide_stage, self.fuse_up, self.fuse_post, self.fuse_bn_finalize, self.cond_stream, self.merge_waits, self.split_min_channels,
                self.always_refold, self.wino, self.wino_stage, tuple(self.wino_sum), tuple(self.wino_sum_wide), tuple(self.wino_fan), ptrs)

    def _forward_hip(self, x, spk, nz, save, lens=None):
        from .forward_plan import ForwardPlanner, DirectStreams
        from . import schedule
        dev = x.device
        main, side, side2 = torch.cuda.current_stream(dev), self._side_stream(dev), self._side_stream(dev, 1)
        if save is not None or not self.use_launch_plan or self.stat_sync is not None:
            return ForwardPlanner(self, x, spk, nz, save, DirectStreams(main, side, side2), lens=lens).run()
        key, refold = self._tape_key(x)
        key = key + (('lengths',) if lens is not None else ())
        tape = self._tapes.get(key)
        if tape is not None:
            y = torch.empty(tape.out[0], device=dev, dtype=tape.out[1])
            tape.replay(main, side, dict(x=x.data_ptr(), spk=spk.data_ptr(), nz=nz.data_ptr(), y=y.data_ptr()), self._profile, side2)
            if self._profile_names is not None:
                self._profile_names.update(tape.kernel_names())
            if refold is not None:
                wvers, sigma = refold
                if wvers is not None:
                    self._fold_key['gen'] = self._fold_key.get('gen', 0) + 1
                    if wvers:
                        self._fold_key.update(vers=wvers, state=(wvers,) + tape.fold_state_tail)
                if sigma:
                    self._fold_key['sigma'] = self._sigma_key(dev)
            if self.training:
                self._fold_key.pop('sigma', None)
            return y
        if self._profile is not None:
            return ForwardPlanner(self, x, spk, nz, None, DirectStreams(main, side, side2), lens=lens).run()
        rec = schedule.Recorder(_hip.load(), main, side, side2)
        epoch = self._ws_epoch
        prev = _hip.set_recorder(rec)
        try:
            y = ForwardPlanner(self, x, spk, nz, None, rec, lens=lens).run()
        finally:
            _hip.set_recorder(prev)
        binds = dict(x=x.data_ptr(), spk=spk.data_ptr(), nz=nz.data_ptr(), y=y.data_ptr())
        if self._ws_epoch != epoch:
            self._tapes.clear()
        state = self._fold_key.get('state')
        if len(set(binds.values())) == 4 and state is not None:
            try:
                rec.tape.finalize(binds, owned=self._owned_ranges())
            except schedule.TapeNotOwned:
                self._tape_refused += 1
                return y
            rec.tape.out = (tuple(y.shape), y.dtype)
            rec.tape.fold_state_tail = tuple(state[1:])
            self._tapes[key] = rec.tape
        return y

    def _owned_ranges(self):
        from . import schedule
        ts = list(self.parameters()) + list(self.buffers()) + list(self._ws.values()) + list(self._wts.values())
        for slab in self._slabs.values():
            ts += [slab.t] + list(slab.retired)
        ts += list(schedule.tensors_in(self._fold_key))
        return schedule.owned_ranges(ts)

    def _sigma_key(self, dev):
        sn_p = [q for c in self.cbns for q in (c.layer.weight_orig, c.layer.weight_u, c.layer.weight_v)]
        return (tuple((q.data_ptr(), q._version) for q in sn_p), str(dev))

    def _tape_key(self, x):
        base = self._plan_key(x)
        if self.training and self.always_refold:
            return base + ('refold',), ((), False)
        vers = self._param_versions()
        wstale = not (self._fold_key.get('vers') == vers and self._fold_key.get('state') is not None)
        sstale = (not self.training) and self._fold_key.get('sigma') != self._sigma_key(x.device)
        if not (wstale or sstale):
            return base + ('folded',), None
        return base + (('w' if wstale else '') + ('s' if sstale else ''),), (vers if wstale else None, sstale)

    def _param_versions(self):
        vers = []
        for _name, m in self._conv_layers():
            ps = (m.weight_v, m.weight_g) if m.weight_normed else (m.weight,)
            vers.append(tuple((p.data_ptr(), p._version) for p in ps))
        return tuple(vers)
```

Baseline: 358.7 million samples/s.

## Add Winograd MFMA kernel for stride-2/4 transposed-conv upsamplers

Adds a Winograd-form transposed-convolution kernel for upsample layers where k = 2u and u is 2 or 4. The layer is rewritten as a polyphase two-tap conv with pre-transformed packed weights built during weight folding, which cuts the multiply count. Output write, bias and per-tile BatchNorm partial statistics are fused into the epilogue. It is enabled by default for ups 1-3 in the f32 MFMA path. If the launch reports a shape error it falls back to the existing convt path, at the cost of extra code and weight buffers.

```diff
diff --git a/include/vec2wav_hip.h b/include/vec2wav_hip.h
--- a/include/vec2wav_hip.h
+++ b/include/vec2wav_hip.h
@@ -262,6 +262,8 @@
 int v2w_conv1d_wino_sum_fwd_order(const v2w_conv1d_args* a, int n, const int32_t* len, int len_mul, const int32_t* order, void* stream);
 int v2w_wino_sum_order(const int32_t* k, int n, int32_t* order);
 int v2w_conv1d_wino_fan_fwd(const v2w_conv1d_args* a, int n, void* stream);
+int v2w_convt1d_wino_fwd(const v2w_convt1d_args* a, const float* in_a, const float* in_s, void* stream);
+int v2w_convt1d_wino_tiles(const v2w_convt1d_args* a, int32_t* wgs);
 int v2w_resblock2_stage_fwd_len(const v2w_stage_args* a, const int32_t* len, int len_mul, void* stream);
 int v2w_conv_post_tanh_len(const float* in, const float* wf, const float* bias, float* out,
                            int B, int C_in, int L, int k, float slope, const int32_t* len, int len_mul, void* stream);
diff --git a/wavthruvec_pytorch_amd/_hip.py b/wavthruvec_pytorch_amd/_hip.py
--- a/wavthruvec_pytorch_amd/_hip.py
+++ b/wavthruvec_pytorch_amd/_hip.py
@@ -250,6 +250,8 @@
     'v2w_conv1d_wino_sum_fwd_order': (C.c_int, [C.POINTER(Conv1dArgs), C.c_int, _fp, C.c_int, C.POINTER(C.c_int32), _fp]),
     'v2w_wino_sum_order': (C.c_int, [C.POINTER(C.c_int32), C.c_int, C.POINTER(C.c_int32)]),
     'v2w_conv1d_wino_fan_fwd': (C.c_int, [C.POINTER(Conv1dArgs), C.c_int, _fp]),
+    'v2w_convt1d_wino_fwd': (C.c_int, [C.POINTER(ConvT1dArgs), _fp, _fp, _fp]),
+    'v2w_convt1d_wino_tiles': (C.c_int, [C.POINTER(ConvT1dArgs), C.POINTER(C.c_int32)]),
     'v2w_resblock2_stage_fwd_len': (C.c_int, [C.POINTER(StageArgs), _fp, C.c_int, _fp]),
     'v2w_conv_post_tanh_len': (C.c_int, [_fp, _fp, _fp, _fp, C.c_int, C.c_int, C.c_int, C.c_int, C.c_float, _fp, C.c_int, _fp]),
     'v2w_mel_phases_len': (C.c_int, [_fp, _fp, C.c_int, C.c_int, C.c_int, C.c_int, C.c_int, _fp, C.c_int, _fp]),
diff --git a/wavthruvec_pytorch_amd/csrc/v2w_conv_mfma.hip b/wavthruvec_pytorch_amd/csrc/v2w_conv_mfma.hip
--- a/wavthruvec_pytorch_amd/csrc/v2w_conv_mfma.hip
+++ b/wavthruvec_pytorch_amd/csrc/v2w_conv_mfma.hip
@@ -768,7 +768,21 @@
         const int c = gg * CKG + j * KSTEP + lane / MF, co = lane % MF;
         dst[o] = d.transposed ? tile[c * rstride + co * K + t] : tile[co * rstride + c * K + t];
     }
-    if (d.wpw) {
+    if (d.wpw && d.transposed) {
+        constexpr int NT = wino_seg_terms(2), WGPC = 4;
+        const int nchw = nch / 2;
+        for (int o = threadIdx.x; o < U * GPC * NT * 256; o += 256) {
+            const int j = o & 3, lane = (o >> 2) & 63;
+            int rest = o >> 8;
+            const int term = rest % NT; rest /= NT;
+            const int g2 = rest % GPC, r = rest / GPC;
+            const int row = r * 32 + lane % 32, co = row / U, ph = row - co * U;
+            const int c = g2 * CKG + j * KSTEP + lane / MF;
+            const float* w = tile + c * rstride + co * K;
+            const int fi = ((ch & 1) * GPC + g2) * NT + term;
+            d.wpw[((((size_t)(mb * U + r) * nchw + ch / 2) * (NT * WGPC) + fi) * 64 + lane) * 4 + j] = wino_weight(2, term, w[ph + U], w[ph], 0.f);
+        }
+    } else if (d.wpw) {
         const int nfr = wino_terms(K) * GPC;
         float* dw = d.wpw + (size_t)(mb * nch + ch) * nfr * 256;
         for (int o = threadIdx.x; o < nfr * 256; o += 256) {
@@ -932,7 +946,9 @@
         if (!cfg.mf) return V2W_E_SHAPE;
         d.mf = cfg.mf; d.ck = cfg.ck;
         if (d.wpd && (d.transposed || d.c_in != d.c_out || cfg.mf != cfg.ck)) return V2W_E_ARG;
-        if (d.wpw && (d.transposed || cfg.mf != 32 || cfg.ck != 32 || wino_terms(d.k) == 0)) return V2W_E_ARG;
+        if (d.wpw && !d.transposed && (cfg.mf != 32 || cfg.ck != 32 || wino_terms(d.k) == 0)) return V2W_E_ARG;
+        if (d.wpw && d.transposed && (cfg.mf != 32 || cfg.ck != 16 || (d.u != 2 && d.u != 4) || d.k != 2 * d.u || d.c_in % 32 != 0 || d.c_in < 64
+                                      || (d.u * d.c_out) % 64 != 0)) return V2W_E_ARG;
         starts[i] = bs; starts[n + 1 + i] = bp;
         bs += d.transposed ? d.c_in : d.c_out;
         bp += (d.c_out / cfg.mf) * (d.c_in / cfg.ck);
diff --git a/wavthruvec_pytorch_amd/csrc/v2w_conv_wino.hip b/wavthruvec_pytorch_amd/csrc/v2w_conv_wino.hip
--- a/wavthruvec_pytorch_amd/csrc/v2w_conv_wino.hip
+++ b/wavthruvec_pytorch_amd/csrc/v2w_conv_wino.hip
@@ -34,7 +34,11 @@
     int K[WSRC], hl[WSRC];
     int nsrc;
 };
+template <int U> struct WinoUpArgs { TileArgs p; };
+template <class A> struct wino_up_of { static constexpr int value = 0; };
+template <int U> struct wino_up_of<WinoUpArgs<U>> { static constexpr int value = U; };
 __device__ __forceinline__ const TileArgs& wino_problem(const MultiArgs& m, int pq) { return m.p[pq]; }
+template <int U> __device__ __forceinline__ const TileArgs& wino_problem(const WinoUpArgs<U>& a, int) { return a.p; }
 __device__ __forceinline__ const TileArgs& wino_problem(const WinoSumArgs& a, int) { return a.p; }
 __device__ __forceinline__ const TileArgs& wino_problem(const WinoFanArgs& a, int) { return a.p; }
 
@@ -42,7 +46,9 @@
 __device__ __forceinline__ void conv_wino_body(const ARGS& m) {
     constexpr bool SUM = std::is_same<ARGS, WinoSumArgs>::value;
     constexpr bool FAN = std::is_same<ARGS, WinoFanArgs>::value;
+    constexpr int UP = wino_up_of<ARGS>::value;
     static_assert(!FAN || (MI == 1 && !LEN), "the fan-out form is written for MI = 1 without per-item lengths");
+    static_assert(!UP || (MI == 1 && !LEN && (UP == 2 || UP == 4)), "the upsampler form is written for MI = 1, stride 2 / 4, without per-item lengths");
     typedef Frag<32> F;
     typedef F::acc_t acc_t;
     constexpr int WM = 2;
@@ -54,7 +60,7 @@
     extern __shared__ __attribute__((aligned(16))) float smem[];
 
     int pq = 0, id = blockIdx.x;
-    if constexpr (!SUM && !FAN) { pq = tile_problem(m); id = blockIdx.x - m.start[pq]; }
+    if constexpr (!SUM && !FAN && !UP) { pq = tile_problem(m); id = blockIdx.x - m.start[pq]; }
     const TileArgs& p = wino_problem(m, pq);
     const int mtiles = p.Cout / MT;
     const TileId ti = tile_coords(mtiles, id);
@@ -62,7 +68,7 @@
     if (ti.tile >= p.ntiles) return;
     const int d = p.dil;
     int b, tl;
-    wino_tile_order(ti.tile, p.B, p.ntl, wino_npairs(p.L, d) % NTP != 0, b, tl);
+    wino_tile_order(ti.tile, p.B, p.ntl, wino_npairs(UP ? p.L + 1 : p.L, d) % NTP != 0, b, tl);
     const int P0 = tl * NTP;
     const int m0 = mt * MT;
     int Lb = p.L;
@@ -79,7 +85,7 @@
     const int hk = lane >> 5;
     const int wm0 = (wave / WN) * (32 * MI);
     const int wn0 = (wave % WN) * 32;
-    const bool live = wino_tpos(P0 + wn0, d) < Lb;
+    const bool live = wino_tpos(P0 + wn0, d) < (UP ? Lb + 1 : Lb);
     const int L = p.L;
     int K = p.K, hl = p.hl;
     const float* sin = p.in;
@@ -169,7 +175,7 @@
         }
     };
 
-    int nfrag = nch * wino_terms(K) * WGPC;
+    int nfrag = nch * (UP ? wino_seg_terms(2) : wino_terms(K)) * WGPC;
     const f32x4* ap[MI];
 #pragma unroll
     for (int i = 0; i < MI; ++i)
@@ -226,6 +232,10 @@
             for (int j = 0; j < nsrc; ++j) etab[j * MT + c] = m.bias[j] ? m.bias[j][m0 + c] : 0.f;
             etab[WSRC * MT + c] = p.res_a ? p.res_a[b * p.Cout + m0 + c] : 1.f;
             etab[(WSRC + 1) * MT + c] = p.res_a ? p.res_s[b * p.Cout + m0 + c] : 0.f;
+            continue;
+        }
+        if constexpr (UP) {
+            etab[c] = p.bias ? p.bias[(m0 + c) / UP] : 0.f;
             continue;
         }
         if constexpr (SUM) {
@@ -309,10 +319,13 @@
             int cn = (ch + 1) * WCK;
             if (live) {
                 const float* xt = Xs + lbase;
-                int s = 0;
-                for (; s + 3 <= K; s += 3) segment(S3{}, xt + s * dstep, dstep);
-                if (K - s == 2) segment(S2{}, xt + s * dstep, dstep);
-                else if (K - s == 1) segment(S1{}, xt + s * dstep, dstep);
+                if constexpr (UP) segment(S2{}, xt, dstep);
+                else {
+                    int s = 0;
+                    for (; s + 3 <= K; s += 3) segment(S3{}, xt + s * dstep, dstep);
+                    if (K - s == 2) segment(S2{}, xt + s * dstep, dstep);
+                    else if (K - s == 1) segment(S1{}, xt + s * dstep, dstep);
+                }
             }
             if constexpr (SUM) {
                 if (!more && js + 1 < nsrc) {
@@ -359,6 +372,57 @@
         }
     }
     if constexpr (FAN) return;
+
+    if constexpr (UP) {
+        constexpr int PAD = UP / 2, NV = 2 * UP, CT = MT / UP;
+        float* const stats = p.stats_part;
+        if (!live && !stats) return;
+        float* const outp = p.out;
+        const int Lo = UP * L, o0 = UP * t0 - PAD;
+        const bool evec = p.evec != 0;
+        float* const red = etab + MT;
+#pragma unroll
+        for (int r0 = 0; r0 < 16; r0 += UP) {
+            const int row = wm0 + F::row(r0, hk);
+            const float bias = etab[row];
+            float v[NV];
+#pragma unroll
+            for (int ph = 0; ph < UP; ++ph) {
+                const float M0 = acc[0][0][r0 + ph], M1 = acc[1][0][r0 + ph], M3 = acc[3][0][r0 + ph];
+                v[ph] = (M0 + M1) + bias; v[UP + ph] = (M1 - M3) + bias;
+            }
+            float* const orow = outp + ((size_t)b * p.CoutT + (m0 + row) / UP) * Lo;
+            float s1 = 0.f, s2 = 0.f;
+#pragma unroll
+            for (int i = 0; i < NV; ++i) {
+                const int o = o0 + i;
+                const bool ok = live && o >= 0 && o < Lo;
+                if (ok) { s1 += v[i]; s2 = fmaf(v[i], v[i], s2); }
+                if (!ok) continue;
+                if (((i ^ PAD) & 1) == 0 && i + 1 < NV && evec) { f32x2 w = {v[i], v[i + 1]}; *reinterpret_cast<f32x2*>(orow + o) = w; }
+                else if (((i ^ PAD) & 1) == 0 || i == 0 || !evec) orow[o] = v[i];
+            }
+            if (stats) {
+#pragma unroll
+                for (int off = 16; off > 0; off >>= 1) { s1 += __shfl_xor(s1, off, 64); s2 += __shfl_xor(s2, off, 64); }
+                if (lr == 0) {
+                    red[((wave % WN) * CT + row / UP) * 2 + 0] = s1;
+                    red[((wave % WN) * CT + row / UP) * 2 + 1] = s2;
+                }
+            }
+        }
+        if (stats) {
+            __syncthreads();
+            for (int c = tid; c < CT; c += NTHREADS) {
+                float t1 = 0.f, t2 = 0.f;
+#pragma unroll
+                for (int w = 0; w < WN; ++w) { t1 += red[(w * CT + c) * 2]; t2 += red[(w * CT + c) * 2 + 1]; }
+                stats[((size_t)ti.tile * p.CoutT + m0 / UP + c) * 2 + 0] = t1;
+                stats[((size_t)ti.tile * p.CoutT + m0 / UP + c) * 2 + 1] = t2;
+            }
+        }
+        return;
+    }
 
     if (!live) return;
     float* const outp = p.out;
@@ -465,6 +529,12 @@
 template <int MI, int WN, int NPF, bool VEC>
 __global__ void __launch_bounds__(128 * WN, 3)
 conv_wino_fan_kernel(const WinoFanArgs a) {
+    conv_wino_body<MI, WN, NPF, VEC, false>(a);
+}
+
+template <int U, int MI, int WN, int NPF, bool VEC>
+__global__ void __launch_bounds__(128 * WN, 3)
+conv_wino_up_kernel(const WinoUpArgs<U> a) {
     conv_wino_body<MI, WN, NPF, VEC, false>(a);
 }
 
@@ -598,6 +668,45 @@
     const int grid = tile_blocks(p.ntiles, p.Cout / MT);
     auto kern = vec ? conv_wino_fan_kernel<MI, WN, NPF, true> : conv_wino_fan_kernel<MI, WN, NPF, false>;
     return v2w_launch_lds(kern, dim3(grid), dim3(NTHREADS), lds, stream, a);
+}
+
+constexpr int WUP_NTP = 64, WUP_MT = 64;
+template <int U>
+int launch_wino_up(TileArgs p, hipStream_t stream) {
+    constexpr int MI = 1, WN = 2, MT = WUP_MT, NTP = WUP_NTP, NTHREADS = 128 * WN;
+    constexpr int NPF = ((WCK / 2) * (((2 * NTP + 2 * WHMAX) / 4 + 7) / 8 * 8) + NTHREADS - 1) / NTHREADS;
+    static_assert(MT == 64 * MI && NTP == 32 * WN, "tile of the one-conv kernel");
+    p.ntl = (wino_npairs(p.L + 1, 1) + NTP - 1) / NTP;
+    p.ntiles = p.B * p.ntl;
+    int rows = 0;
+    for (int tl = 0; tl < p.ntl; ++tl) {
+        const int P0 = tl * NTP;
+        const int pos0 = (wino_tpos(P0, 1) - p.hl) & ~3;
+        const int r = wino_tpos(P0 + NTP - 1, 1) + 1 + p.hr - pos0 + 1;
+        if (r > rows) rows = r;
+    }
+    p.xrows = (rows + 3) & ~3;
+    if (p.xrows > 2 * NTP + 2 * WHMAX) return V2W_E_SHAPE;
+    const bool vec = (p.L % 4 == 0) && v2w_al16(p.in);
+    p.vec4 = vec;
+    p.evec = (reinterpret_cast<uintptr_t>(p.out) & 7) == 0;
+    const int nbuf = p.Cin / WCK > 1 ? 2 : 1;
+    p.atab_off = nbuf * p.xrows * WG::RS;
+    const size_t lds = ((size_t)p.atab_off + 3 * MT + (p.in_a ? 2 * p.Cin : 0)) * sizeof(float);
+    WinoUpArgs<U> a{};
+    a.p = p;
+    const int grid = tile_blocks(p.ntiles, p.Cout / MT);
+    auto kern = vec ? conv_wino_up_kernel<U, MI, WN, NPF, true> : conv_wino_up_kernel<U, MI, WN, NPF, false>;
+    return v2w_launch_lds(kern, dim3(grid), dim3(NTHREADS), lds, stream, a);
+}
+
+int wino_up_shape(const v2w_convt1d_args* a) {
+    if (!a) return V2W_E_ARG;
+    if (a->B <= 0 || a->C_in <= 0 || a->C_out <= 0 || a->L <= 0 || a->k <= 0 || a->u <= 0 || a->io_bf16 != 0) return V2W_E_ARG;
+    if ((a->u != 2 && a->u != 4) || a->k != 2 * a->u) return V2W_E_SHAPE;
+    if (a->C_in % WCK != 0 || a->C_in < 64 || (a->u * a->C_out) % WUP_MT != 0) return V2W_E_SHAPE;
+    if ((long long)a->u * a->L >= (1ll << 31) - 4 * WUP_NTP * a->u) return V2W_E_SHAPE;
+    return 0;
 }
 
 __global__ void __launch_bounds__(256)
@@ -705,6 +814,26 @@
     return launch_wino_fan<1, 2>(ps, n, (hipStream_t)stream);
 }
 
+extern "C" int v2w_convt1d_wino_fwd(const v2w_convt1d_args* a, const float* in_a, const float* in_s, void* stream) {
+    if (const int rc = wino_up_shape(a)) return rc;
+    if (!a->in || !a->wp || !a->out || (in_a == nullptr) != (in_s == nullptr)) return V2W_E_ARG;
+    TileArgs p{};
+    p.in = a->in; p.in_a = in_a; p.in_s = in_s; p.wp = a->wp; p.bias = a->bias; p.out = a->out; p.stats_part = a->stats_part;
+    p.B = a->B; p.Cin = p.CinT = a->C_in; p.Cout = a->u * a->C_out; p.CoutT = a->C_out; p.L = a->L; p.K = 2; p.dil = 1;
+    p.hl = 1; p.hr = 0; p.pad = a->u / 2; p.up_u = a->u;
+    p.slope = a->slope;
+    return a->u == 4 ? launch_wino_up<4>(p, (hipStream_t)stream) : launch_wino_up<2>(p, (hipStream_t)stream);
+}
+
+extern "C" int v2w_convt1d_wino_tiles(const v2w_convt1d_args* a, int32_t* wgs) {
+    if (const int rc = wino_up_shape(a)) return rc;
+    const long long ntl = (wino_npairs(a->L + 1, 1) + WUP_NTP - 1) / WUP_NTP;
+    const long long tiles = (long long)a->B * ntl, w = tiles * (a->u * a->C_out / WUP_MT);
+    if (w >= (1ll << 31)) return V2W_E_SHAPE;
+    if (wgs) *wgs = (int32_t)w;
+    return (int)tiles;
+}
+
 extern "C" int v2w_wino_sum_order(const int32_t* k, int n, int32_t* order) {
     if (!k || !order || n < 1 || n > WSRC) return V2W_E_ARG;
     int Ks[WSRC], walk[WSRC];
diff --git a/wavthruvec_pytorch_amd/forward_plan.py b/wavthruvec_pytorch_amd/forward_plan.py
--- a/wavthruvec_pytorch_amd/forward_plan.py
+++ b/wavthruvec_pytorch_amd/forward_plan.py
@@ -62,6 +62,15 @@
     blocks = list(blocks)
     return (C in tuple(wino_fan or ()) and precision == 'f32' and algo != hipops.ALGO_DIRECT and not save and not lengths and bool(streams)
             and 1 <= len(blocks) <= 3 and all(k >= 3 and k % 2 == 1 and d == blocks[0][1] for k, d in blocks))
+
+
+def wino_up_shape(c_in, c_out, k, u) -> bool:
+    return u in (2, 4) and k == 2 * u and c_in % 32 == 0 and c_in >= 64 and (u * c_out) % 64 == 0
+
+
+def wino_up_selected(wino_up, i, precision, algo, c_in, c_out, k, u, *, save=False, lengths=False, stream=True) -> bool:
+    return (i in tuple(wino_up or ()) and precision == 'f32' and algo != hipops.ALGO_DIRECT and wino_up_shape(c_in, c_out, k, u)
+            and not save and not lengths and bool(stream))
 
 
 def _branches(rbs, names, wps):
@@ -272,9 +281,12 @@
         elif f'ups.{i}' in self.wps:
             self.join_side()
         part, nt_stats = None, 0
+        wpw, nt_wino = self.wino_up(i)
         if self.training:
             if self.up_done is not None:
                 nt_stats = self.up_done
+            elif nt_wino:
+                nt_stats = nt_wino
             elif f'ups.{i}' in self.wps:
                 nt_stats = hipops.convt_bf16_stats_tiles(self.cur, self.xr, up.kernel_size, up.stride, io_bf16=3 if st else 0)
             elif self.algo != hipops.ALGO_DIRECT and self.wp[f'ups.{i}'] is not None:
@@ -283,6 +295,15 @@
                 part = self.buf(f'bn.part{i}', (nt_stats * C * 2,))
         if self.up_done is not None:
             pass
+        elif nt_wino and self.timed(f'ups.{i}', hipops.convt1d_wino, self.cur, wpw, up.bias.detach(), self.xr, k=up.kernel_size, u=up.stride,
+                                    slope=LRELU_SLOPE, stats_part=part):
+            pass
+        elif nt_wino:
+            if self.training:
+                nt_stats = hipops.convt_stats_tiles(B, up.in_channels, C, L, up.kernel_size, up.stride)
+                part = self.buf(f'bn.part{i}', (nt_stats * C * 2,)) if nt_stats else None
+            self.timed(f'ups.{i}', hipops.convt1d, self.cur, self.wf[f'ups.{i}'], up.bias.detach(), self.xr, k=up.kernel_size,
+                       u=up.stride, slope=LRELU_SLOPE, algo=self.algo, wp=self.wp[f'ups.{i}'], stats_part=part, splitk_ws=self.slab)
         elif f'ups.{i}' in self.wps and (nt_stats or not self.training):
             self.timed(f'ups.{i}', hipops.convt1d_bf16, self.cur, self.wps[f'ups.{i}'], up.bias.detach(), self.xr, k=up.kernel_size,
                        u=up.stride, slope=LRELU_SLOPE, stats_part=part, io_bf16=3 if st else 0)
@@ -293,6 +314,16 @@
                        u=up.stride, slope=LRELU_SLOPE, algo=self.algo, wp=self.wp[f'ups.{i}'], stats_part=part, splitk_ws=self.slab, **self.lkw())
         self.up_done = None
         return nt_stats, part
+
+    def wino_up(self, i):
+        g, up = self.g, self.g.ups[i]
+        wpw = g._fold_key.get('wpw_up', {}).get(f'ups.{i}')
+        if (self.st or self.up_done is not None or f'ups.{i}' in self.wps
+                or not wino_up_selected(g.wino_up, i, g.precision, self.algo, up.in_channels, up.out_channels, up.kernel_size, up.stride,
+                                        save=self.save is not None, lengths=self.lens is not None, stream=wpw is not None)):
+            return None, 0
+        tiles, wgs = hipops.convt_wino_tiles(self.B, up.in_channels, up.out_channels, self.L, up.kernel_size, up.stride)
+        return (wpw, tiles) if tiles and wgs > 128 else (None, 0)
 
     def statistics(self, i, nt_stats, part):
         g, C, B, Lo = self.g, self.C, self.B, self.Lo
diff --git a/wavthruvec_pytorch_amd/hipops.py b/wavthruvec_pytorch_amd/hipops.py
--- a/wavthruvec_pytorch_amd/hipops.py
+++ b/wavthruvec_pytorch_amd/hipops.py
@@ -346,6 +346,28 @@
     return out
 
 
+def convt_wino_tiles(B, c_in, c_out, L, k, u):
+    a = _hip.ConvT1dArgs(); a.B, a.C_in, a.C_out, a.L, a.k, a.u = B, c_in, c_out, L, k, u
+    wgs = C.c_int32(0)
+    tiles = _hip.load().v2w_convt1d_wino_tiles(C.byref(a), C.byref(wgs))
+    return (int(tiles), int(wgs.value)) if tiles > 0 else (0, 0)
+
+
+def convt1d_wino(x, wpw, bias, out, *, k, u, slope=1.0, in_affine=None, stats_part=None):
+    B, ci, L = x.shape
+    a = _hip.ConvT1dArgs()
+    a.in_ = x.data_ptr(); a.wp = _hip.ptr(wpw); a.bias = _hip.ptr(bias); a.out = out.data_ptr()
+    a.stats_part = _hip.ptr(stats_part)
+    a.B, a.C_in, a.C_out, a.L, a.k, a.u = B, ci, out.shape[1], L, k, u
+    a.slope = slope
+    ia, is_ = (None, None) if in_affine is None else in_affine
+    rc = _hip.load().v2w_convt1d_wino_fwd(C.byref(a), _hip.ptr(ia), _hip.ptr(is_), _stream(x))
+    if rc == -2:
+        return False
+    _hip.check(rc, 'v2w_convt1d_wino_fwd')
+    return True
+
+
 def pack_bf16_convt(wf, u, out=None):
     k, ci, co = wf.shape
     nbytes = int(_hip.load().v2w_pack_bf16_convt_bytes(k, ci, co, u))
diff --git a/wavthruvec_pytorch_amd/models.py b/wavthruvec_pytorch_amd/models.py
--- a/wavthruvec_pytorch_amd/models.py
+++ b/wavthruvec_pytorch_amd/models.py
@@ -195,6 +195,7 @@
         self.wino_sum = (64,)
         self.wino_sum_wide = (256, 128)
         self.wino_fan = (64,)
+        self.wino_up = (1, 2, 3)
         self.merge_waits = True
         self.cond_stream = None
         self.fuse_post = True
@@ -340,7 +341,8 @@
         wino = self.wino and self.precision == 'f32' and self.algo != hipops.ALGO_DIRECT
         stage_names = self._wino_stage_layers()
         sum_names = self._wino_sum_layers()
-        state = (tuple(vers), self.algo, str(device), need_wf, bf16_only, wino, bool(stage_names), tuple(sorted(sum_names)))
+        up_names = set() if need_wf else self._wino_up_layers()
+        state = (tuple(vers), self.algo, str(device), need_wf, bf16_only, wino, bool(stage_names), tuple(sorted(sum_names)), tuple(sorted(up_names)))
         force = (self.training and self.always_refold) or need_wf
         if not force and self._fold_key.get('state') == state:
             return self._fold_key['wf'], self._fold_key['wp']
@@ -349,6 +351,7 @@
         wpw = {}
         wpw_stage = {}
         wpw_sum = {}
+        wpw_up = {}
         for name, m in layers:
             if bf16_only and name != 'conv_post':
                 wf[name], wp[name] = None, None
@@ -366,6 +369,8 @@
                 wpwb = wpw_stage[name] = self._wbuf('wpw.' + name, (hipops.wino_terms(m.kernel_size) * m.in_channels * m.out_channels,), device=device)
             if mfma_ok and wpwb is None and name in sum_names:
                 wpwb = wpw_sum[name] = self._wbuf('wpw.' + name, (hipops.wino_terms(m.kernel_size) * m.in_channels * m.out_channels,), device=device)
+            if mfma_ok and name in up_names:
+                wpwb = wpw_up[name] = self._wbuf('wpw.' + name, (3 * m.stride * m.out_channels * m.in_channels,), device=device)
             if mfma_ok and need_wf:
                 n_el = m.kernel_size * m.in_channels * m.out_channels
                 wfb = self._wbuf('wf.' + name, (m.kernel_size, m.in_channels, m.out_channels), device=device)
@@ -394,7 +399,7 @@
                 plan.key = key
                 self._fold_key['plan'] = plan
             plan.run()
-        self._fold_key.update(state=state, wf=wf, wp=wp, wpd=wpd, wpw=wpw, wpw_stage=wpw_stage, wpw_sum=wpw_sum, vers=tuple(vers), gen=self._fold_key.get('gen', 0) + 1)
+        self._fold_key.update(state=state, wf=wf, wp=wp, wpd=wpd, wpw=wpw, wpw_stage=wpw_stage, wpw_sum=wpw_sum, wpw_up=wpw_up, vers=tuple(vers), gen=self._fold_key.get('gen', 0) + 1)
         return wf, wp
 
     def _wino_stage_layers(self):
@@ -407,6 +412,11 @@
                     [(rb.kernel_size, rb.convs[0].dilation, rb.convs[1].dilation) for rb in rbs]):
                 names.update(f'resblocks.{i * nk + j}.convs.{c}' for j in range(nk) for c in (0, 1))
         return names
+
+    def _wino_up_layers(self):
+        from .forward_plan import wino_up_selected
+        return {f'ups.{i}' for i, up in enumerate(self.ups)
+                if wino_up_selected(self.wino_up, i, self.precision, self.algo, up.in_channels, up.out_channels, up.kernel_size, up.stride)}
 
     def _wino_sum_layers(self):
         from .forward_plan import wino_sum_selected
@@ -595,7 +605,7 @@
         ptrs = tuple(p.data_ptr() for p in self.parameters()) + tuple(b.data_ptr() for b in self.buffers())
         return (tuple(x.shape), str(x.device), torch.cuda.current_stream(x.device).cuda_stream, self.training, self.precision, self.algo, self.bf16_storage, tuple(self.fuse_stage), tuple(self.fuse_pairs),
                 self.fuse_wide, self.fuse_wide_stage, self.fuse_up, self.fuse_post, self.fuse_bn_finalize, self.cond_stream, self.merge_waits, self.split_min_channels,
-                self.always_refold, self.wino, self.wino_stage, tuple(self.wino_sum), tuple(self.wino_sum_wide), tuple(self.wino_fan), ptrs)
+                self.always_refold, self.wino, self.wino_stage, tuple(self.wino_sum), tuple(self.wino_sum_wide), tuple(self.wino_fan), tuple(self.wino_up), ptrs)
 
     def _forward_hip(self, x, spk, nz, save, lens=None):
         from .forward_plan import ForwardPlanner, DirectStreams
```

Measured after the change: 364.1 million samples/s (median of 6 runs). 1.5% higher.
